# DataZooDE/anofox-forecast

Measured on AMD Instinct MI355X. Metric: series/sec fit+forecast, AutoETS h=28 on M5-shape batches, higher is better.
Workload: dtype f64

## Files before the change

### anofox-forecast_amd/csrc/ets_device.hpp

```cpp
#pragma once
#include <hip/hip_runtime.h>
#include <type_traits>
#include "det_math.hpp"
#include "nm.hpp"

namespace anofox {

enum { C_NONE = 0, C_ADD = 1, C_MUL = 2 };

constexpr double ETS_TOL = 1.0e-10;
constexpr double ETS_HUGEN = 1.0e10;
constexpr double ETS_LN2 = 0.693147180559945309417232121458;
constexpr double PAR_LO = 1.0e-4, PAR_HI = 0.9999, PHI_LO = 0.8, PHI_HI = 0.98;
constexpr int ETS_MERGED_LDS_PERIOD = 16;
constexpr int ETS_LDS_PERIOD = 64;
constexpr int ETS_MAX_PERIOD = 2048;

struct SeriesView {
    const double *y;
    size_t ld;
    int len;
    int wave_len;
    int wave_min_len;
    int rows;
    const double *yb;
    int col;
};

__device__ __forceinline__ int wave_max_i32(int v)
{
#pragma unroll
    for (int o = 32; o >= 1; o >>= 1) { int w = __shfl_xor(v, o); v = w > v ? w : v; }
    return v;
}
__device__ __forceinline__ int wave_min_i32(int v)
{
#pragma unroll
    for (int o = 32; o >= 1; o >>= 1) { int w = __shfl_xor(v, o); v = w < v ? w : v; }
    return v;
}

enum { YT_F64 = 0, YT_F32 = 1, YT_U16 = 2 };
template <class YT> struct YtCode;
template <> struct YtCode<double> { static constexpr int value = YT_F64; };
template <> struct YtCode<float> { static constexpr int value = YT_F32; };
template <> struct YtCode<unsigned short> { static constexpr int value = YT_U16; };
#ifndef ANOFOX_DM_RETRY
#define ANOFOX_DM_RETRY 0
#endif
#ifndef ANOFOX_TWO_BLOCK
#define ANOFOX_TWO_BLOCK 1
#endif
#ifndef ANOFOX_S_DM
#define ANOFOX_S_DM 8
#endif
#ifndef ANOFOX_S_GEN
#define ANOFOX_S_GEN 16
#endif
#ifndef ANOFOX_S_HBM_RING_COMPACT
#define ANOFOX_S_HBM_RING_COMPACT 16
#endif
#ifndef ANOFOX_S_COMPACT_MUL
#define ANOFOX_S_COMPACT_MUL 2
#endif
#ifndef ANOFOX_S_COMPACT_MUL_ADD
#define ANOFOX_S_COMPACT_MUL_ADD 1
#endif
#ifndef ANOFOX_K4_S_SEAS
#define ANOFOX_K4_S_SEAS 8
#endif
template <int ERR, int TREND, bool DAMPED, int SEAS>
struct EtsCfg {
    static constexpr int E = ERR, T = TREND, S = SEAS;
    static constexpr bool D = DAMPED;
    static constexpr int DIM = 1 + (TREND != C_NONE) + (SEAS != C_NONE) + (DAMPED ? 1 : 0);
    static constexpr bool ADDITIVE = (ERR == C_ADD) && (TREND != C_MUL) && (SEAS != C_MUL);
    static constexpr bool CLASSIC = false;
};

struct EtsPar { double alpha, bstar, phi, beta, gamma; DmPowLane pl; DmPowNear1 pc; };
struct EtsState { double l, b, sse, mant; int eacc; int bad; double f; double dlo, dhi, bmin; double rfar; };

template <class Cfg>
__device__ __forceinline__ void ets_unpack(const double (&x)[Cfg::DIM], EtsPar &p)
{
    int k = 0;
    p.alpha = x[k++];
    p.bstar = 0.0;
    double gstar = 0.0;
    p.phi = 1.0;
    if constexpr (Cfg::T != C_NONE) p.bstar = x[k++];
    if constexpr (Cfg::S != C_NONE) gstar = x[k++];
    if constexpr (Cfg::D) p.phi = x[k++];
    p.beta = p.alpha * p.bstar;
    p.gamma = gstar * (1.0 - p.alpha);
}

template <class Cfg, bool NEAR = false>
__device__ __forceinline__ void ets_step(const EtsPar &p, EtsState &st, double y, double &s)
{
    if constexpr (Cfg::ADDITIVE) {
        double phib = 0.0, q = st.l;
        if constexpr (Cfg::T == C_ADD) {
            phib = Cfg::D ? p.phi * st.b : st.b;
            q = st.l + phib;
        }
        double f = q;
        if constexpr (Cfg::S == C_ADD) f = q + s;
        double e = y - f;
        st.sse = fma(e, e, st.sse);
        st.l = fma(p.alpha, e, q);
        st.f = f;
        if constexpr (Cfg::T == C_ADD) st.b = fma(p.beta, e, phib);
        if constexpr (Cfg::S == C_ADD) s = fma(p.gamma, e, s);
    } else {
        double phib = 0.0, q = st.l;
        if constexpr (Cfg::T == C_ADD) {
            phib = Cfg::D ? p.phi * st.b : st.b;
            q = st.l + phib;
        } else if constexpr (Cfg::T == C_MUL) {
            if constexpr (Cfg::D) {
                const double r = st.b - 1.0;
                phib = dm_pow_near1(r, p.pc);
                if constexpr (NEAR) st.rfar = __builtin_fmax(st.rfar, fabs(r));
                else if (!(fabs(r) <= DM_POW_NEAR1_R)) {
                    if (!(st.b >= 0x1p-1000 && st.b <= 0x1p+1000)) st.bad = 1;
                    phib = dm_pow_step(st.b, p.phi, p.pl);
                }
            } else {
                st.bmin = __builtin_fmin(st.bmin, st.b);
                phib = st.b;
            }
            q = st.l * phib;
        }
        double f = q;
        if constexpr (Cfg::S == C_ADD) f = q + s;
        else if constexpr (Cfg::S == C_MUL) f = q * s;
        st.f = f;
        auto recip = [&](const double d) __attribute__((always_inline)) {
            const double ad = fabs(d);
            st.dlo = __builtin_fmin(st.dlo, ad);
            st.dhi = __builtin_fmax(st.dhi, ad);
            return dm_recip(d);
        };
        if constexpr (Cfg::E == C_MUL) {
            static_assert(Cfg::S != C_ADD, "multiplicative error with an additive season is not a valid spec");
            const double rf = recip(f);
            const double eps = (y - f) * rf;
            st.mant = st.mant * fabs(f);
            st.sse = fma(eps, eps, st.sse);
            const double qe = q * eps;
            st.l = fma(p.alpha, qe, q);
            if constexpr (Cfg::T == C_ADD) st.b = fma(p.beta, qe, phib);
            else if constexpr (Cfg::T == C_MUL) st.b = fma(p.beta, phib * eps, phib);
            if constexpr (Cfg::S == C_MUL) s = fma(p.gamma, s * eps, s);
        } else {
            const double e = y - f;
            st.sse = fma(e, e, st.sse);
            if constexpr (Cfg::S == C_MUL && Cfg::T == C_MUL) {
                const double R = recip(f * st.l);
                const double esl = e * (R * q);
                const double es = esl * st.l;
                const double sl = s * st.l;
                st.l = fma(p.alpha, es, q);
                st.b = fma(p.beta, esl, phib);
                s = fma(p.gamma, e * (R * sl), s);
            } else if constexpr (Cfg::S == C_MUL) {
                const double R = recip(f);
                const double es = e * (R * q);
                st.l = fma(p.alpha, es, q);
                if constexpr (Cfg::T == C_ADD) st.b = fma(p.beta, es, phib);
                s = fma(p.gamma, e * (R * s), s);
            } else {
                static_assert(Cfg::T == C_MUL, "general class: a multiplicative component");
                const double rl = recip(st.l);
                st.l = fma(p.alpha, e, q);
                st.b = fma(p.beta, e * rl, phib);
                if constexpr (Cfg::S == C_ADD) s = fma(p.gamma, e, s);
            }
        }
    }
}

template <class Cfg>
__device__ __forceinline__ void ets_renorm(EtsState &st)
{
    if constexpr (Cfg::E == C_MUL) {
        int ex;
        st.mant = frexp(st.mant, &ex);
        st.eacc += ex;
    }
}

template <class Cfg>
__device__ __forceinline__ double ets_objective_value(const EtsState &st, int n)
{
    if (st.bad || !(fabs(st.sse) <= 1.7976931348623157e308)) return __builtin_huge_val();
    if constexpr (!Cfg::ADDITIVE) {
        constexpr double D_LO = Cfg::E == C_MUL ? 0x1p-120 : 0x1p-1000, D_HI = Cfg::E == C_MUL ? 0x1p+120 : 0x1p+1000;
        if (n > 0 && !(st.dlo >= D_LO && st.dhi <= D_HI)) return __builtin_huge_val();
        if constexpr (Cfg::T == C_MUL && !Cfg::D) { if (n > 0 && !(st.bmin > 0.0)) return __builtin_huge_val(); }
    }
    double lik = (double)n * dm_log(st.sse);
    if constexpr (Cfg::E == C_MUL) lik = lik + 2.0 * (dm_log(st.mant) + (double)st.eacc * ETS_LN2);
    if (lik != lik) return __builtin_huge_val();
    if (lik < -1.0e10) lik = -1.0e10;
    return lik;
}

struct EtsInit {
    double l0, b0;
    const double *fig;
    size_t fig_ld;
    int m;
};

struct EtsFinalOut {
    double *yhat; int h; double *sse_out;
    double *fitted; size_t fitted_ld; double *states; size_t states_ld;
    double mean; double *var_out;
};

template <class Cfg, int MS, int K, bool FINAL, class YT = double>
__device__ __forceinline__ void ets_pass(const SeriesView &v, const EtsInit &in,
                                         const double (&cand)[K][Cfg::DIM], double (&fout)[K],
                                         double *ring, const EtsFinalOut *fin)
{
    static_assert((Cfg::S == C_NONE) == (MS == 0), "MS == 0 iff no seasonal component");
    const int lane = threadIdx.x & (NM_BLOCK - 1);
    EtsPar par[K];
    EtsState st[K];
#pragma unroll
    for (int k = 0; k < K; k++) {
        ets_unpack<Cfg>(cand[k], par[k]);
        if constexpr (Cfg::T == C_MUL && Cfg::D) { par[k].pl = dm_pow_lane(); dm_pow_near1_coef(par[k].phi, par[k].pc); }
        st[k].l = in.l0; st[k].b = in.b0; st[k].sse = 0.0; st[k].mant = 1.0; st[k].eacc = 0; st[k].bad = 0;
        st[k].f = 0.0; st[k].dlo = __builtin_huge_val(); st[k].dhi = 0.0; st[k].bmin = __builtin_huge_val(); st[k].rfar = 0.0;

    }
    const double *yp = v.yb;
    const unsigned col_bytes = (unsigned)v.col * (unsigned)sizeof(YT);
    const size_t ld = v.ld;

    const int wave_len = __builtin_amdgcn_readfirstlane(v.wave_len);
    const int wave_min_len = __builtin_amdgcn_readfirstlane(v.wave_min_len);
    const int row_max = __builtin_amdgcn_readfirstlane(v.rows) - 1;
    constexpr int S_WIDE = std::is_same_v<YT, double> ? 1 : (Cfg::ADDITIVE ? ANOFOX_S_COMPACT_MUL_ADD : ANOFOX_S_COMPACT_MUL);
    constexpr int S_FULL = (Cfg::ADDITIVE ? (K == 4 ? (MS > 0 ? ANOFOX_K4_S_SEAS : 16) : 32) : ((Cfg::T == C_MUL && Cfg::D) ? ANOFOX_S_DM : ANOFOX_S_GEN)) * S_WIDE;
    constexpr int S_HBM_CAP = (MS == -2 && !FINAL && !std::is_same_v<YT, double>) ? ANOFOX_S_HBM_RING_COMPACT : 8;
    constexpr int S_TARGET = ((MS == -2 || MS == -4) && K == 1 && S_FULL > S_HBM_CAP) ? S_HBM_CAP : S_FULL;
    constexpr int S = (MS > 0) ? ((S_TARGET / MS > 0 ? S_TARGET / MS : 1) * MS) : S_TARGET;
    typedef std::conditional_t<std::is_same_v<YT, unsigned short>, unsigned, YT> ybuf_t;
    auto widen = [](const ybuf_t x) __attribute__((always_inline)) { return (double)x; };
    ybuf_t cur[S], nxt[S];
    typedef unsigned int u32x2_t __attribute__((ext_vector_type(2)));
    const size_t row_bytes = ld * sizeof(YT);
    const size_t total_bytes = (size_t)(row_max + 1) * row_bytes;
    const int rows_total = row_max + 1;
    auto load_block = [&](ybuf_t (&buf)[S], const int row0) __attribute__((always_inline)) {
        unsigned nrec;
        size_t off;
        if constexpr (Cfg::ADDITIVE) {
            const unsigned rows_left = row0 < rows_total ? (unsigned)(rows_total - row0) : 0u;
            const unsigned long long rem = (unsigned long long)rows_left * (unsigned long long)(unsigned)row_bytes;
            nrec = (unsigned)(rem >> 32) != 0u ? 0xffffffffu : (unsigned)rem;
            off = rows_left ? (size_t)((unsigned long long)(unsigned)row0 * (unsigned long long)(unsigned)row_bytes) : (size_t)0;
        } else {
            const size_t o = (size_t)row0 * row_bytes;
            const size_t rem = o < total_bytes ? total_bytes - o : 0;
            nrec = rem > 0xffffffffull ? 0xffffffffu : (unsigned)rem;
            off = rem ? o : 0;
        }
        const auto rsrc = __builtin_amdgcn_make_buffer_rsrc((void *)((const char *)yp + off), 0, nrec, 0x00020000);
#pragma unroll
        for (int j = 0; j < S; j++) {
            if constexpr (std::is_same_v<YT, double>) {
                const u32x2_t w = __builtin_amdgcn_raw_buffer_load_b64(rsrc, col_bytes, (unsigned)(j * row_bytes), 0);
                buf[j] = __builtin_bit_cast(double, w);
            } else if constexpr (std::is_same_v<YT, float>) {
                const unsigned w = __builtin_amdgcn_raw_buffer_load_b32(rsrc, col_bytes, (unsigned)(j * row_bytes), 0);
                buf[j] = __builtin_bit_cast(float, w);
            } else {
                buf[j] = (unsigned)__builtin_amdgcn_raw_buffer_load_b16(rsrc, col_bytes, (unsigned)(j * row_bytes), 0);
            }
        }
    };
    load_block(cur, 0);
    double var_acc = 0.0;
    auto keep_fit = [&](const int t, const double yv) __attribute__((always_inline)) {
        if constexpr (FINAL) {
            if (fin->fitted && t < v.len) fin->fitted[(size_t)t * fin->fitted_ld] = st[0].f;
            const double dv = yv - fin->mean;
            var_acc += dv * dv;
        }
    };

    if constexpr (MS >= 0) {
        constexpr int MR = MS > 0 ? MS : 1;
        double s[K][MR];
        if constexpr (MS > 0) {
#pragma unroll
            for (int j = 0; j < MS; j++) {
                double f0 = in.fig[(size_t)j * in.fig_ld];
#pragma unroll
                for (int k = 0; k < K; k++) s[k][j] = f0;
            }
        } else {
#pragma unroll
            for (int k = 0; k < K; k++) s[k][0] = 0.0;
        }
        auto run_block = [&](const ybuf_t (&buf)[S], const int base, auto pred_tag) __attribute__((always_inline)) {
            constexpr bool PRED = decltype(pred_tag)::value;
            if constexpr (ANOFOX_DM_RETRY && Cfg::T == C_MUL && Cfg::D && K == 1 && !PRED && !FINAL) {
                const EtsState st0 = st[0];
                double s0[MR];
#pragma unroll
                for (int jj = 0; jj < MR; jj++) s0[jj] = s[0][jj];
                st[0].rfar = 0.0;
#pragma unroll
                for (int j = 0; j < S; j++) {
                    ets_step<Cfg, true>(par[0], st[0], widen(buf[j]), s[0][MS > 0 ? j % MR : 0]);
                    if ((j & 3) == 3 || j == S - 1) ets_renorm<Cfg>(st[0]);
                }
                const bool again = v.len > 0 && (!(st[0].rfar <= DM_POW_NEAR1_R) || st[0].b != st[0].b);
                if (__builtin_amdgcn_ballot_w64(again) == 0ull) return;
                st[0] = st0;
#pragma unroll
                for (int jj = 0; jj < MR; jj++) s[0][jj] = s0[jj];
            }
#pragma unroll
            for (int j = 0; j < S; j++) {
                if (!PRED || base + j < v.len) {
#pragma unroll
                    for (int k = 0; k < K; k++) {
                        ets_step<Cfg>(par[k], st[k], widen(buf[j]), s[k][MS > 0 ? j % MR : 0]);
                        if ((j & 3) == 3 || j == S - 1) ets_renorm<Cfg>(st[k]);
                    }
                    keep_fit(base + j, widen(buf[j]));
                }
            }
        };
        int base = 0;
        constexpr bool TWO = ANOFOX_TWO_BLOCK == 2 || (ANOFOX_TWO_BLOCK == 1 && Cfg::ADDITIVE);
        if constexpr (TWO) {
            for (; base + 2 * S <= wave_min_len; base += 2 * S) {
                load_block(nxt, base + S);
                run_block(cur, base, std::false_type{});
                load_block(cur, base + 2 * S);
                run_block(nxt, base + S, std::false_type{});
            }
        }
        for (; base < wave_len; base += S) {
            load_block(nxt, base + S);
            if (base + S <= wave_min_len) run_block(cur, base, std::false_type{});
            else run_block(cur, base, std::true_type{});
#pragma unroll
            for (int j = 0; j < S; j++) cur[j] = nxt[j];
        }
        if constexpr (FINAL) {
            if constexpr (MS > 0) {
                if (fin->states && v.len > 0) {
#pragma unroll
                    for (int jj = 0; jj < MS; jj++) fin->states[(size_t)(2 + jj) * fin->states_ld] = s[0][jj];
                }
            }
            double pp = par[0].phi, phistar = par[0].phi;
            for (int i = 0; i < fin->h; i++) {
                double f;
                if constexpr (Cfg::T == C_NONE) f = st[0].l;
                else if constexpr (Cfg::T == C_ADD) f = st[0].l + phistar * st[0].b;
                else f = (st[0].b > 0.0) ? st[0].l * dm_pow_pos(st[0].b, phistar) : __builtin_nan("");
                if constexpr (MS > 0) {
                    const int j = (v.len + i) % MS;
                    double sv = s[0][0];
#pragma unroll
                    for (int jj = 1; jj < MS; jj++) sv = (j == jj) ? s[0][jj] : sv;
                    f = (Cfg::S == C_ADD) ? f + sv : f * sv;
                }
                if (v.len > 0) fin->yhat[i] = f;
                pp = pp * par[0].phi;
                phistar = phistar + pp;
            }
        }
    } else {
        constexpr bool LANE_M = MS <= -3;
        static_assert(!LANE_M || K == 1, "per-lane periods: one candidate per lane");
        const int m = LANE_M ? in.m : __builtin_amdgcn_readfirstlane(in.m);
        const int m_max = LANE_M ? __builtin_amdgcn_readfirstlane(wave_max_i32(in.m)) : m;
        for (int j = 0; j < m_max; j++) {
            if (LANE_M && j >= m) continue;
            double f0 = in.fig[(size_t)j * in.fig_ld];
#pragma unroll
            for (int k = 0; k < K; k++) ring[(k * m + j) * NM_BLOCK + lane] = f0;
        }
        int j = 0;
        constexpr bool HBM_RING = (MS == -2 || MS == -4);
        if constexpr (HBM_RING && K == 1) {
            static_assert(2 * S <= ((MS == -2 && !FINAL) ? ETS_LDS_PERIOD : ETS_MERGED_LDS_PERIOD), "the ring prefetch needs periods of at least two blocks");
            double rc[S], rn[S];
            auto ring_load = [&](double (&buf)[S], int j0) __attribute__((always_inline)) {
#pragma unroll
                for (int i = 0; i < S; i++) {
                    buf[i] = ring[(size_t)j0 * NM_BLOCK + lane];
                    j0 = (j0 + 1 == m) ? 0 : j0 + 1;
                }
                return j0;
            };
            int jn = ring_load(rc, 0);
            int base = 0;
            for (; base < wave_len; base += S) {
                load_block(nxt, base + S);
// ... 22 lines not shown
#pragma unroll
                    for (int k = 0; k < K; k++) {
                        double sv = ring[(k * m + j) * NM_BLOCK + lane];
                        ets_step<Cfg>(par[k], st[k], widen(cur[i]), sv);
                        if ((i & 3) == 3 || i == S - 1) ets_renorm<Cfg>(st[k]);
                        ring[(k * m + j) * NM_BLOCK + lane] = sv;
                    }
                    keep_fit(base + i, widen(cur[i]));
                }
                j = (j + 1 == m) ? 0 : j + 1;
            }
        };
        int base = 0;
        for (; base < wave_len; base += S) {
            load_block(nxt, base + S);
            ring_block(base, base + S <= wave_min_len);
#pragma unroll
            for (int i = 0; i < S; i++) cur[i] = nxt[i];
        }
        }
        if constexpr (FINAL) {
            if (fin->states && v.len > 0)
                for (int jj = 0; jj < m; jj++) fin->states[(size_t)(2 + jj) * fin->states_ld] = ring[(0 * m + jj) * NM_BLOCK + lane];
            double pp = par[0].phi, phistar = par[0].phi;
            for (int i = 0; i < fin->h; i++) {
                double f;
                if constexpr (Cfg::T == C_NONE) f = st[0].l;
                else if constexpr (Cfg::T == C_ADD) f = st[0].l + phistar * st[0].b;
                else f = (st[0].b > 0.0) ? st[0].l * dm_pow_pos(st[0].b, phistar) : __builtin_nan("");
                const int jj = (v.len + i) % m;
                double sv = ring[(0 * m + jj) * NM_BLOCK + lane];
                f = (Cfg::S == C_ADD) ? f + sv : f * sv;
                if (v.len > 0) fin->yhat[i] = f;
                pp = pp * par[0].phi;
                phistar = phistar + pp;
            }
        }
    }
#pragma unroll
    for (int k = 0; k < K; k++) {
        ets_renorm<Cfg>(st[k]);
        fout[k] = ets_objective_value<Cfg>(st[k], v.len);
    }
    if constexpr (FINAL) {
        if (fin->sse_out && v.len > 0) *fin->sse_out = st[0].sse;
        if (fin->var_out) *fin->var_out = var_acc;
        if (fin->states && v.len > 0) { fin->states[0] = st[0].l; fin->states[fin->states_ld] = Cfg::T != C_NONE ? st[0].b : __builtin_nan(""); }
    }
}

template <class Cfg, int MS, int CPL, class YT = double>
struct EtsModel {
    static constexpr int DIM = Cfg::DIM;
    SeriesView v;
    EtsInit in;
    double *ring;
    __device__ void bounds(double (&lo)[DIM], double (&hi)[DIM], double (&x0)[DIM]) const
    {
        int k = 0;
        lo[k] = PAR_LO; hi[k] = PAR_HI; x0[k] = 0.3; k++;
        if constexpr (Cfg::T != C_NONE) { lo[k] = PAR_LO; hi[k] = PAR_HI; x0[k] = 0.1; k++; }
        if constexpr (Cfg::S != C_NONE) { lo[k] = PAR_LO; hi[k] = PAR_HI; x0[k] = 0.1; k++; }
        if constexpr (Cfg::D) { lo[k] = PHI_LO; hi[k] = PHI_HI; x0[k] = 0.9; k++; }
    }
    __device__ double eval1(const double (&x)[DIM]) const
    {
        double c1[1][DIM], f1[1];
#pragma unroll
        for (int i = 0; i < DIM; i++) c1[0][i] = x[i];
        ets_pass<Cfg, MS, 1, false, YT>(v, in, c1, f1, ring, nullptr);
        return f1[0];
    }
    __device__ void eval(const double (&cand)[NM_K][DIM], double (&f)[NM_K]) const
    {
        if constexpr (CPL == NM_K) {
            ets_pass<Cfg, MS, NM_K, false, YT>(v, in, cand, f, ring, nullptr);
        } else {
            const int sub = threadIdx.x & 3;
            double mine[1][DIM], f1[1];
#pragma unroll
            for (int i = 0; i < DIM; i++)
                mine[0][i] = sub == 0 ? cand[0][i] : (sub == 1 ? cand[1][i] : (sub == 2 ? cand[2][i] : cand[3][i]));
            ets_pass<Cfg, MS, 1, false, YT>(v, in, mine, f1, ring, nullptr);
            const int base = (threadIdx.x & (NM_BLOCK - 1)) & ~3;
#pragma unroll
            for (int k = 0; k < NM_K; k++) f[k] = __shfl(f1[0], base + k);
        }
    }
};

}
```

### anofox-forecast_amd/csrc/ets_fit_kernel.hpp

```cpp
#pragma once
#include "ets_device.hpp"
#include "classic_device.hpp"
#include "kernels.hpp"

#ifndef ANOFOX_ROUND_WAVES
#define ANOFOX_ROUND_WAVES 2
#endif
namespace anofox {

#ifndef ANOFOX_PARK_CLASS
#define ANOFOX_PARK_CLASS 0
#endif
#ifndef ANOFOX_PARK_WAVES
#define ANOFOX_PARK_WAVES 4
#endif
#ifndef ANOFOX_DM_WPB
#define ANOFOX_DM_WPB 1
#endif
#ifndef ANOFOX_SETPRIO
#define ANOFOX_SETPRIO 0
#endif
#ifndef ANOFOX_ROUND_WAVES_COMPACT
#define ANOFOX_ROUND_WAVES_COMPACT ANOFOX_ROUND_WAVES
#endif
#ifndef ANOFOX_SEQ_WAVES_COMPACT
#define ANOFOX_SEQ_WAVES_COMPACT 0
#endif
template <class Cfg, class YT = double> struct RoundTraits {
    static constexpr bool DAMPED_MUL = !Cfg::CLASSIC && Cfg::T == C_MUL && Cfg::D;
    static constexpr bool PARK = !Cfg::CLASSIC && (ANOFOX_PARK_CLASS >= 3 || (ANOFOX_PARK_CLASS == 2 && !Cfg::ADDITIVE) || (ANOFOX_PARK_CLASS == 1 && DAMPED_MUL));
    static constexpr int WAVES = PARK ? ANOFOX_PARK_WAVES : (std::is_same_v<YT, double> ? ANOFOX_ROUND_WAVES : ANOFOX_ROUND_WAVES_COMPACT);
    static constexpr int WPB = DAMPED_MUL ? ANOFOX_DM_WPB : 1;
};

template <class Cfg, int MS, class YT = double, bool CLASSIC = Cfg::CLASSIC> struct RoundModelOf { using type = EtsModel<Cfg, MS, 1, YT>; };
template <class Cfg, int MS, class YT> struct RoundModelOf<Cfg, MS, YT, true> { using type = ClassicRoundModel<Cfg::KIND, MS>; };

template <class Cfg, int MS, int SPEC, bool K4 = false, class YT = double>
__device__ __forceinline__ void ets_round_body(const FitArgs &a, const int vblock, const int vgrid, const int wave, double *const lds_all)
{
    constexpr int D = Cfg::DIM;
    constexpr bool PARK = RoundTraits<Cfg>::PARK;
    if constexpr (ANOFOX_SETPRIO >= 1 && RoundTraits<Cfg>::DAMPED_MUL) __builtin_amdgcn_s_setprio(3);
    else if constexpr (ANOFOX_SETPRIO >= 2 && !Cfg::CLASSIC && !Cfg::ADDITIVE) __builtin_amdgcn_s_setprio(ANOFOX_SETPRIO == 2 ? 1 : 2);
    if (a.wave_prio == 3) __builtin_amdgcn_s_setprio(3);
    else if (a.wave_prio == 2) __builtin_amdgcn_s_setprio(2);
    else if (a.wave_prio == 1) __builtin_amdgcn_s_setprio(1);
    if constexpr (Cfg::T == C_MUL && Cfg::D) dm_pow_tab_init();
    const int lane = threadIdx.x & (NM_BLOCK - 1);
    const int lds_per_wave = (PARK ? 0 : nm_lds_doubles<D>()) + ((MS == -1 || MS == -3) ? a.m * NM_BLOCK : 0);
    double *const lds = lds_all + (size_t)wave * (size_t)lds_per_wave;
    double *const nmst = PARK ? a.nm_scratch + (size_t)vblock * (size_t)nm_lds_doubles<D>() : lds;
    double *const lds_ring = PARK ? lds : lds + nm_lds_doubles<D>();
    const unsigned long long trace_t0 = a.wave_trace ? __builtin_amdgcn_s_memrealtime() : 0ull;
    const int n_act = a.n_active ? *a.n_active : a.n_series;
    int mode = SPEC;
    if constexpr (SPEC == 3) mode = n_act > a.spec_below ? 0 : ((a.spec2_below > 0 && n_act <= a.spec2_below && n_act <= vgrid) ? 2 : 1);
    else if (a.spec_below >= 0) {
        const int owner = n_act > a.spec_below ? 0 : (n_act > a.spec2_below ? 1 : 2);
        if (owner != SPEC) return;
    }
    const int LPP = mode == 0 ? 1 : (mode == 1 ? NM_K : NM_BLOCK);
    const int PPB = NM_BLOCK / LPP;
    if (vblock * PPB >= n_act) return;
    const int p = vblock * PPB + lane / LPP;
    const bool valid = p < n_act;
    const int s = valid ? (a.series_of ? a.series_of[p] : p) : 0;
    const int len = valid ? a.len[s] : 0;

    const int m = a.m_col ? (MS <= -3 ? a.m_col[s] : __builtin_amdgcn_readfirstlane(a.m_col[s])) : a.m;
    const int n_param = a.n_param - ((Cfg::S != C_NONE && a.m_col) ? a.m - m : 0);
    bool active = valid;
    if (!a.first_round && a.series_of == nullptr && valid && a.st.done[s]) active = false;
    if (a.first_round) {
        int st = FIT_OK;
        if constexpr (Cfg::CLASSIC) {
            const int min_len = Cfg::KIND == CK_HW ? 2 * m : (Cfg::KIND == CK_SEASONAL_ES ? m : a.min_len);
            if (len <= 0 || (a.mask != nullptr && valid && a.mask[s] != a.want)) st = FIT_SKIPPED;
            else if (len < min_len) st = FIT_SHORT;
        } else {
            const uint32_t fl = valid ? a.flags[s] : 0u;
            if (len <= 0) st = FIT_SKIPPED;
            else if (Cfg::S != C_NONE && len < 2 * m) st = FIT_SHORT;
            else if (len < n_param + 2) st = FIT_SHORT;
            else if (a.need_positive && !(fl & SF_POSITIVE)) st = FIT_NONPOSITIVE;
            else if (a.skip_constant && (fl & SF_CONSTANT)) st = FIT_SKIPPED;
        }
        active = valid && st == FIT_OK;
        if (valid) {
            a.status[s] = st;
            if (!active) { a.st.done[s] = 1; a.st.passes[s] = 0; a.st.evals[s] = 0; a.st.iters[s] = 0; }
        }
    }

    SeriesView v;
    const bool gathered = a.gathered != 0 && n_act <= a.gather_cap;
    v.col = valid ? (gathered ? p : s) : 0;
    v.yb = gathered ? a.y_round : a.y;
    v.y = v.yb + v.col;
    v.ld = gathered ? a.ld_round : a.ld;
    v.len = active ? len : 0;
    v.wave_len = wave_max_i32(v.len);
    v.wave_min_len = wave_min_i32(active ? len : 0x7fffffff);
    v.rows = a.t_rows;
    if (v.wave_len == 0) return;

    typename RoundModelOf<Cfg, MS, YT>::type mdl;
    mdl.v = v;
    mdl.in.l0 = (active && !Cfg::CLASSIC) ? a.l0[s] : 0.0;
    mdl.in.b0 = (active && !Cfg::CLASSIC && Cfg::T != C_NONE) ? a.b0[s] : 0.0;
    mdl.in.fig = a.fig ? a.fig + s : nullptr;
    mdl.in.fig_ld = a.fig_ld;
    mdl.in.m = m;
    mdl.ring = (MS == -2 || MS == -4) ? a.ring_scratch + (size_t)vblock * (size_t)a.m * NM_BLOCK : lds_ring;

    NmRun r;
    if (a.first_round) nm_init_simplex(mdl, nmst, r, active);
    else {
#pragma unroll
        for (int k = 0; k <= D; k++) {
#pragma unroll
            for (int i = 0; i < D; i++) nmst[(k * D + i) * NM_BLOCK + lane] = active ? a.st.sim[(size_t)(k * D + i) * a.ld + s] : 0.0;
            nmst[((D + 1) * D + k) * NM_BLOCK + lane] = active ? a.st.fs[(size_t)k * a.ld + s] : 0.0;
        }
        r.phase = active ? a.st.phase[s] : NM_ITER;
        r.evals = active ? a.st.evals[s] : 0;
        r.iters = active ? a.st.iters[s] : 0;
        r.passes = active ? a.st.passes[s] : 0;
        r.done = !active;
    }
    const int passes_in = r.passes;

    const int budget = mode == 2 ? (1 << 30) : ((SPEC == 3 && mode == 0 && !K4) ? a.budget_seq : a.budget);
#define ANOFOX_ADVANCE_LANE()                                                                          \
    do {                                                                                               \
        if constexpr (K4) {                                                                            \
            EtsModel<Cfg, MS, NM_K, YT> mdl4;                                                          \
            mdl4.v = mdl.v; mdl4.in = mdl.in; mdl4.ring = mdl.ring;                                    \
            nm_advance_spec(mdl4, nmst, r, budget);                                                    \
        } else nm_advance_seq(mdl, nmst, r, budget);                                                   \
    } while (0)
    if constexpr (SPEC == 3) {
        if (mode == 2) nm_advance_spec2(mdl, nmst, r, budget);
        else if (mode == 1) nm_advance_spec(mdl, nmst, r, budget);
        else ANOFOX_ADVANCE_LANE();
    } else if constexpr (SPEC == 2) nm_advance_spec2(mdl, nmst, r, budget);
    else if constexpr (SPEC == 1) nm_advance_spec(mdl, nmst, r, budget);
    else ANOFOX_ADVANCE_LANE();
#undef ANOFOX_ADVANCE_LANE
    nm_fence();

    if (a.wave_trace && lane == 0) {
        const unsigned long long slot = atomicAdd(a.wave_trace, 1ull);
        if (slot < a.wave_trace[1]) {
            unsigned long long *rec = a.wave_trace + 4 + 4 * slot;
            rec[0] = a.wave_trace_tag | ((unsigned long long)mode << 8) | (unsigned long long)(K4 ? 4 : 0);
            rec[1] = trace_t0;
            rec[2] = __builtin_amdgcn_s_memrealtime();
            rec[3] = (unsigned long long)__builtin_amdgcn_s_getreg(0xF804) | ((unsigned long long)__builtin_amdgcn_s_getreg(0xF814) << 32);
        }
    }
    if (a.lane_stats) {
        const int mine = r.passes - passes_in;
        int sum = mine;
#pragma unroll
        for (int o = 32; o >= 1; o >>= 1) sum += __shfl_xor(sum, o);
        const int most = wave_max_i32(mine);
        if (lane == 0 && most > 0) {
            atomicAdd(a.lane_stats, (unsigned long long)most);
            atomicAdd(a.lane_stats + 1, (unsigned long long)sum);
        }
    }
    if (active && (lane % LPP) == 0) {
#pragma unroll
        for (int k = 0; k <= D; k++) {
#pragma unroll
            for (int i = 0; i < D; i++) a.st.sim[(size_t)(k * D + i) * a.ld + s] = nmst[(k * D + i) * NM_BLOCK + lane];
            a.st.fs[(size_t)k * a.ld + s] = nmst[((D + 1) * D + k) * NM_BLOCK + lane];
        }
        a.st.phase[s] = r.phase;
        a.st.evals[s] = r.evals;
        a.st.iters[s] = r.iters;
        a.st.passes[s] = r.passes;
        a.st.done[s] = r.done ? 1 : 0;
    }
}

template <class Cfg, int MS, int SPEC, bool K4 = false, class YT = double>
__global__ __launch_bounds__(NM_BLOCK * RoundTraits<Cfg>::WPB, ((ANOFOX_SEQ_WAVES_COMPACT > 0 && SPEC == 0 && !K4 && !std::is_same_v<YT, double> && !Cfg::CLASSIC ? ANOFOX_SEQ_WAVES_COMPACT : RoundTraits<Cfg, YT>::WAVES) + RoundTraits<Cfg>::WPB - 1) / RoundTraits<Cfg>::WPB) void ets_round_kernel(const FitArgs a)
{
    extern __shared__ double lds_all[];
    constexpr int WPB = RoundTraits<Cfg>::WPB;
    const int wave = WPB > 1 ? __builtin_amdgcn_readfirstlane((int)(threadIdx.x >> 6)) : 0;
    ets_round_body<Cfg, MS, SPEC, K4, YT>(a, (int)blockIdx.x * WPB + wave, (int)gridDim.x * WPB, wave, lds_all);
}

template <class Cfg, int MS, class YT = double>
__global__ __launch_bounds__(NM_BLOCK) void ets_final_kernel(const FitArgs a)
{
    extern __shared__ double lds[];
    constexpr int D = Cfg::DIM;
    const int lane = threadIdx.x;
    const int s = blockIdx.x * NM_BLOCK + lane;
    const bool valid = s < a.n_series;
    const int len = valid ? a.len[s] : 0;
    int st = valid ? a.status[s] : FIT_SKIPPED;
    const bool inspect = a.insp_sel != nullptr;
    const bool active = valid && len > 0 && st == FIT_OK && (!inspect || a.insp_sel[s] == a.insp_code);

    SeriesView v;
    v.col = valid ? s : 0;
    v.yb = a.y;
    v.y = a.y + v.col;
    v.ld = a.ld;
    v.len = active ? len : 0;
    v.wave_len = wave_max_i32(v.len);
    v.wave_min_len = wave_min_i32(active ? len : 0x7fffffff);
    v.rows = a.t_rows;
    if (v.wave_len == 0) {
        if (!inspect && valid && len > 0) {
            a.aicc[s] = __builtin_huge_val(); a.evals[s] = 0; a.iters[s] = 0; a.passes[s] = 0;
            if (a.sd_out != nullptr) a.sd_out[s] = 0.0;
        }
// ... 110 lines not shown
```

### anofox-forecast_amd/csrc/host_api.hip

```cpp
#include <hip/hip_runtime.h>

#include <algorithm>
#include <cctype>
#include <atomic>
#include <memory>
#include <unordered_map>
#include <chrono>
#include <cmath>
#include <condition_variable>
#include <mutex>
#include <cstdio>
#include <cstdlib>
#include <cstring>
#include <limits>
#include <map>
#include <stdexcept>
#include <string>
#include <system_error>
#include <thread>
#include <vector>

#include "classic_device.hpp"
#include "host_semantics.hpp"
#include "kernels.hpp"
// ... 12 lines not shown
    ModelType model;
    std::string ets_notation;
    int ets_spec_id = -1;
    int pool = 0;
    std::string static_name;
    double z = 1.645;
};

thread_local unsigned tl_host_thread_share = 1;
std::atomic<int> g_default_arima_method{0};
std::atomic<int> g_arima_runs{0};
thread_local int tl_arima_method = -1;
static int arima_method_in_force() { return tl_arima_method >= 0 ? tl_arima_method : g_default_arima_method.load(); }
struct ArimaMethodScope {
    int saved;
    explicit ArimaMethodScope(int m) : saved(tl_arima_method) { tl_arima_method = m; }
    ~ArimaMethodScope() { tl_arima_method = saved; }
};

}

struct AnofoxHipBatch {
    int dev = 0;
    size_t n = 0, t_max = 0, ld = 0;
    int h = 0;
    ForecastOptions opt;
    Plan plan;
    bool has_block = false, owns_y = false;
    double *d_y = nullptr;
    int32_t *d_len = nullptr;
    bool owns_len = false;
    std::vector<int32_t> h_len;
    bool quiesced = true;
    std::vector<int32_t> h_period;
    std::vector<int32_t> h_base_status;
    std::vector<int32_t> h_slot_spec;
    double *h_stage = nullptr;
    size_t h_stage_elems = 0;
    std::vector<double> h_clean;
    std::vector<size_t> h_clean_off;
    double *d_mean = nullptr, *d_sd = nullptr, *d_fig_add = nullptr, *d_fig_mul = nullptr, *d_l0 = nullptr, *d_b0 = nullptr;
    uint32_t *d_flags = nullptr;
    int fig_m = 0;
    int n_slots_cap = 0;
    double *d_aicc = nullptr, *d_yhat_slots = nullptr;
    int32_t *d_status_slots = nullptr, *d_evals_slots = nullptr, *d_iters_slots = nullptr, *d_passes_slots = nullptr, *d_slot_spec = nullptr;
    float *d_yc32 = nullptr;
    unsigned short *d_yc16 = nullptr;
    size_t yc_cells = 0;
    unsigned int *d_misfit = nullptr;
    unsigned int h_misfit[2] = {1u, 1u};
    int y_type = 0;
    unsigned long long *d_wave_trace = nullptr;
    unsigned long long *d_lane_stats = nullptr;
    double *d_yhat = nullptr, *d_lo = nullptr, *d_hi = nullptr;
    int32_t *d_model_code = nullptr, *d_status = nullptr, *d_detail = nullptr, *d_passes_total = nullptr, *d_evals_total = nullptr;
    uint32_t *d_mask = nullptr;
    int32_t *d_len_group = nullptr;
    int32_t *d_count = nullptr;
    int32_t *d_pos_map = nullptr, *d_pos_cnt = nullptr, *d_notpos = nullptr;
    double *d_ypos = nullptr;
    bool use_pos = false;
    bool none_pos = false;
    std::vector<anofox::FitArgs> insp_args;
    std::vector<anofox::FitLaunchers> insp_fns;
    std::vector<int> insp_spec, insp_stream;
    bool insp_ok = false;
    int insp_m = 1;
    int32_t live_pos = -1, live_all = -1;
    int arima_method = 0;
    size_t ar_ws_bytes = 0;
    double *ar_w = nullptr, *ar_wmean = nullptr, *ar_wsd = nullptr, *ar_l0 = nullptr, *ar_l1 = nullptr, *ar_x = nullptr, *ar_aicc = nullptr;
    int32_t *ar_wlen = nullptr, *ar_d = nullptr, *ar_D = nullptr, *ar_order = nullptr, *ar_status = nullptr, *ar_evals = nullptr, *ar_passes = nullptr, *ar_models = nullptr;
    StreamSet *sset = nullptr;
    hipStream_t own_stream = nullptr;
    hipStream_t aux[N_AUX_STREAMS] = {};
    hipEvent_t ev_start = nullptr, ev_stop = nullptr, ev_fit0 = nullptr, ev_fit1 = nullptr, ev_fork = nullptr;
    hipEvent_t ev_join[N_AUX_STREAMS] = {};
    struct Lane {
        double *ybuf = nullptr;
        size_t ybuf_cols = 0;
        int32_t *map[2] = {nullptr, nullptr};
        int32_t *cnt = nullptr;
        anofox::NmStateBuf st{};
        double *nm_scratch = nullptr;
        size_t nm_scratch_doubles = 0;
    } lanes[N_AUX_STREAMS];
    anofox::FitArgs *d_group_tab = nullptr, *h_group_tab = nullptr;
    size_t group_tab_cap = 0;
    hipEvent_t ev_group_tab = nullptr;
    hipStream_t last_stream = nullptr;
    bool ran = false, timed_fit = false;
    uint32_t fit_launches = 0;
    uint64_t n_problems = 0;
    Tunables tun;
    int seq_rounds = 3;
    int seq_rounds_env = -1;
    int spec_below_md = 8192;
    anofox::NmStateBuf classic_st{};
    int32_t *d_classic_status = nullptr, *classic_map[2] = {nullptr, nullptr}, *classic_cnt = nullptr;
    double *d_classic_ybuf = nullptr;
    size_t classic_ybuf_cols = 0;
    std::vector<void *> retired;
    int merged_m_max = 0;
    int32_t *d_m_col = nullptr;
    int spec2_below_md = 2048;
    int spec2_below = 1024;
    int spec_below = 8192;
    bool use_gather = false;
    double gather_budget = 0.0;
    bool sd_in_final = false;
    double *d_ring = nullptr;
    size_t ring_elems = 0;
    double *d_prep_scratch = nullptr;
    size_t prep_scratch_elems = 0;
    bool fixed_params = false;
    double fixed_x[4] = {0.0, 0.0, 0.0, 0.0};
    int32_t *d_im_level = nullptr, *d_im_gmax = nullptr;
    double *d_im_fc = nullptr;
    size_t im_fc_elems = 0;
    double *d_th_sidx = nullptr;
    size_t th_sidx_elems = 0;
    int32_t *d_th_adj = nullptr;
    int exog_k = 0;
    const double *d_exog_x = nullptr, *d_exog_f = nullptr;
    bool owns_exog = false;
    double *d_exog_b0 = nullptr, *d_exog_beta = nullptr;
    uint32_t *d_exog_used = nullptr;
};

namespace {

bool make_plan(const ForecastOptions *o, Plan &p, AnofoxError *err)
{
    std::string mname = cstr_field(o->model, sizeof o->model);
    if (!parse_model(mname, p.model)) {
// ... 70 lines not shown
void fill_nulls_interpolate(const double *values, const uint64_t *validity, size_t n, double *out)
{
    auto valid = [&](size_t i) { return validity == nullptr || ((validity[i / 64] >> (i % 64)) & 1ull); };
    long first = -1, last = -1;
    for (size_t i = 0; i < n; i++)
        if (valid(i)) { if (first < 0) first = (long)i; last = (long)i; }
    for (size_t i = 0; i < n; i++) out[i] = std::nan("");
    if (first < 0) return;
    for (long i = 0; i < first; i++) out[i] = values[first];
    for (size_t i = (size_t)last + 1; i < n; i++) out[i] = values[last];
    long prev = first;
    double pv = values[first];
    out[first] = pv;
    for (long i = first + 1; i <= last; i++) {
        if (valid((size_t)i)) {
            double v = values[i];
            long gap = i - prev;
            if (gap > 1) {
                double slope = (v - pv) / (double)gap;
                for (long j = 1; j < gap; j++) out[prev + j] = pv + slope * (double)j;
            }
            out[i] = v;
            prev = i;
            pv = v;
        }
    }
}

void batch_attach_streams(AnofoxHipBatch *b)
{
    if (b->sset) return;
    b->sset = stream_set_take();
    b->own_stream = b->sset->own;
    for (int i = 0; i < N_AUX_STREAMS; i++) { b->aux[i] = b->sset->aux[i]; b->ev_join[i] = b->sset->ev_join[i]; }
    b->ev_start = b->sset->ev_start; b->ev_stop = b->sset->ev_stop; b->ev_fit0 = b->sset->ev_fit0; b->ev_fit1 = b->sset->ev_fit1;
    b->ev_fork = b->sset->ev_fork;
}
void batch_detach_streams(AnofoxHipBatch *b)
{
    if (!b->sset) return;
    stream_set_give(b->sset);
    b->sset = nullptr; b->own_stream = nullptr; b->last_stream = nullptr; b->ran = false;
    for (auto &q : b->aux) q = nullptr;
}

void free_batch_buffers(AnofoxHipBatch *b)
{
    auto F = [](void *p) { dev_free(p, true); };
    if (b->owns_y) F(b->d_y);
    pin_free(b->h_stage);
    if (b->owns_len) F(b->d_len);
    F(b->d_mean); F(b->d_sd); F(b->d_fig_add); F(b->d_fig_mul); F(b->d_l0); F(b->d_b0); F(b->d_flags);
    F(b->d_aicc); F(b->d_yhat_slots); F(b->d_status_slots); F(b->d_evals_slots); F(b->d_iters_slots);
    F(b->d_passes_slots); F(b->d_slot_spec); F(b->d_lane_stats); F(b->d_wave_trace); F(b->d_yc32); F(b->d_yc16); F(b->d_misfit);
    F(b->d_yhat); F(b->d_lo); F(b->d_hi); F(b->d_model_code); F(b->d_status); F(b->d_detail);
    F(b->classic_st.sim); F(b->classic_st.fs); F(b->classic_st.phase); F(b->classic_st.evals); F(b->classic_st.iters); F(b->classic_st.passes); F(b->classic_st.done);
    F(b->d_classic_ybuf); F(b->d_classic_status); F(b->classic_map[0]); F(b->classic_map[1]); F(b->classic_cnt);
    for (void *p : b->retired) F(p);
    b->retired.clear();
    F(b->d_m_col); F(b->d_ring); F(b->d_prep_scratch);
    F(b->d_group_tab); pin_free(b->h_group_tab); b->d_group_tab = b->h_group_tab = nullptr; b->group_tab_cap = 0;
    if (b->ev_group_tab) { (void)hipEventDestroy(b->ev_group_tab); b->ev_group_tab = nullptr; }
    F(b->d_im_level); F(b->d_im_gmax); F(b->d_im_fc);
    F(b->d_th_sidx); F(b->d_th_adj);
    if (b->owns_exog) { F((void *)b->d_exog_x); F((void *)b->d_exog_f); }
    b->d_exog_x = b->d_exog_f = nullptr; b->owns_exog = false; b->exog_k = 0;
    F(b->d_exog_b0); F(b->d_exog_beta); F(b->d_exog_used);
    F(b->d_passes_total); F(b->d_evals_total); F(b->d_mask); F(b->d_len_group); F(b->d_count); F(b->d_pos_map); F(b->d_pos_cnt); F(b->d_notpos); F(b->d_ypos);
    F(b->ar_w); F(b->ar_wmean); F(b->ar_wsd); F(b->ar_l0); F(b->ar_l1); F(b->ar_x); F(b->ar_aicc); F(b->ar_wlen); F(b->ar_d); F(b->ar_D);
    F(b->ar_order); F(b->ar_status); F(b->ar_evals); F(b->ar_passes); F(b->ar_models);
    batch_detach_streams(b);
    for (auto &l : b->lanes) {
        F(l.ybuf); l.ybuf_cols = 0; F(l.map[0]); F(l.map[1]); F(l.cnt);
        F(l.st.sim); F(l.st.fs); F(l.st.phase); F(l.st.evals); F(l.st.iters); F(l.st.passes); F(l.st.done);
        F(l.nm_scratch); l.nm_scratch_doubles = 0;
    }
}

int max_slots_for(const Plan &p)
{
    if (p.model == M_AutoETS) return 30;
    if (p.model == M_ETS && p.ets_spec_id >= 0) return 1;
    return 0;
}

void alloc_common(AnofoxHipBatch *b)
{
    const size_t n = b->n, ld = b->ld, h = (size_t)std::max(b->h, 0);
    b->d_mean = dalloc<double>(ld);
    b->d_sd = dalloc<double>(ld);
    b->d_flags = dalloc<uint32_t>(ld);
    b->d_yhat = dalloc<double>(n * h);
    b->d_lo = dalloc<double>(n * h);
    b->d_hi = dalloc<double>(n * h);
    b->d_model_code = dalloc<int32_t>(ld);
    b->d_status = dalloc<int32_t>(ld);
    b->d_detail = dalloc<int32_t>(ld);
    b->d_passes_total = dalloc<int32_t>(ld);
    b->d_evals_total = dalloc<int32_t>(ld);
    b->d_mask = dalloc<uint32_t>(ld);
    b->d_len_group = dalloc<int32_t>(ld);
    b->d_count = dalloc<int32_t>(2);
    if (b->plan.model == M_AutoETS) {
        b->d_pos_map = dalloc<int32_t>(ld); b->d_pos_cnt = dalloc<int32_t>(2); b->d_notpos = dalloc<int32_t>(ld);
    }
    if (is_intermittent_model(b->plan.model)) {
        b->d_im_level = dalloc<int32_t>(ld);
        b->d_im_gmax = dalloc<int32_t>((size_t)intermittent_groups((int)n) + 1);
    }
    if (is_theta_model(b->plan.model)) b->d_th_adj = dalloc<int32_t>(ld);
    if (b->plan.model == M_AutoARIMA) {
        const size_t T = std::max<size_t>(b->t_max, 1);
        b->ar_ws_bytes = arima_workspace_bytes((int)b->n, (int)T);
        b->ar_w = (double *)dalloc<char>(b->ar_ws_bytes);
        HIPCHECK(hipMemset(b->ar_w, 0, b->ar_ws_bytes));
        b->ar_wmean = dalloc<double>(ld); b->ar_wsd = dalloc<double>(ld); b->ar_l0 = dalloc<double>(ld); b->ar_l1 = dalloc<double>(ld);
        b->ar_x = dalloc<double>(6 * ld); b->ar_aicc = dalloc<double>(ld);
        b->ar_wlen = dalloc<int32_t>(ld); b->ar_d = dalloc<int32_t>(ld); b->ar_D = dalloc<int32_t>(ld); b->ar_order = dalloc<int32_t>(5 * ld);
        b->ar_status = dalloc<int32_t>(ld); b->ar_evals = dalloc<int32_t>(ld); b->ar_passes = dalloc<int32_t>(ld); b->ar_models = dalloc<int32_t>(ld);
        HIPCHECK(hipMemset(b->ar_wlen, 0, ld * sizeof(int32_t)));
    }
    HIPCHECK(hipMemset(b->d_model_code, 0, ld * sizeof(int32_t)));
    HIPCHECK(hipMemset(b->d_detail, 0, ld * sizeof(int32_t)));
    HIPCHECK(hipMemset(b->d_passes_total, 0, ld * sizeof(int32_t)));
    HIPCHECK(hipMemset(b->d_evals_total, 0, ld * sizeof(int32_t)));
    HIPCHECK(hipMemset(b->d_mask, 0, ld * sizeof(uint32_t)));
    b->n_slots_cap = max_slots_for(b->plan);
    if (b->n_slots_cap > 0) {
        const size_t S = (size_t)b->n_slots_cap;
        b->d_l0 = dalloc<double>(9 * ld);
        b->d_b0 = dalloc<double>(9 * ld);
        b->d_aicc = dalloc<double>(S * ld);
        b->d_yhat_slots = dalloc<double>(S * n * h);
        b->d_status_slots = dalloc<int32_t>(S * ld);
        b->d_evals_slots = dalloc<int32_t>(S * ld);
        b->d_iters_slots = dalloc<int32_t>(S * ld);
        b->d_passes_slots = dalloc<int32_t>(S * ld);
        b->d_slot_spec = dalloc<int32_t>(S);
        b->d_lane_stats = dalloc<unsigned long long>(2 * S);
        HIPCHECK(hipMemset(b->d_lane_stats, 0, 2 * S * sizeof(unsigned long long)));
        const int n_lanes = std::min<int>(N_AUX_STREAMS, b->n_slots_cap);
        for (int q = 0; q < n_lanes; q++) {
            auto &l = b->lanes[q];
            l.map[0] = dalloc<int32_t>(ld);
            l.map[1] = dalloc<int32_t>(ld);
            l.cnt = dalloc<int32_t>(3);
            l.st.sim = dalloc<double>(20 * ld);
            l.st.fs = dalloc<double>(5 * ld);
            l.st.phase = dalloc<int32_t>(ld);
            l.st.evals = dalloc<int32_t>(ld);
            l.st.iters = dalloc<int32_t>(ld);
            l.st.passes = dalloc<int32_t>(ld);
            l.st.done = dalloc<int32_t>(ld);
        }
    }
    batch_attach_streams(b);
}

void ensure_fig(AnofoxHipBatch *b, int m)
{
    if (m <= b->fig_m) return;
    if (b->d_fig_add) b->retired.push_back(b->d_fig_add);
    if (b->d_fig_mul) b->retired.push_back(b->d_fig_mul);
    b->d_fig_add = nullptr; b->d_fig_mul = nullptr; b->fig_m = 0;
    b->d_fig_add = dalloc<double>((size_t)m * b->ld);
    b->d_fig_mul = dalloc<double>((size_t)m * b->ld);
    b->fig_m = m;
}

double *ensure_ring(AnofoxHipBatch *b, size_t elems)
{
    if (b->ring_elems < elems) {
        if (b->d_ring) b->retired.push_back(b->d_ring);
        b->d_ring = nullptr; b->ring_elems = 0;
        b->d_ring = dalloc<double>(elems);
        b->ring_elems = elems;
    }
    return b->d_ring;
}
double *ensure_prep_scratch(AnofoxHipBatch *b, size_t elems)
{
    if (b->prep_scratch_elems < elems) {
        if (b->d_prep_scratch) b->retired.push_back(b->d_prep_scratch);
        b->d_prep_scratch = nullptr; b->prep_scratch_elems = 0;
        b->d_prep_scratch = dalloc<double>(elems);
        b->prep_scratch_elems = elems;
    }
    return b->d_prep_scratch;
}

void detect_periods_block(const double *d_y, size_t ld, const int32_t *d_len, size_t n, size_t t_rows, int32_t *h_out, hipStream_t st)
{
    if (n == 0) return;
    int32_t *d_per = dalloc<int32_t>(n);
    const size_t sc = detect_scratch_doubles((int)n, (int)t_rows);
    double *d_sc = sc ? dalloc<double>(sc) : nullptr;
    try {
        launch_detect_periods(d_y, ld, d_len, (int)n, (int)t_rows, d_sc, d_per, nullptr, st);
        LAUNCHCHECK("seasonal period detection");
        HIPCHECK(hipMemcpyAsync(h_out, d_per, n * sizeof(int32_t), hipMemcpyDeviceToHost, st));
        HIPCHECK(hipStreamSynchronize(st));
    } catch (...) { dev_free(d_per); dev_free(d_sc); throw; }
    dev_free(d_per, true);
    dev_free(d_sc, true);
}

// ... 361 lines not shown
    const int yt = b->y_type;
    const void *ybase = yt == YT_F32 ? (const void *)b->d_yc32 : (yt == YT_U16 ? (const void *)b->d_yc16 : (const void *)b->d_y);
    const int ybytes = yt == YT_F32 ? 4 : (yt == YT_U16 ? 2 : 8);
    const int lds_limit = merged ? ETS_MERGED_LDS_PERIOD : ETS_LDS_PERIOD;
    const bool inline_stream = specs.size() == 1;
    const int n_fork = inline_stream ? 0 : n_lanes;
    auto spec_stream = [&](int idx) -> hipStream_t { return inline_stream ? st : b->aux[idx]; };
    std::vector<size_t> order(specs.size());
    for (size_t i = 0; i < order.size(); i++) order[i] = i;
    auto cost = [&](int id) {
        static const int measured[30] = { 3, 8, 14,  7, 13, 27,  17, 29, 41,  14, 26, 22,  63, 92, 84,
                                          7, 0, 15,  18, 0, 29,  33, 0, 48,  16, 0, 28,  65, 0, 95};
        return (id >= 0 && id < 30 && measured[id] > 0) ? measured[id] : 1;
    };
    auto work = [&](int id) {
        const double live = (b->live_all >= 0 && spec_has_mult(id)) ? (double)b->live_pos : (b->live_all >= 0 ? (double)b->live_all : 1.0);
        return (double)cost(id) * (live + 1.0);
    };
    std::stable_sort(order.begin(), order.end(), [&](size_t x, size_t y) { return work(specs[x]) > work(specs[y]); });
    std::vector<int> stream_of(order.size());
    for (size_t oi = 0; oi < order.size(); oi++) stream_of[oi] = (int)(oi % (size_t)n_lanes);
    std::vector<FitArgs> args(order.size());
    std::vector<FitLaunchers> fns(order.size());
    for (size_t oi = 0; oi < order.size(); oi++) {
        const size_t k = order[oi];
        const int id = specs[k];
        const int q = (int)(oi % (size_t)n_lanes);
        auto &lane = b->lanes[q];
        const int se = spec_season(id), ti = spec_trend_idx(id);
        const int tt = ti == 0 ? 0 : (ti <= 2 ? 1 : 2);
        FitArgs &a = args[oi];
        a = FitArgs{};
        a.y = (const double *)ybase; a.ld = ld; a.len = d_len; a.n_series = (int)n; a.t_rows = (int)std::max<size_t>(b->t_max, 1);
        a.m = se != 0 ? m : 1; a.h = b->h;
        a.l0 = b->d_l0 + (size_t)(se * 3 + tt) * ld;
        a.b0 = b->d_b0 + (size_t)(se * 3 + tt) * ld;
        a.fig = se == 1 ? b->d_fig_add : (se == 2 ? b->d_fig_mul : nullptr);
        a.fig_ld = ld;
        a.flags = b->d_flags;
        a.need_positive = spec_has_mult(id) ? 1 : 0;
        a.skip_constant = skip_constant ? 1 : 0;
        a.n_param = spec_n_param(id, a.m);
        a.aicc = b->d_aicc + k * ld;
        a.yhat = b->d_yhat_slots + k * n * (size_t)b->h;
        a.status = b->d_status_slots + k * ld;
        a.evals = b->d_evals_slots + k * ld;
        a.iters = b->d_iters_slots + k * ld;
        a.passes = b->d_passes_slots + k * ld;
        a.st = lane.st;
        a.ring_scratch = nullptr;
        a.m_col = b->d_m_col;
        if (b->sd_in_final && order.size() == 1) { a.mean = b->d_mean; a.sd_out = b->d_sd; }
        a.lane_stats = b->d_lane_stats ? b->d_lane_stats + 2 * k : nullptr;
        a.wave_trace = b->d_wave_trace;
        fns[oi] = ets_fit_launcher(id, (merged && se != 0) ? (a.m > lds_limit ? ETS_PERLANE_HBM : ETS_PERLANE_LDS) : a.m, yt);
        if (!fns[oi].round_seq || !fns[oi].round_spec || !fns[oi].round_auto || !fns[oi].final) throw HipFail{"no kernel for ETS spec id " + std::to_string(id)};
    }
    {
        size_t n_long = 0;
        for (size_t oi = 0; oi < order.size(); oi++) if (args[oi].m > lds_limit) n_long++;
        if (n_long) {
            const bool tiny_batch = (uint64_t)n * order.size() <= (uint64_t)TINY_BATCH_PROBLEMS;
            const size_t wg = std::max<size_t>((n + 15) / 16, std::min<size_t>(n, tiny_batch ? n : (size_t)std::max(b->spec2_below, b->spec2_below_md)));
            const size_t per_spec = wg * (size_t)m * 64u;
            if ((double)n_long * (double)per_spec * 8.0 > 64.0 * 1073741824.0)
                throw HipFail{"seasonal period " + std::to_string(m) + " on " + std::to_string(n) + " series needs more than 64 GiB of ring scratch: shard the batch"};
            double *base = ensure_ring(b, n_long * per_spec);
            size_t k = 0;
            for (size_t oi = 0; oi < order.size(); oi++) if (args[oi].m > lds_limit) { args[oi].ring_scratch = base + (k++) * per_spec; args[oi].ring_scratch_doubles = per_spec; }
        }
    }
    {
        const bool tiny_batch = (uint64_t)n * order.size() <= (uint64_t)TINY_BATCH_PROBLEMS;
        const size_t wg = std::max<size_t>((n + 15) / 16, std::min<size_t>(n, tiny_batch ? n : (size_t)std::max(b->spec2_below, b->spec2_below_md)));
        for (size_t oi = 0; oi < order.size(); oi++) {
            if (!fns[oi].nm_scratch_per_wg) continue;
            auto &lane = b->lanes[oi % (size_t)n_lanes];
            const size_t need = (wg + 8) * fns[oi].nm_scratch_per_wg;
            if (lane.nm_scratch_doubles < need) {
                if (lane.nm_scratch) b->retired.push_back(lane.nm_scratch);
                lane.nm_scratch = nullptr; lane.nm_scratch_doubles = 0;
                lane.nm_scratch = dalloc<double>(need);
                lane.nm_scratch_doubles = need;
            }
            args[oi].nm_scratch = lane.nm_scratch; args[oi].nm_scratch_doubles = lane.nm_scratch_doubles;
        }
    }
    std::vector<char> dead(order.size(), 0);
    if (b->none_pos && !b->fixed_params)
        for (size_t oi = 0; oi < order.size(); oi++)
            if (args[oi].need_positive) dead[oi] = 1;
    std::vector<char> k4(order.size(), 0);
    {
        bool all_additive = true;
        for (size_t oi = 0; oi < order.size(); oi++)
            if (!dead[oi] && spec_has_mult(specs[order[oi]]) && !(b->live_all > 0 && b->live_pos >= 0 && 2 * (int64_t)b->live_pos < (int64_t)b->live_all))
                all_additive = false;
        int64_t additive_live = 0;
        for (size_t oi = 0; oi < order.size(); oi++)
            if (!dead[oi] && !spec_has_mult(specs[order[oi]])) additive_live += b->live_all >= 0 ? (int64_t)b->live_all : (int64_t)n;
        int64_t all_live = 0;
        for (size_t oi = 0; oi < order.size(); oi++)
            if (!dead[oi]) all_live += (spec_has_mult(specs[order[oi]]) && b->live_pos >= 0) ? (int64_t)b->live_pos : (b->live_all >= 0 ? (int64_t)b->live_all : (int64_t)n);
        const bool on = b->tun.k4 > 0 || (b->tun.k4 < 0 && yt == YT_F64 && ((all_additive && additive_live >= 131072) || all_live >= 524288));
        for (size_t oi = 0; oi < order.size(); oi++)
            k4[oi] = on && !dead[oi] && !b->fixed_params && !spec_has_mult(specs[order[oi]]) && fns[oi].round_k4 && fns[oi].round_auto_k4;
// ... 94 lines not shown
            else add(of_class[GROUP_GENERAL], GROUP_GENERAL);
            add(of_class[GROUP_ADDITIVE], GROUP_ADDITIVE);
            grouped = !groups.empty();
        }
        if (grouped) {
            for (size_t g = 0; g < groups.size(); g++) {
                const bool dm = spec_trend_idx(specs[order[groups[g][0]]]) == 4;
                group_stream.push_back(dm ? (int)g : N_AUX_STREAMS - 1 - (int)g);
                for (size_t oi : groups[g]) { group_of[oi] = (int)g; stream_of[oi] = group_stream[g]; slot_of[oi] = n_slots++; }
            }
            for (size_t oi = 0; oi < order.size(); oi++) if (dead[oi]) stream_of[oi] = group_stream[0];
        }
    }
    bool emit = true;
    std::vector<int> slot_blocks, slot_k4;
    GroupCompactArgs gc{};
    GroupGatherArgs gg{};
    int gg_cols = 0;
    auto run_round = [&](const size_t oi, const int kind, const FitArgs &a, hipStream_t sq, const int r) {
        if (!grouped) {
            const FitLaunchFn f = kind == RK_SEQ ? fns[oi].round_seq : kind == RK_SPEC ? fns[oi].round_spec : kind == RK_SPEC2 ? fns[oi].round_spec2 :
                                  kind == RK_AUTO ? fns[oi].round_auto : kind == RK_K4 ? fns[oi].round_k4 : fns[oi].round_auto_k4;
            f(a, sq);
            return;
        }
        if (emit) return;
        FitArgs t = a;
        if (kind == RK_SEQ || kind == RK_K4) { t.spec_below = -1; t.spec2_below = -1; t.budget_seq = t.budget; }
        else if (kind == RK_SPEC) { t.spec_below = 0x7fffffff; t.spec2_below = -1; }
        else if (kind == RK_SPEC2) throw HipFail{"launch_fit_slots: the one-wave-per-problem round of a tiny batch has no group form"};
        const int g_seq = (int)((n + NM_BLOCK - 1) / NM_BLOCK);
        const int g_spec = (int)((std::min<int64_t>((int64_t)n, std::max(t.spec_below, 0)) + NM_BLOCK / NM_K - 1) / (NM_BLOCK / NM_K));
        const int g_spec2 = (int)std::min<int64_t>((int64_t)n, std::max(t.spec2_below, 0));
        const int blocks = std::max(g_seq, std::max(g_spec, g_spec2));
        if (t.ring_scratch != nullptr && (size_t)blocks * (size_t)t.m * NM_BLOCK > t.ring_scratch_doubles)
            throw HipFail{"launch_fit_slots: the seasonal-ring scratch does not cover a group slot"};
        const size_t cell = (size_t)r * n_slots + slot_of[oi];
        b->h_group_tab[cell] = t;
        slot_blocks[cell] = blocks;
        slot_k4[cell] = (kind == RK_K4 || kind == RK_AUTO_K4) ? 1 : 0;
    };
    auto enqueue_round = [&](const int r, const size_t oi) {
            if (dead[oi]) return;
            const int q = (int)(oi % (size_t)n_lanes);
            auto &lane = b->lanes[q];
            hipStream_t sq = spec_stream(stream_of[oi]);
            FitArgs &a = args[oi];
            const bool spec_mode = r >= b->seq_rounds;
            a.first_round = (r == 0);
            a.wave_trace_tag = ((unsigned long long)specs[order[oi]] << 32) | ((unsigned long long)r << 16);
            a.wave_prio = (int)oi < b->tun.prio_top ? std::max(1, 3 - (int)oi) : 0;
            a.spec_below = -1; a.spec2_below = -1;
            a.gathered = 0;
            if (tiny) {
                a.y_round = b->d_y; a.ld_round = ld; a.series_of = nullptr; a.n_active = nullptr;
                a.budget = 1 << 30; a.budget_seq = a.budget;
                run_round(oi, RK_SPEC2, a, sq, r);
                b->fit_launches++;
                return;
            }
            if (r == 0 && b->use_pos && a.need_positive) {
                if (emit)
                    hipLaunchKernelGGL(retire_nonpositive_kernel, dim3((unsigned)((n + 255) / 256)), dim3(256), 0, sq, (int)n, d_len, b->d_notpos,
                                       a.status, lane.st.done, lane.st.passes, lane.st.evals, lane.st.iters);
                a.series_of = b->d_pos_map; a.n_active = b->d_pos_cnt;
                if (b->d_ypos) { a.y_round = b->d_ypos; a.ld_round = ld; a.gathered = 1; a.gather_cap = (int)ld; }
                else { a.y_round = b->d_y; a.ld_round = ld; }
            } else if (r == 0) {
                a.y_round = a.y; a.ld_round = ld; a.series_of = nullptr; a.n_active = nullptr;
            } else {
                const int32_t *prev_map = (r == 1) ? nullptr : lane.map[(r - 1) & 1];
                const int32_t *prev_cnt = (r == 1) ? nullptr : lane.cnt + ((r - 1) % 3);
                if (emit && !grouped && r == 1) HIPCHECK(hipMemsetAsync(lane.cnt, 0, 3 * sizeof(int32_t), sq));
                if (emit && !grouped) launch_compact(prev_map, prev_cnt, (int)n, lane.st.done, lane.map[r & 1], lane.cnt + (r % 3), sq, lane.cnt + ((r + 1) % 3));
                if (emit && grouped) {
                    const int k = gc.n_slots++;
                    gc.prev[k] = prev_map; gc.n_prev[k] = prev_cnt; gc.done[k] = lane.st.done;
                    gc.next[k] = lane.map[r & 1]; gc.n_next[k] = lane.cnt + (r % 3); gc.n_clear[k] = lane.cnt + ((r + 1) % 3);
                }
                a.series_of = lane.map[r & 1]; a.n_active = lane.cnt + (r % 3);
                if (b->use_gather && lane.ybuf) {
                    if (emit && !grouped)
                        launch_gather_columns(a.y, ld, lane.map[r & 1], lane.cnt + (r % 3), (int)n, (int)b->t_max, lane.ybuf, lane.ybuf_cols, sq,
                                              (int)lane.ybuf_cols, ybytes);
                    if (emit && grouped) {
                        const int k = gg.n_slots++;
                        gg.series_of[k] = lane.map[r & 1]; gg.n_active[k] = lane.cnt + (r % 3);
                        gg.out[k] = lane.ybuf; gg.ld_out[k] = lane.ybuf_cols; gg.cap[k] = (int)lane.ybuf_cols;
                        gg_cols = std::max(gg_cols, (int)std::min<size_t>(n, lane.ybuf_cols));
                    }
                    a.y_round = lane.ybuf; a.ld_round = lane.ybuf_cols; a.gathered = 1; a.gather_cap = (int)lane.ybuf_cols;
                } else {
                    a.y_round = a.y; a.ld_round = ld;
                }
            }
            const int s2 = (spec_trend_idx(specs[order[oi]]) == 4) ? b->spec2_below_md : b->spec2_below;
            if (fill_mode && !k4[oi]) {
                const int64_t live_i = (spec_has_mult(specs[order[oi]]) && b->live_pos >= 0) ? (int64_t)b->live_pos : (b->live_all >= 0 ? (int64_t)b->live_all : (int64_t)n);
                const int s2v = (int)std::max<int64_t>(32, std::min<int64_t>(s2 > 0 ? s2 : 32, live_i / std::max(1, b->tun.fill_s2_div)));
                a.budget = BUDGET[r]; a.budget_seq = (BUDGET[r] * 7) / 4;
                if (r == 0) {
                    if (fill_spec4[oi]) run_round(oi, RK_SPEC, a, sq, r);
                    else { a.budget = a.budget_seq; run_round(oi, RK_SEQ, a, sq, r); }
                } else {
                    a.spec_below = fill_spec4[oi] ? 0x7fffffff : (int)std::max<int64_t>(64, live_i / std::max(1, b->tun.fill_late_div));
                    a.spec2_below = s2v;
                    run_round(oi, RK_AUTO, a, sq, r);
                }
                if (!grouped) b->fit_launches++;
                return;
            }
            if (k4[oi]) {
                a.budget = BUDGET[r]; a.budget_seq = BUDGET[r];
                const int64_t live = b->live_all >= 0 ? b->live_all : (int64_t)n;
                const int sb = ((int)oi < b->tun.k4_top && b->tun.k4_top_below > 0) ? b->tun.k4_top_below : b->spec_below;
                if (r == 0) run_round(oi, live > sb ? RK_K4 : RK_SPEC, a, sq, r);
                else {
                    a.spec_below = sb; a.spec2_below = s2 > 0 ? s2 : -1;
                    run_round(oi, RK_AUTO_K4, a, sq, r);
                }
            } else if (r == 0 || b->seq_rounds_env >= 0 || b->seq_rounds == 0) {
                a.budget = spec_mode ? BUDGET[r] : (BUDGET[r] * 7) / 4;
                if (spec_mode && r > 0 && s2 > 0) {
                    a.spec_below = 0x7fffffff; a.spec2_below = s2; a.budget_seq = a.budget;
                    run_round(oi, RK_AUTO, a, sq, r);
                } else
                    run_round(oi, spec_mode ? RK_SPEC : RK_SEQ, a, sq, r);
            } else {
                a.spec_below = (spec_trend_idx(specs[order[oi]]) == 4) ? b->spec_below_md : b->spec_below;
                a.spec2_below = s2 > 0 ? s2 : -1;
                if ((int)oi < b->tun.top_boost_n) {
                    a.spec_below = (int)std::min<int64_t>(0x7fffffff, (int64_t)a.spec_below * b->tun.top_boost_pct / 100);
                    if (a.spec2_below > 0) a.spec2_below = (int)std::min<int64_t>(0x7fffffff, (int64_t)a.spec2_below * b->tun.top_boost_pct / 100);
                }
                a.budget_seq = (BUDGET[r] * 7) / 4;
                a.budget = BUDGET[r];
                run_round(oi, RK_AUTO, a, sq, r);
            }
            if (!grouped) b->fit_launches++;
    };
    if (grouped) {
        const size_t cells = (size_t)total_rounds * n_slots;
        if (b->ev_group_tab) HIPCHECK(hipEventSynchronize(b->ev_group_tab));
        else HIPCHECK(hipEventCreateWithFlags(&b->ev_group_tab, hipEventDisableTiming));
        if (b->group_tab_cap < cells) {
            if (b->d_group_tab) b->retired.push_back(b->d_group_tab);
            pin_free(b->h_group_tab);
            b->d_group_tab = nullptr; b->h_group_tab = nullptr; b->group_tab_cap = 0;
            b->d_group_tab = dalloc<FitArgs>(cells);
            b->h_group_tab = (FitArgs *)pin_alloc_bytes(cells * sizeof(FitArgs));
            b->group_tab_cap = cells;
        }
        slot_blocks.assign(cells, 0); slot_k4.assign(cells, 0);
        emit = false;
        for (int r = 0; r < total_rounds; r++) for (size_t oi = 0; oi < order.size(); oi++) enqueue_round(r, oi);
        emit = true;
        HIPCHECK(hipMemcpyAsync(b->d_group_tab, b->h_group_tab, cells * sizeof(FitArgs), hipMemcpyHostToDevice, st));
        HIPCHECK(hipEventRecord(b->ev_group_tab, st));
        HIPCHECK(hipEventRecord(b->ev_fork, st));
        for (int q : group_stream) HIPCHECK(hipStreamWaitEvent(b->aux[q], b->ev_fork, 0));
    } else
        for (int i = 0; i < n_fork; i++) HIPCHECK(hipStreamWaitEvent(b->aux[i], b->ev_fit0, 0));
    for (size_t oi = 0; oi < order.size(); oi++)
        if (dead[oi]) {
            const FitArgs &a = args[oi];
            hipLaunchKernelGGL(retire_nonpositive_kernel, dim3((unsigned)((n + 255) / 256)), dim3(256), 0, spec_stream(stream_of[oi]), (int)n, d_len,
                               b->d_notpos, a.status, a.st.done, a.st.passes, a.st.evals, a.st.iters, a.aicc, a.passes, a.evals, a.iters);
        }
    if (b->fixed_params) {
        for (size_t oi = 0; oi < order.size(); oi++) {
            const int id = specs[order[oi]];
            FitArgs &a = args[oi];
            double x[4] = {0.0, 0.0, 0.0, 0.0};
            int d = 0;
            x[d++] = b->fixed_x[0];
            if (spec_trend_idx(id) != 0) x[d++] = b->fixed_x[1];
            if (spec_season(id) != 0) x[d++] = b->fixed_x[2];
            if (spec_trend_idx(id) == 2 || spec_trend_idx(id) == 4) x[d++] = b->fixed_x[3];
            hipLaunchKernelGGL(ets_fixed_setup_kernel, dim3((unsigned)((n + 255) / 256)), dim3(256), 0, spec_stream(stream_of[oi]), (int)n, ld, d_len,
                               b->d_flags, spec_season(id) != 0 ? 1 : 0, a.m, a.n_param, a.need_positive, d, x[0], x[1], x[2], x[3], a.status,
                               a.st.sim, a.st.evals, a.st.iters, a.st.passes, a.st.done);
        }
        LAUNCHCHECK("ETS fixed-parameter setup");
    }
    auto enqueue_group_round = [&](const int r, const size_t g) {
        hipStream_t sg = b->aux[group_stream[g]];
        if (r == 0) {
            int32_t *zero[GROUP_MAX_SLOTS] = {};
            for (size_t k = 0; k < groups[g].size(); k++) zero[k] = b->lanes[groups[g][k] % (size_t)n_lanes].cnt;
            launch_group_zero3((int)groups[g].size(), zero, sg);
        }
        gc = GroupCompactArgs{}; gc.n_series = (int)n;
        gg = GroupGatherArgs{}; gg.t_max = (int)b->t_max; gg.elem_bytes = ybytes; gg.y = ybase; gg.ld = ld; gg_cols = 0;
        for (size_t oi : groups[g]) enqueue_round(r, oi);
        if (gc.n_slots > 0) launch_group_compact(gc, sg);
        if (gg.n_slots > 0) launch_group_gather(gg, gg_cols, sg);
        GroupRoundArgs ga{};
        ga.n_slots = (int)groups[g].size();
        const size_t row = (size_t)r * n_slots + slot_of[groups[g][0]];
        for (int k = 0; k < ga.n_slots; k++) {
            const size_t oi = groups[g][(size_t)k];
            ga.spec[k] = specs[order[oi]];
            ga.k4[k] = slot_k4[(size_t)r * n_slots + slot_of[oi]];
            ga.start[k + 1] = ga.start[k] + slot_blocks[(size_t)r * n_slots + slot_of[oi]];
        }
        group_fn[g](b->d_group_tab + row, ga, m, sg);
        b->fit_launches++;
    };
    int head = 0;
    if (grouped && total_rounds > 0 && b->tun.dm_head_rounds > 0 && groups.size() > 1 && group_stream[0] == 0 &&
        spec_trend_idx(specs[order[groups[0][0]]]) == 4) {
        head = std::min(b->tun.dm_head_rounds, total_rounds);
        for (int r = 0; r < head; r++) enqueue_group_round(r, 0);
        LAUNCHCHECK("ETS fit head rounds");
        HIPCHECK(hipEventRecord(b->ev_join[0], b->aux[0]));
        for (size_t g = 1; g < groups.size(); g++) HIPCHECK(hipStreamWaitEvent(b->aux[group_stream[g]], b->ev_join[0], 0));
    } else if (!grouped && !tiny && !inline_stream && total_rounds > 0 && b->tun.dm_head_rounds > 0) {
        std::vector<size_t> dm, rest;
        for (size_t oi = 0; oi < order.size(); oi++)
            if (!dead[oi]) (spec_trend_idx(specs[order[oi]]) == 4 ? dm : rest).push_back(oi);
        if (!dm.empty() && !rest.empty()) {
            head = std::min(b->tun.dm_head_rounds, total_rounds);
            for (int r = 0; r < head; r++) for (size_t oi : dm) enqueue_round(r, oi);
            LAUNCHCHECK("ETS fit head rounds");
            for (size_t oi : dm) HIPCHECK(hipEventRecord(b->ev_join[stream_of[oi]], spec_stream(stream_of[oi])));
            for (size_t oi : rest) for (size_t od : dm) HIPCHECK(hipStreamWaitEvent(spec_stream(stream_of[oi]), b->ev_join[stream_of[od]], 0));
        }
    }
    for (int r = 0; r < total_rounds; r++) {
        if (grouped) {
            for (size_t g = 0; g < groups.size(); g++) if (!(r < head && g == 0)) enqueue_group_round(r, g);
        } else
            for (size_t oi = 0; oi < order.size(); oi++) {
                if (r < head && spec_trend_idx(specs[order[oi]]) == 4) continue;
                enqueue_round(r, oi);
            }
        LAUNCHCHECK("ETS fit round");
    }
    if (b->fixed_params && order.size() == 1) HIPCHECK(hipEventRecord(b->ev_fit0, spec_stream(stream_of[0])));
    for (size_t oi = 0; oi < order.size(); oi++) if (!dead[oi]) fns[oi].final(args[oi], spec_stream(stream_of[oi]));
    if (b->fixed_params && order.size() == 1) HIPCHECK(hipEventRecord(b->ev_fit1, spec_stream(stream_of[0])));
    LAUNCHCHECK("ETS final pass");
    if (grouped)
        for (int q : group_stream) {
            HIPCHECK(hipEventRecord(b->ev_join[q], b->aux[q]));
            HIPCHECK(hipStreamWaitEvent(st, b->ev_join[q], 0));
// ... 266 lines not shown
        aa.m = period > 1 ? period : 1;
        aa.long_scratch = nullptr;
        aa.m_col = (b->d_m_col && aa.m > 24) ? b->d_m_col : nullptr;
        if (aa.m > 24) aa.long_scratch = ensure_ring(b, arima_long_scratch_doubles((int)n, aa.m, arima_max_fit_waves()));
        aa.h = b->h;
        aa.ws = b->ar_w; aa.ws_bytes = b->ar_ws_bytes; aa.t_max = (int)std::max<size_t>(b->t_max, 1); aa.wlen = b->ar_wlen; aa.d = b->ar_d; aa.D = b->ar_D; aa.wmean = b->ar_wmean; aa.wsd = b->ar_wsd;
        aa.last_d0 = b->ar_l0; aa.last_d1 = b->ar_l1; aa.order = b->ar_order; aa.xbest = b->ar_x; aa.aicc = b->ar_aicc;
        aa.status = b->d_detail; aa.evals = b->d_evals_total; aa.passes = b->d_passes_total; aa.models = b->ar_models;
        aa.yhat = b->d_yhat; aa.model_code = b->d_model_code;
        aa.ml_refit = b->arima_method == ANOFOX_ARIMA_CSS_ML ? 1 : 0;
        aa.trace = b->tun.arima_trace;
        aa.lookahead = b->tun.arima_lookahead; aa.lookahead_depth = b->tun.arima_lookahead_depth; aa.spec_factor = b->tun.arima_spec_factor; aa.refit_budget = b->tun.arima_refit_budget; aa.queue_sort = b->tun.arima_queue_sort;
        aa.prep_lanes = b->tun.arima_prep_lanes < 1 ? 1 : (b->tun.arima_prep_lanes > 64 ? 64 : b->tun.arima_prep_lanes);
        aa.concurrent = &g_arima_runs; aa.shared_chunk_rounds = b->tun.arima_shared_chunk_rounds;
        HIPCHECK(hipEventRecord(b->ev_fit0, st));
        struct RunCount { RunCount() { g_arima_runs.fetch_add(1); } ~RunCount() { g_arima_runs.fetch_sub(1); } } run_count;
        try { b->fit_launches += launch_arima(aa, st); }
        catch (const std::exception &e) { throw HipFail{e.what()}; }
        HIPCHECK(hipEventRecord(b->ev_fit1, st));
        b->timed_fit = true;
        b->n_problems += n;
        finish();
        break;
    }
    case M_CrostonClassic: case M_CrostonSBA: case M_TSB: case M_ADIDA: case M_IMAPA: {
        prep(1, false);
        run_intermittent(b, d_len, st);
        finish();
        break;
    }
    case M_DynamicTheta: case M_DynamicOptimizedTheta: {
        prep(1, false);
        run_theta(b, period, d_len, st);
        finish();
        break;
    }
    default: throw HipFail{"model not implemented"};
    }
    LAUNCHCHECK(model_name(p.model));
}

void run_batch(AnofoxHipBatch *b, hipStream_t st)
{
    const size_t n = b->n, ld = b->ld;
    (void)hipGetLastError();
    b->fit_launches = 0;
    b->n_problems = 0;
    b->timed_fit = false;
    b->insp_ok = false;
    b->quiesced = false;
    b->last_stream = st;
    HIPCHECK(hipEventRecord(b->ev_start, st));
    if (b->d_lane_stats) HIPCHECK(hipMemsetAsync(b->d_lane_stats, 0, 2 * (size_t)b->n_slots_cap * sizeof(unsigned long long), st));
    if (!b->tun.wave_trace.empty() && b->n_slots_cap > 0) {
        constexpr size_t WAVE_TRACE_RECORDS = 4u << 20;
        if (!b->d_wave_trace) b->d_wave_trace = dalloc<unsigned long long>(4 + 4 * WAVE_TRACE_RECORDS);
        const unsigned long long head[4] = {0ull, (unsigned long long)WAVE_TRACE_RECORDS, 0ull, 0ull};
        HIPCHECK(hipMemcpyAsync(b->d_wave_trace, head, sizeof head, hipMemcpyHostToDevice, st));
        HIPCHECK(hipStreamSynchronize(st));
    }
    {
        const size_t nh = n * (size_t)std::max(b->h, 0);
        const size_t cover = std::max<size_t>(std::max(nh, ld), 1);
        hipLaunchKernelGGL(seed_outputs_kernel, dim3((unsigned)((cover + 255) / 256)), dim3(256), 0, st, (int)n, (int)ld, nh, (const int32_t *)b->d_len, b->d_status,
                           b->d_yhat, b->d_lo, b->d_hi, b->d_passes_total, b->d_evals_total, b->d_model_code);
        LAUNCHCHECK("output seeding");
    }
    auto used_period = [&](int period) {
        switch (b->plan.model) {
        case M_Naive: case M_RandomWalkDrift: case M_ARIMA: case M_SES: case M_SESOptimized: case M_Holt: return 1;
        case M_CrostonClassic: case M_CrostonSBA: case M_TSB: case M_ADIDA: case M_IMAPA: return 1;
        case M_AutoARIMA:
            if (exog_in_force(b)) return 1;
            return period > ETS_MAX_PERIOD ? ETS_MAX_PERIOD + 1 : (period > 1 ? period : 1);
        default: return period;
        }
    };
    std::map<int, std::vector<size_t>> groups;
    bool uniform = true;
    for (size_t s = 1; s < n; s++) if (used_period(b->h_period[s]) != used_period(b->h_period[0])) { uniform = false; break; }
    if (b->d_m_col) run_group(b, b->merged_m_max, b->d_len, st);
    else if (uniform) run_group(b, n ? used_period(b->h_period[0]) : 1, b->d_len, st);
    else {
        for (size_t s = 0; s < n; s++) groups[used_period(b->h_period[s])].push_back(s);
        std::vector<int32_t> eff(ld);
        for (auto &g : groups) {
            std::fill(eff.begin(), eff.end(), 0);
            for (size_t s : g.second) if (b->h_base_status[s] == 0) eff[s] = b->h_len[s];
            HIPCHECK(hipStreamSynchronize(st));
            HIPCHECK(hipMemcpy(b->d_len_group, eff.data(), ld * sizeof(int32_t), hipMemcpyHostToDevice));
            run_group(b, g.first, b->d_len_group, st);
        }
    }
    IntervalArgs ia{};
    ia.n_series = (int)n; ia.h = b->h; ia.yhat = b->d_yhat; ia.sd = b->d_sd; ia.status = b->d_status; ia.z = b->plan.z;
    ia.lower = b->d_lo; ia.upper = b->d_hi;
    launch_intervals(ia, st);
    LAUNCHCHECK("intervals");
    HIPCHECK(hipEventRecord(b->ev_stop, st));
    b->last_stream = st;
    b->ran = true;
    b->quiesced = false;
}

std::string series_error_message(const AnofoxHipBatch *b, size_t s, int code, int detail)
{
// ... 438 lines not shown
    return true;
}

bool anofox_hip_selftest_recip(uint64_t n_operands, uint64_t seed, uint64_t *out_mismatches, double *out_first_bad)
{
    if (!out_mismatches) return false;
    AnofoxError err;
    if (!device_ready(&err)) return false;
    double fb = 0.0;
    const unsigned long long r = anofox::recip_selftest(n_operands, seed, &fb, nullptr);
    if (r == ~0ull) return false;
    *out_mismatches = r;
    if (out_first_bad) *out_first_bad = fb;
    return true;
}

bool anofox_hip_batch_lane_stats(AnofoxHipBatch *b, AnofoxHipLaneStats *out, size_t struct_size)
{
    if (!b || !out || !b->ran || struct_size < sizeof(uint64_t)) return false;
    DeviceGuard guard(b->dev);
    AnofoxHipLaneStats r;
    std::memset(&r, 0, sizeof r);
    r.struct_size = sizeof r;
    if (hipEventSynchronize(b->ev_stop) != hipSuccess) return false;
    if (b->d_wave_trace && !b->tun.wave_trace.empty()) {
        unsigned long long head[4] = {0, 0, 0, 0};
        if (hipMemcpy(head, b->d_wave_trace, sizeof head, hipMemcpyDeviceToHost) != hipSuccess) return false;
        const size_t used = (size_t)std::min(head[0], head[1]);
        std::vector<unsigned long long> rec(4 * used);
        if (used && hipMemcpy(rec.data(), b->d_wave_trace + 4, rec.size() * sizeof(unsigned long long), hipMemcpyDeviceToHost) != hipSuccess) return false;
        if (FILE *f = std::fopen(b->tun.wave_trace.c_str(), "wb")) {
            std::fwrite(head, sizeof head, 1, f);
            if (used) std::fwrite(rec.data(), sizeof(unsigned long long), rec.size(), f);
            std::fclose(f);
        }
    }
    if (b->insp_ok && b->d_lane_stats && !b->fixed_params) {
        std::vector<unsigned long long> c(2 * (size_t)b->n_slots_cap);
        if (hipMemcpy(c.data(), b->d_lane_stats, c.size() * sizeof(unsigned long long), hipMemcpyDeviceToHost) != hipSuccess) return false;
        for (size_t k = 0; k < b->h_slot_spec.size() && k < (size_t)b->n_slots_cap; k++) {
            const int id = b->h_slot_spec[k];
            const int cls = !spec_has_mult(id) ? 0 : (spec_trend_idx(id) == 4 ? 2 : 1);
            r.wave_passes[cls] += c[2 * k];
            r.live_lane_passes[cls] += c[2 * k + 1];
            if (k < 30) { r.slot_spec_id[k] = id; r.slot_wave_passes[k] = c[2 * k]; r.slot_live_lane_passes[k] = c[2 * k + 1]; r.n_slots = (uint32_t)(k + 1); }
        }
    }
    const size_t nbytes = std::min(struct_size, sizeof r);
    r.struct_size = nbytes;
    std::memcpy(out, &r, nbytes);
    return true;
}

bool anofox_hip_batch_device_results(AnofoxHipBatch *b, void **d_yhat, void **d_lower, void **d_upper, void **d_model_code,
                                     void **d_status)
{
    if (!b) return false;
    if (d_yhat) *d_yhat = b->d_yhat;
    if (d_lower) *d_lower = b->d_lo;
    if (d_upper) *d_upper = b->d_hi;
    if (d_model_code) *d_model_code = b->d_model_code;
    if (d_status) *d_status = b->d_status;
    return true;
}

void anofox_hip_model_name(const ForecastOptions *options, int32_t model_code, char out_name[64])
{
    out_name[0] = 0;
    if (model_code >= 1000000) { auto_arima_name(model_code, options ? options->seasonal_period : 1, out_name); return; }
    if (model_code >= 100 && model_code < 130) { auto_ets_name(model_code - 100, out_name); return; }
    if (model_code == MODEL_CODE_ARIMAX) { std::snprintf(out_name, 64, "ARIMAX"); return; }
    Plan p;
    AnofoxError e;
    if (options && make_plan(options, p, &e)) {
        std::snprintf(out_name, 64, "%s", p.static_name.c_str());
    }
}

void anofox_hip_batch_model_name(const AnofoxHipBatch *b, size_t series, int32_t model_code, char out_name[64])
{
    out_name[0] = 0;
    if (!b) return;
    if (model_code >= 1000000) {
        const int period = (series < b->h_period.size()) ? b->h_period[series] : (b->opt.seasonal_period > 0 ? b->opt.seasonal_period : 1);
        auto_arima_name(model_code, period, out_name);
        return;
    }
    anofox_hip_model_name(&b->opt, model_code, out_name);
}

bool anofox_hip_batch_fetch(AnofoxHipBatch *b, ForecastResult *out_results, AnofoxError *out_errors)
{
    if (!b || !out_results || !b->ran) return false;
    DeviceGuard guard(b->dev);
    const size_t n = b->n, h = (size_t)std::max(b->h, 0);
    if (hipStreamSynchronize(b->last_stream) != hipSuccess) return false;
    b->quiesced = true;
    const size_t nh = n * h;
    struct PinBlock { void *p = nullptr; ~PinBlock() { pin_free(p); } } pin;
    try { pin.p = pin_alloc_bytes(std::max<size_t>(3 * nh * sizeof(double) + 3 * n * sizeof(int32_t), 64)); }
    catch (...) { return false; }
    double *const yhat = (double *)pin.p, *const lo = yhat + nh, *const hi = lo + nh;
    int32_t *const status = (int32_t *)(hi + nh), *const code = status + n, *const detail = code + n;
    bool ok = true;
    hipStream_t cs = b->last_stream;
    if (nh) {
// ... 4235 lines not shown
```

### anofox-forecast_amd/csrc/host_resources.hpp

```cpp
#pragma once

constexpr int N_AUX_STREAMS = 32;

struct HipFail { std::string msg; bool oom = false; };
void report_hip_failure(AnofoxError *out_error, const HipFail &f)
{
    if (f.oom) anofox::set_error(out_error, ALLOCATION_ERROR, "Allocation error: " + f.msg);
    else anofox::set_error(out_error, INTERNAL_ERROR, "Internal error: " + f.msg);
}
#define HIPCHECK(expr)                                                                             \
    do {                                                                                           \
        hipError_t _e = (expr);                                                                    \
        if (_e != hipSuccess) throw HipFail{std::string(#expr) + ": " + hipGetErrorString(_e), _e == hipErrorOutOfMemory};    \
    } while (0)

#define LAUNCHCHECK(what)                                                                          \
    do {                                                                                           \
        hipError_t _e = hipGetLastError();                                                         \
        if (_e != hipSuccess) throw HipFail{std::string("kernel launch failed (") + (what) + "): " + hipGetErrorString(_e), false};    \
    } while (0)

constexpr int32_t STATUS_NOT_COMPUTED = -1;

struct Tunables {
    std::vector<int> budgets{24, 24, 24, 24, 24, 24, 48, 48, 96, 96, 192, 1024};
    int seq_rounds = -1;
    int gather_cols = 0;
    int gather = -1;
    int spec_below = 8192;
    int spec_below_md = 8192;
    int spec2_below = 1024;
    int spec2_below_md = 2048;
    int k4 = -1;
    int k4_top = 1, k4_top_below = 20480;
    std::string wave_trace;
    int compact = -1;
    int fill_policy = 1;
    int fill_target = 150;
    int fill_late_div = 2;
    int fill_s2_div = 16;
    int top_boost_n = 0, top_boost_pct = 200;
    int prio_top = 0;
    int group_launch = 1;
    int group_split = 1;
    int dm_head_rounds = 0;
    bool merge_periods = true;
    int part_threads = 16;
    int pack_threads = 0;
    bool timing = false;
    int arima_trace = 0;
    double arima_lookahead = 6.0;
    int arima_lookahead_depth = 2;
    double arima_spec_factor = 4.0;
    double arima_shared_chunk_rounds = 1.0;
    int arima_prep_lanes = 64;
    int arima_queue_sort = 1;
    int arima_refit_budget = 100;
    static std::map<std::string, std::string> tune_map()
    {
        std::map<std::string, std::string> kv;
        const char *e = std::getenv("ANOFOX_HIP_TUNE");
        if (!e) return kv;
        std::string all(e);
        for (size_t pos = 0; pos < all.size();) {
            size_t end = all.find(';', pos);
            if (end == std::string::npos) end = all.size();
            const std::string item = all.substr(pos, end - pos);
            const size_t eq = item.find('=');
            if (eq != std::string::npos) {
                std::string k = item.substr(0, eq), v = item.substr(eq + 1);
                while (!k.empty() && k.front() == ' ') k.erase(k.begin());
                while (!k.empty() && k.back() == ' ') k.pop_back();
                kv[k] = v;
            }
            pos = end + 1;
        }
        return kv;
    }
    static Tunables from_env()
    {
        Tunables t;
        const std::map<std::string, std::string> kv = tune_map();
        auto geti = [&](const char *k, int &v) { auto it = kv.find(k); if (it != kv.end()) v = std::atoi(it->second.c_str()); };
        auto getd = [&](const char *k, double &v) { auto it = kv.find(k); if (it != kv.end()) v = std::atof(it->second.c_str()); };
        if (kv.count("budgets")) {
            std::vector<int> v;
            for (const char *q = kv.at("budgets").c_str(); *q;) {
                char *end = nullptr;
                long x = std::strtol(q, &end, 10);
                if (end == q) break;
                if (x > 0) v.push_back((int)x);
                q = (*end == ',') ? end + 1 : end;
            }
            if (!v.empty()) t.budgets = v;
        }
        if (kv.count("wave_trace")) t.wave_trace = kv.at("wave_trace");
        geti("compact", t.compact); geti("prio_top", t.prio_top); geti("top_boost_n", t.top_boost_n); geti("top_boost_pct", t.top_boost_pct);
        geti("fill_policy", t.fill_policy); geti("fill_target", t.fill_target); geti("fill_late_div", t.fill_late_div); geti("fill_s2_div", t.fill_s2_div);
        geti("seq_rounds", t.seq_rounds);
        geti("gather", t.gather);
        if (kv.count("spec_below")) t.spec_below = t.spec_below_md = std::atoi(kv.at("spec_below").c_str());
        geti("spec_below_md", t.spec_below_md);
        geti("gather_cols", t.gather_cols);
        geti("group_launch", t.group_launch); geti("group_split", t.group_split);
        geti("k4", t.k4); geti("dm_head_rounds", t.dm_head_rounds); geti("k4_top", t.k4_top); geti("k4_top_below", t.k4_top_below);
        if (kv.count("spec2_below")) t.spec2_below = t.spec2_below_md = std::atoi(kv.at("spec2_below").c_str());
        geti("spec2_below_md", t.spec2_below_md);
        if (kv.count("merge_periods")) t.merge_periods = std::atoi(kv.at("merge_periods").c_str()) != 0;
        geti("part_threads", t.part_threads);
        if (kv.count("arima_trace")) t.arima_trace = std::atoi(kv.at("arima_trace").c_str());
        getd("arima_lookahead", t.arima_lookahead);
        geti("arima_lookahead_depth", t.arima_lookahead_depth);
        getd("arima_spec_factor", t.arima_spec_factor);
        geti("arima_queue_sort", t.arima_queue_sort);
        geti("arima_prep_lanes", t.arima_prep_lanes);
        getd("arima_shared_chunk_rounds", t.arima_shared_chunk_rounds);
        geti("arima_refit_budget", t.arima_refit_budget);
        if (const char *e = std::getenv("ANOFOX_HIP_PACK_THREADS")) t.pack_threads = std::max(1, std::atoi(e));
        t.timing = std::getenv("ANOFOX_HIP_TIMING") != nullptr;
        return t;
    }
};
struct ProcessTunables {
    double cache_gb = -1.0, pinned_cache_gb = 2.0;
    double coalesce_us = 1000.0;
    int prio_streams = -1;
    std::string devices;
    static const ProcessTunables &get()
    {
        static const ProcessTunables t = [] {
            ProcessTunables p;
            if (const char *e = std::getenv("ANOFOX_HIP_CACHE_GB")) p.cache_gb = std::atof(e);
            if (const char *e = std::getenv("ANOFOX_HIP_PINNED_CACHE_GB")) p.pinned_cache_gb = std::atof(e);
            { const auto kv = Tunables::tune_map(); auto it = kv.find("prio_streams"); if (it != kv.end()) p.prio_streams = std::atoi(it->second.c_str()); }
            if (const char *e = std::getenv("ANOFOX_HIP_COALESCE_US")) p.coalesce_us = std::atof(e);
            if (const char *e = std::getenv("ANOFOX_HIP_DEVICES")) p.devices = e;
            return p;
        }();
        return t;
    }
};

struct DeviceGuard {
    int prev = -1;
    bool switched = false;
    explicit DeviceGuard(int dev)
    {
        if (hipGetDevice(&prev) == hipSuccess && prev != dev) switched = hipSetDevice(dev) == hipSuccess;
    }
    ~DeviceGuard() { if (switched) (void)hipSetDevice(prev); }
};

struct DevCache {
    struct Idle { int dev; size_t size; void *ptr; };
    std::mutex mu;
    std::map<uint64_t, Idle> by_age;
    std::multimap<std::pair<int, size_t>, uint64_t> by_key;
// ... 406 lines not shown
```

### anofox-forecast_amd/csrc/kernels.hip

```cpp
#include "classic_device.hpp"
#include "fit_units.hpp"
#include "kernels.hpp"

namespace anofox {

__global__ __launch_bounds__(NM_BLOCK) void select_kernel(const SelectArgs a)
{
    const int s = blockIdx.x * NM_BLOCK + threadIdx.x;
    if (s >= a.n_series) return;
    if (a.len[s] <= 0) { a.fallback_mask[s] = 0u; return; }
    int best = -1;
    double best_aicc = __builtin_huge_val();
    int passes = 0, evals = 0;
    for (int k = 0; k < a.n_slots; k++) {
        passes += a.passes_slots[(size_t)k * a.ld + s];
        evals += a.evals_slots[(size_t)k * a.ld + s];
        if (a.status_slots[(size_t)k * a.ld + s] != FIT_OK) continue;
        double v = a.aicc[(size_t)k * a.ld + s];
        if (v < best_aicc) { best_aicc = v; best = k; }
    }
    a.passes_total[s] = passes;
    a.evals_total[s] = evals;
    if (best < 0) {
        a.status[s] = -1;
// ... 222 lines not shown
        keep = done[s] == 0;
    }
    const unsigned long long bal = __ballot(keep);
    const int cnt = __popcll(bal);
    if (cnt == 0) return;
    int base = 0;
    if (lane == 0) base = atomicAdd(n_next_ptr, cnt);
    base = __shfl(base, 0);
    const int before = __popcll(bal & ((1ull << lane) - 1ull));
    if (keep) series_next[base + before] = s;
}

void launch_compact(const int32_t *series_prev, const int32_t *n_prev, int n_series, const int32_t *done,
                    int32_t *series_next, int32_t *n_next, hipStream_t stream, int32_t *n_clear)
{
    if (!n_clear) anofox_check_attr(hipMemsetAsync(n_next, 0, sizeof(int32_t), stream));
    const int grid = (n_series + NM_BLOCK - 1) / NM_BLOCK;
    hipLaunchKernelGGL(compact_kernel, dim3(grid), dim3(NM_BLOCK), 0, stream, series_prev, n_prev, n_series, done, series_next, n_next, n_clear);
}

constexpr int GATHER_TB = 32;
template <class E>
__global__ __launch_bounds__(NM_BLOCK) void gather_columns_kernel(const E *y, size_t ld, const int32_t *series_of,
                                                                  const int32_t *n_active, int t_max, E *out, size_t ld_out, int cap)
{
    const int n_act = *n_active;
    if ((int)blockIdx.x * NM_BLOCK >= n_act || n_act > cap) return;
    const int p = blockIdx.x * NM_BLOCK + threadIdx.x;
    const int s = series_of[p < n_act ? p : n_act - 1];
    const int t0 = blockIdx.y * GATHER_TB;
    const int t1 = t0 + GATHER_TB < t_max ? t0 + GATHER_TB : t_max;
    for (int t = t0; t < t1; t++) out[(size_t)t * ld_out + p] = y[(size_t)t * ld + s];
}

void launch_gather_columns(const void *y, size_t ld, const int32_t *series_of, const int32_t *n_active, int n_series,
                           int t_max, void *out, size_t ld_out, hipStream_t stream, int cap, int elem_bytes)
{
    if (n_series <= 0 || t_max <= 0) return;
    const int n_cols = std::min(n_series, cap);
    if (n_cols <= 0) return;
    dim3 grid((n_cols + NM_BLOCK - 1) / NM_BLOCK, (t_max + GATHER_TB - 1) / GATHER_TB);
    if (elem_bytes == 8)
        hipLaunchKernelGGL(gather_columns_kernel<double>, grid, dim3(NM_BLOCK), 0, stream, (const double *)y, ld, series_of, n_active, t_max, (double *)out, ld_out, cap);
    else if (elem_bytes == 4)
        hipLaunchKernelGGL(gather_columns_kernel<float>, grid, dim3(NM_BLOCK), 0, stream, (const float *)y, ld, series_of, n_active, t_max, (float *)out, ld_out, cap);
    else
        hipLaunchKernelGGL(gather_columns_kernel<unsigned short>, grid, dim3(NM_BLOCK), 0, stream, (const unsigned short *)y, ld, series_of, n_active, t_max, (unsigned short *)out, ld_out, cap);
}

constexpr int GROUP_COMPACT_BLOCKS = 256, GROUP_GATHER_COL_BLOCKS = 128, GROUP_GATHER_ROW_BLOCKS = 8;
__global__ __launch_bounds__(NM_BLOCK) void group_compact_kernel(const GroupCompactArgs g)
{
    const int k = blockIdx.y;
    if (g.n_clear[k] && blockIdx.x == 0 && threadIdx.x == 0) *g.n_clear[k] = 0;
    const int n_prev = g.n_prev[k] ? *g.n_prev[k] : g.n_series;
    const int32_t *prev = g.prev[k], *done = g.done[k];
    const int lane = threadIdx.x;
    for (int base0 = (int)blockIdx.x * NM_BLOCK; base0 < n_prev; base0 += (int)gridDim.x * NM_BLOCK) {
        const int idx = base0 + lane;
        int s = 0;
        bool keep = false;
        if (idx < n_prev) {
            s = prev ? prev[idx] : idx;
            keep = done[s] == 0;
        }
        const unsigned long long bal = __ballot(keep);
        const int cnt = __popcll(bal);
        if (cnt == 0) continue;
        int base = 0;
        if (lane == 0) base = atomicAdd(g.n_next[k], cnt);
        base = __shfl(base, 0);
        const int before = __popcll(bal & ((1ull << lane) - 1ull));
        if (keep) g.next[k][base + before] = s;
    }
}

void launch_group_compact(const GroupCompactArgs &g, hipStream_t stream)
{
    if (g.n_slots <= 0 || g.n_series <= 0) return;
    const int grid = std::min((g.n_series + NM_BLOCK - 1) / NM_BLOCK, GROUP_COMPACT_BLOCKS);
    hipLaunchKernelGGL(group_compact_kernel, dim3(grid, g.n_slots), dim3(NM_BLOCK), 0, stream, g);
}

struct GroupZeroArgs { int32_t *p[GROUP_MAX_SLOTS]; };
__global__ void group_zero3_kernel(const int n, const GroupZeroArgs z)
{
    const int i = threadIdx.x;
    if (i < 3 * n) z.p[i / 3][i % 3] = 0;
}

void launch_group_zero3(int n, int32_t *const *zero, hipStream_t stream)
{
    if (n <= 0) return;
    GroupZeroArgs z{};
    for (int k = 0; k < n && k < GROUP_MAX_SLOTS; k++) z.p[k] = zero[k];
    hipLaunchKernelGGL(group_zero3_kernel, dim3(1), dim3(64), 0, stream, std::min(n, GROUP_MAX_SLOTS), z);
}

template <class E>
__global__ __launch_bounds__(NM_BLOCK) void group_gather_kernel(const GroupGatherArgs g)
{
    const int k = blockIdx.z;
    const int n_act = *g.n_active[k];
    if (n_act > g.cap[k]) return;
    const E *y = (const E *)g.y;
    E *out = (E *)g.out[k];
    const size_t ld_out = g.ld_out[k];
    const int32_t *series_of = g.series_of[k];
    for (int p0 = (int)blockIdx.x * NM_BLOCK; p0 < n_act; p0 += (int)gridDim.x * NM_BLOCK) {
        const int p = p0 + (int)threadIdx.x;
        const int s = series_of[p < n_act ? p : n_act - 1];
        for (int t0 = (int)blockIdx.y * GATHER_TB; t0 < g.t_max; t0 += (int)gridDim.y * GATHER_TB) {
            const int t1 = t0 + GATHER_TB < g.t_max ? t0 + GATHER_TB : g.t_max;
            for (int t = t0; t < t1; t++) out[(size_t)t * ld_out + p] = y[(size_t)t * g.ld + s];
        }
    }
}

void launch_group_gather(const GroupGatherArgs &g, int n_cols_max, hipStream_t stream)
{
    if (g.n_slots <= 0 || g.t_max <= 0 || n_cols_max <= 0) return;
    dim3 grid(std::min((n_cols_max + NM_BLOCK - 1) / NM_BLOCK, GROUP_GATHER_COL_BLOCKS),
              std::min((g.t_max + GATHER_TB - 1) / GATHER_TB, GROUP_GATHER_ROW_BLOCKS), g.n_slots);
    if (g.elem_bytes == 8) hipLaunchKernelGGL(group_gather_kernel<double>, grid, dim3(NM_BLOCK), 0, stream, g);
    else if (g.elem_bytes == 4) hipLaunchKernelGGL(group_gather_kernel<float>, grid, dim3(NM_BLOCK), 0, stream, g);
    else hipLaunchKernelGGL(group_gather_kernel<unsigned short>, grid, dim3(NM_BLOCK), 0, stream, g);
}

__global__ __launch_bounds__(NM_BLOCK) void compact_block_kernel(const double *y, size_t ld, const int32_t *len, int n_series, int t_rows, float *out32,
                                                                 unsigned short *out16, unsigned int *misfit)
{
    const int s = blockIdx.x * NM_BLOCK + threadIdx.x;
    const int t0 = blockIdx.y * GATHER_TB;
    const int t1 = t0 + GATHER_TB < t_rows ? t0 + GATHER_TB : t_rows;
    const int L = s < n_series ? len[s] : 0;
    unsigned bad32 = 0, bad16 = 0;
    if ((size_t)s < ld) {
        for (int t = t0; t < t1; t++) {
            const double v = y[(size_t)t * ld + s];
            const float f = (float)v;
            const unsigned short u = (v >= 0.0 && v <= 65535.0) ? (unsigned short)v : (unsigned short)0;
            out32[(size_t)t * ld + s] = f;
            if (out16) out16[(size_t)t * ld + s] = u;
            if (t < L) {
                bad32 += (__double_as_longlong((double)f) == __double_as_longlong(v)) ? 0u : 1u;
                bad16 += (__double_as_longlong((double)u) == __double_as_longlong(v)) ? 0u : 1u;
            }
        }
    }
#pragma unroll
    for (int o = 32; o >= 1; o >>= 1) { bad32 += __shfl_xor(bad32, o); bad16 += __shfl_xor(bad16, o); }
    if (threadIdx.x == 0) {
        if (bad32) atomicAdd(misfit, bad32);
        if (bad16) atomicAdd(misfit + 1, bad16);
    }
}

void launch_compact_block(const double *y, size_t ld, const int32_t *len, int n_series, int t_rows, float *out32, unsigned short *out16,
                          unsigned int *misfit, hipStream_t stream)
{
    if (ld == 0 || t_rows <= 0) return;
    dim3 grid((unsigned)((ld + NM_BLOCK - 1) / NM_BLOCK), (unsigned)((t_rows + GATHER_TB - 1) / GATHER_TB));
    hipLaunchKernelGGL(compact_block_kernel, grid, dim3(NM_BLOCK), 0, stream, y, ld, len, n_series, t_rows, out32, out16, misfit);
}
// ... 119 lines not shown
```

### anofox-forecast_amd/csrc/kernels.hpp

```cpp
#pragma once
#include <hip/hip_runtime.h>
#include <stddef.h>
#include <stdint.h>
#include <atomic>

#include <stdexcept>
#include <string>

namespace anofox {

inline void anofox_check_attr(hipError_t e)
{
    if (e != hipSuccess) throw std::runtime_error(std::string("launch preparation failed: ") + hipGetErrorString(e));
}

enum : uint32_t { SF_POSITIVE = 1u, SF_CONSTANT = 2u, SF_HAS_NAN = 4u };

enum : int32_t { FIT_OK = 0, FIT_SHORT = 1, FIT_NONPOSITIVE = 2, FIT_NONFINITE = 3, FIT_PERIOD = 4, FIT_SKIPPED = 5 };

struct PrepArgs {
    const double *y; size_t ld; const int32_t *len; int n_series;
    int m;
    const int32_t *m_col;
    double *mean, *sd;
    uint32_t *flags;
    double *fig_add, *fig_mul;
    double *l0, *b0;
    double *scratch;
    int pre_fig;
    int t_rows;
    int skip_sd;
    int skip_types;
};

size_t season_scratch_doubles(int n_series, int t_rows, int m_max);
void launch_season_figures(const PrepArgs &a, hipStream_t stream);

struct NmStateBuf {
    double *sim;
    double *fs;
    int32_t *phase, *evals, *iters, *passes, *done;
};

struct FitArgs {
    const double *y; size_t ld; const int32_t *len; int n_series;
    int t_rows;
    const double *y_round; size_t ld_round;
    const int32_t *series_of;
    const int32_t *n_active;
    int budget, first_round;
    const int32_t *m_col;
    int spec_below;
    const uint32_t *mask;
    uint32_t want;
    int min_len;
    int budget_seq;
    int spec2_below;
    int gathered;
    int gather_cap;
    NmStateBuf st;
    double *ring_scratch;
    size_t ring_scratch_doubles;
    double *nm_scratch;
    size_t nm_scratch_doubles;
    int m, h;
    const double *l0, *b0;
    const double *fig; size_t fig_ld;
    const uint32_t *flags;
    int need_positive;
    int skip_constant;
    int n_param;
    double *aicc;
    double *yhat;
    int32_t *status;
    int32_t *evals, *iters, *passes;
    const int32_t *insp_sel;
    int32_t insp_code;
    double *insp_fitted;
    double *insp_states;
    double *insp_info;
    unsigned long long *lane_stats;
    const double *mean;
    double *sd_out;
    int wave_prio;
    unsigned long long *wave_trace;
    unsigned long long wave_trace_tag;
};

struct SelectArgs {
    int n_series, h, n_slots;
    size_t ld;
    const int32_t *len;
    const double *aicc;
    const double *yhat_slots;
    const int32_t *slot_spec;
    const int32_t *status_slots;
    const int32_t *passes_slots;
    const int32_t *evals_slots;
    double *yhat;
    int32_t *model_code;
    int32_t *status;
    uint32_t *fallback_mask;
// ... 335 lines not shown
constexpr int EXOG_MAX_REGRESSORS = 8;
constexpr int32_t MODEL_CODE_ARIMAX = 50;
struct ExogArgs {
    const double *y; size_t ld; const int32_t *len; int n_series;
    int k, h;
    size_t t_rows;
    const double *x;
    const double *f;
    double *yhat;
    int32_t *status;
    int32_t *model_code;
    double *b0, *beta;
    uint32_t *used;
};
void launch_exog_arimax(const ExogArgs &, hipStream_t);

struct IntervalArgs {
    int n_series, h;
    const double *yhat, *sd;
    const int32_t *status;
    double z;
    double *lower, *upper;
};

typedef void (*FitLaunchFn)(const FitArgs &, hipStream_t);
struct FitLaunchers { FitLaunchFn round_seq, round_spec, round_spec2, round_auto, final; size_t nm_scratch_per_wg; FitLaunchFn round_k4, round_auto_k4; };
constexpr int ETS_PERLANE_LDS = -3, ETS_PERLANE_HBM = -4;
FitLaunchers ets_fit_launcher(int spec_id, int m, int yt = 0);
constexpr int GROUP_MAX_SLOTS = 16;
enum { GROUP_DAMPED_MUL = 0, GROUP_GENERAL = 1, GROUP_ADDITIVE = 2, N_GROUP_CLASSES = 3 };
struct GroupRoundArgs {
    int n_slots;
    int spec[GROUP_MAX_SLOTS];
    int k4[GROUP_MAX_SLOTS];
    int start[GROUP_MAX_SLOTS + 1];
};
typedef void (*GroupLaunchFn)(const FitArgs *tab, const GroupRoundArgs &g, int m, hipStream_t);
GroupLaunchFn ets_group_launcher(int group_class, int m, int yt);
inline int ets_group_class(int spec_id)
{
    if (spec_id < 0 || spec_id >= 30 || (spec_id >= 15 && spec_id % 3 == 1)) return -1;
    const int e = spec_id / 15, ti = (spec_id % 15) / 3, s = spec_id % 3;
    if (ti == 4) return GROUP_DAMPED_MUL;
    return (e == 0 && ti < 3 && s < 2) ? GROUP_ADDITIVE : GROUP_GENERAL;
}
FitLaunchers classic_fit_launcher(int kind, int m);
struct ClassicArgs;
void launch_classic_final(int kind, const FitArgs &a, const ClassicArgs &c, hipStream_t stream);

struct GroupCompactArgs {
    int n_slots, n_series;
    const int32_t *prev[GROUP_MAX_SLOTS], *n_prev[GROUP_MAX_SLOTS], *done[GROUP_MAX_SLOTS];
    int32_t *next[GROUP_MAX_SLOTS], *n_next[GROUP_MAX_SLOTS], *n_clear[GROUP_MAX_SLOTS];
};
void launch_group_compact(const GroupCompactArgs &g, hipStream_t);
void launch_group_zero3(int n, int32_t *const *zero, hipStream_t);
struct GroupGatherArgs {
    int n_slots, t_max, elem_bytes;
    const void *y; size_t ld;
    const int32_t *series_of[GROUP_MAX_SLOTS], *n_active[GROUP_MAX_SLOTS];
    void *out[GROUP_MAX_SLOTS]; size_t ld_out[GROUP_MAX_SLOTS]; int cap[GROUP_MAX_SLOTS];
};
void launch_group_gather(const GroupGatherArgs &g, int n_cols_max, hipStream_t);
void launch_compact(const int32_t *series_prev, const int32_t *n_prev, int n_series, const int32_t *done,
                    int32_t *series_next, int32_t *n_next, hipStream_t, int32_t *n_clear = nullptr);
constexpr int DETECT_LDS_ROWS = 8192;
constexpr int DETECT_LONG_GRID = 1024;
size_t detect_scratch_doubles(int n_series, int t_rows);
void launch_detect_periods(const double *y, size_t ld, const int32_t *len, int n_series, int t_rows, double *scratch, int32_t *period,
                           double *best_acf, hipStream_t stream);
void launch_gather_columns(const void *y, size_t ld, const int32_t *series_of, const int32_t *n_active, int n_series,
                           int t_max, void *out, size_t ld_out, hipStream_t stream, int cap, int elem_bytes = 8);
void launch_compact_block(const double *y, size_t ld, const int32_t *len, int n_series, int t_rows, float *out32, unsigned short *out16,
                          unsigned int *misfit, hipStream_t stream);

struct ArimaArgs {
    const double *y; size_t ld; const int32_t *len; int n_series;
    int m, h;
    int t_max;
    void *ws; size_t ws_bytes;
    int32_t *wlen, *d, *D;
    double *wmean, *wsd, *last_d0, *last_d1;
    int32_t *order;
    double *xbest;
    double *aicc;
    int32_t *status, *evals, *passes, *models;
    double *yhat;
    int32_t *model_code;
    int trace;
    double lookahead, spec_factor;
    int lookahead_depth;
    const std::atomic<int> *concurrent;
    double shared_chunk_rounds;
    int prep_lanes;
    int queue_sort;
    int refit_budget;
    double *long_scratch;
    int ml_refit;
    const int32_t *m_col;
};
size_t arima_workspace_bytes(int n_series, int t_max);
size_t arima_long_scratch_doubles(int n_series, int m, int max_fit_waves);
int arima_max_fit_waves();
int launch_arima(const ArimaArgs &, hipStream_t);

unsigned long long recip_selftest(unsigned long long n, unsigned long long seed, double *first_bad, hipStream_t stream);

void launch_prep(const PrepArgs &, hipStream_t);
void launch_select(const SelectArgs &, hipStream_t);
void launch_classic(int kind, const ClassicArgs &, hipStream_t);
void launch_simple(const SimpleArgs &, hipStream_t);
void launch_intervals(const IntervalArgs &, hipStream_t);

// ... 2 lines not shown
```

### anofox-forecast_amd/csrc/nm.hpp

```cpp
#pragma once
#include <hip/hip_runtime.h>

namespace anofox {

constexpr int NM_K = 4;
constexpr int NM_BLOCK = 64;

__device__ __forceinline__ double nm_clip(double v, double lo, double hi)
{
    if (v < lo) v = lo;
    if (v > hi) v = hi;
    return v;
}

enum { NM_INIT0 = 0, NM_INIT1 = 1, NM_ITER = 2, NM_SHRINK = 3, NM_SEQ_INIT = 4, NM_SEQ_E = 5, NM_SEQ_OC = 6, NM_SEQ_IC = 7, NM_SEQ_SHRINK = 8 };

struct NmRun { int phase; int evals; int iters; int passes; bool done; };
struct NmStats { int iters; int evals; int passes; };

template <int D> constexpr int nm_lds_doubles() { return ((D + 1) * D + (D + 1)) * NM_BLOCK; }

template <int D> struct NmSimplex { double x[D + 1][D]; double f[D + 1]; };

template <int D> __device__ __forceinline__ void nm_load(const double *st, int lane, NmSimplex<D> &S)
{
#pragma unroll
    for (int k = 0; k <= D; k++) {
#pragma unroll
        for (int i = 0; i < D; i++) S.x[k][i] = st[(k * D + i) * NM_BLOCK + lane];
        S.f[k] = st[((D + 1) * D + k) * NM_BLOCK + lane];
    }
}
template <int D> __device__ __forceinline__ void nm_store(double *st, int lane, const NmSimplex<D> &S)
{
#pragma unroll
    for (int k = 0; k <= D; k++) {
#pragma unroll
        for (int i = 0; i < D; i++) st[(k * D + i) * NM_BLOCK + lane] = S.x[k][i];
        st[((D + 1) * D + k) * NM_BLOCK + lane] = S.f[k];
    }
}
__device__ __forceinline__ void nm_fence() { __asm__ volatile("" ::: "memory"); }

template <int D> __device__ __forceinline__ double nm_store_x(const double *st, int lane, int k, int i) { return st[(k * D + i) * NM_BLOCK + lane]; }
template <int D> __device__ __forceinline__ void nm_store_set_f(double *st, int lane, int k, double f) { st[((D + 1) * D + k) * NM_BLOCK + lane] = f; }

template <int D> __device__ __forceinline__ bool nm_converged(const NmSimplex<D> &S)
{
    bool small = true;
#pragma unroll
    for (int k = 1; k <= D; k++) {
#pragma unroll
        for (int i = 0; i < D; i++)
            if (!(fabs(S.x[k][i] - S.x[0][i]) <= 1.0e-4)) small = false;
        if (!(fabs(S.f[0] - S.f[k]) <= 1.0e-8)) small = false;
    }
    return small;
}

template <int D> __device__ __forceinline__ double nm_trial(const NmSimplex<D> &S, int which, int i, double lo, double hi)
{
    double s = S.x[0][i];
#pragma unroll
    for (int k = 1; k < D; k++) s = s + S.x[k][i];
    const double xb = s / (double)D;
    const double xw = S.x[D][i];
    const double a = which == 0 ? 2.0 : (which == 1 ? 3.0 : (which == 2 ? 1.5 : 0.5));
    const double b = which == 0 ? 1.0 : (which == 1 ? 2.0 : 0.5);
    const double v = which == 3 ? a * xb + b * xw : a * xb - b * xw;
    return nm_clip(v, lo, hi);
}
// ... 26 lines not shown
#pragma unroll
    for (int k = 1; k <= D; k++)
#pragma unroll
        for (int i = 0; i < D; i++)
            S.x[k][i] = nm_clip(S.x[0][i] + 0.5 * (S.x[k][i] - S.x[0][i]), lo[i], hi[i]);
}

template <int D> __device__ __forceinline__ void nm_sort_all(NmSimplex<D> &S)
{
#pragma unroll
    for (int k = 1; k <= D; k++) {
#pragma unroll
        for (int j = k; j >= 1; j--) {
            const bool sw = S.f[j] < S.f[j - 1];
            const double t = S.f[j];
            S.f[j] = sw ? S.f[j - 1] : t;
            S.f[j - 1] = sw ? t : S.f[j - 1];
#pragma unroll
            for (int i = 0; i < D; i++) {
                const double u = S.x[j][i];
                S.x[j][i] = sw ? S.x[j - 1][i] : u;
                S.x[j - 1][i] = sw ? u : S.x[j - 1][i];
            }
        }
    }
}

template <class Model>
__device__ void nm_init_simplex(Model &mdl, double *st, NmRun &r, bool active)
{
    constexpr int D = Model::DIM;
    const int lane = threadIdx.x & (NM_BLOCK - 1);
    double lo[D], hi[D], x0[D];
    mdl.bounds(lo, hi, x0);
    NmSimplex<D> S;
#pragma unroll
    for (int i = 0; i < D; i++) S.x[0][i] = nm_clip(x0[i], lo[i], hi[i]);
#pragma unroll
    for (int k = 0; k < D; k++) {
#pragma unroll
        for (int i = 0; i < D; i++) S.x[k + 1][i] = S.x[0][i];
        double v = S.x[0][k];
        v = (v != 0.0) ? (1.0 + 0.05) * v : 0.00025;
        S.x[k + 1][k] = nm_clip(v, lo[k], hi[k]);
    }
#pragma unroll
    for (int k = 0; k <= D; k++) S.f[k] = 0.0;
    nm_store<D>(st, lane, S);
    r.phase = NM_INIT0;
    r.evals = 0;
    r.iters = 1;
    r.passes = 0;
    r.done = !active;
}

template <class Model>
__device__ void nm_advance_spec(Model &mdl, double *st, NmRun &r, int budget)
{
    constexpr int D = Model::DIM;
    const int lane = threadIdx.x & (NM_BLOCK - 1);
    double lo[D], hi[D], x0[D];
    mdl.bounds(lo, hi, x0);
    const int maxiter = 200 * D, maxfun = 200 * D;
    int phase = r.phase, evals = r.evals, iters = r.iters, passes = r.passes;
    bool done = r.done, parked = false;
    double cand[NM_K][D], fc[NM_K];

    for (int pass = 0;; pass++) {
        if (!done && !parked) {
            NmSimplex<D> S;
            nm_load<D>(st, lane, S);
            if (phase == NM_INIT0) {
#pragma unroll
                for (int k = 0; k < NM_K; k++)
#pragma unroll
                    for (int i = 0; i < D; i++) cand[k][i] = S.x[k <= D ? k : D][i];
            } else if (phase == NM_INIT1) {
#pragma unroll
                for (int i = 0; i < D; i++) cand[0][i] = S.x[D][i];
            } else if (phase == NM_ITER) {
                if (!(evals < maxfun && iters < maxiter)) done = true;
                else if (nm_converged<D>(S)) done = true;
                if (!done) {
#pragma unroll
                    for (int k = 0; k < NM_K; k++)
#pragma unroll
                        for (int i = 0; i < D; i++) cand[k][i] = nm_trial<D>(S, k, i, lo[i], hi[i]);
                }
            } else {
#pragma unroll
                for (int k = 0; k < NM_K; k++)
#pragma unroll
                    for (int i = 0; i < D; i++) cand[k][i] = S.x[k + 1 <= D ? k + 1 : D][i];
            }
        }
        if (!done && pass >= budget && (phase == NM_ITER || phase == NM_INIT0)) parked = true;
        if (__all(done || parked)) break;

        mdl.eval(cand, fc);
        passes += (done || parked) ? 0 : 1;
        nm_fence();

        if (!done && !parked) {
            NmSimplex<D> S;
            nm_load<D>(st, lane, S);
            if (phase == NM_INIT0) {
#pragma unroll
                for (int k = 0; k < NM_K; k++)
                    if (k <= D) S.f[k] = fc[k];
                evals += (D + 1 < NM_K ? D + 1 : NM_K);
                phase = (D + 1 > NM_K) ? NM_INIT1 : NM_ITER;
                if (phase == NM_ITER) nm_sort_all<D>(S);
            } else if (phase == NM_INIT1) {
                S.f[D] = fc[0];
                evals += 1;
                phase = NM_ITER;
                nm_sort_all<D>(S);
            } else if (phase == NM_ITER) {
                const double fxr = fc[0];
                evals += 1;
                bool shrink = false;
                int which = 0;
                double fnew = fxr;
                if (fxr < S.f[0]) {
                    evals += 1;
                    if (fc[1] < fxr) { which = 1; fnew = fc[1]; }
                } else if (fxr < S.f[D - 1]) {
                    which = 0;
                } else if (fxr < S.f[D]) {
                    evals += 1;
                    if (fc[2] <= fxr) { which = 2; fnew = fc[2]; } else shrink = true;
                } else {
                    evals += 1;
                    if (fc[3] < S.f[D]) { which = 3; fnew = fc[3]; } else shrink = true;
                }
                if (!shrink) {
                    nm_accept<D>(S, which, fnew, lo, hi);
                    iters += 1;
                } else {
                    nm_shrink_vertices<D>(S, lo, hi);
                    phase = NM_SHRINK;
                }
            } else {
#pragma unroll
                for (int k = 0; k < NM_K; k++)
                    if (k + 1 <= D) S.f[k + 1] = fc[k];
                evals += D;
                iters += 1;
                phase = NM_ITER;
                nm_sort_all<D>(S);
            }
            nm_store<D>(st, lane, S);
        }
    }
    r.phase = phase; r.evals = evals; r.iters = iters; r.passes = passes; r.done = done;
}

template <int D> __device__ __forceinline__ void nm_hypothesis(int hh, int &P, int &j)
{
    if (hh == 0) { P = 1; j = 0; }
    else if (hh <= D) { P = 0; j = hh - 1; }
    else if (hh <= 2 * D + 1) { P = 2; j = hh - D - 1; }
    else { P = 3; j = hh - 2 * D - 2; }
}

template <int D> __device__ __forceinline__ double nm_trial2(const NmSimplex<D> &S, int P, int j, int which, int i, double lo, double hi)
{
    const double xp = nm_trial<D>(S, P, i, lo, hi);
    double s = 0.0;
#pragma unroll
    for (int pos = 0; pos < D; pos++) {
        double v;
        if (j == D) v = S.x[pos][i];
        else {
            const double before = S.x[pos][i];
            const double after = pos >= 1 ? S.x[pos - 1][i] : before;
            v = pos < j ? before : (pos == j ? xp : after);
        }
        s = pos == 0 ? v : s + v;
    }
    const double xb = s / (double)D;
    const double xw = j == D ? xp : S.x[D - 1][i];
    const double a = which == 0 ? 2.0 : (which == 1 ? 3.0 : (which == 2 ? 1.5 : 0.5));
    const double b = which == 0 ? 1.0 : (which == 1 ? 2.0 : 0.5);
    const double t = which == 3 ? a * xb + b * xw : a * xb - b * xw;
    return nm_clip(t, lo, hi);
}

template <int D> __device__ __forceinline__ bool nm_decide(const NmSimplex<D> &S, const double (&fc)[NM_K], int &evals, int &which, double &fnew)
{
    const double fxr = fc[0];
    evals += 1;
    which = 0;
    fnew = fxr;
    if (fxr < S.f[0]) {
        evals += 1;
        if (fc[1] < fxr) { which = 1; fnew = fc[1]; }
        return true;
    }
    if (fxr < S.f[D - 1]) return true;
    if (fxr < S.f[D]) {
        evals += 1;
        if (fc[2] <= fxr) { which = 2; fnew = fc[2]; return true; }
        return false;
    }
    evals += 1;
    if (fc[3] < S.f[D]) { which = 3; fnew = fc[3]; return true; }
    return false;
}

template <class Model>
__device__ void nm_advance_spec2(Model &mdl, double *st, NmRun &r, int budget)
{
    constexpr int D = Model::DIM;
    constexpr int NH = 3 * D + 3;
    const int lane = threadIdx.x & (NM_BLOCK - 1);
    double lo[D], hi[D], x0[D];
    mdl.bounds(lo, hi, x0);
    const int maxiter = 200 * D, maxfun = 200 * D;
    int phase = r.phase, evals = r.evals, iters = r.iters, passes = r.passes;
    bool done = r.done, parked = false;
    const int hh = lane >= NM_K ? (lane - NM_K) >> 2 : 0, w2 = (lane - NM_K) & 3;
    int hp = 0, hj = 0;
    nm_hypothesis<D>(hh < NH ? hh : 0, hp, hj);
    double x[D];

    for (int pass = 0;; pass++) {
        if (!done && !parked) {
            NmSimplex<D> S;
            nm_load<D>(st, lane, S);
            const int sub = lane < NM_K ? lane : NM_K - 1;
            if (phase == NM_INIT0) {
#pragma unroll
                for (int i = 0; i < D; i++) x[i] = nm_store_x<D>(st, lane, sub <= D ? sub : D, i);
            } else if (phase == NM_INIT1) {
#pragma unroll
                for (int i = 0; i < D; i++) x[i] = S.x[D][i];
            } else if (phase == NM_ITER) {
                if (!(evals < maxfun && iters < maxiter)) done = true;
                else if (nm_converged<D>(S)) done = true;
                if (!done) {
                    if (lane < NM_K) {
#pragma unroll
                        for (int i = 0; i < D; i++) x[i] = nm_trial<D>(S, lane, i, lo[i], hi[i]);
                    } else {
#pragma unroll
                        for (int i = 0; i < D; i++) x[i] = nm_trial2<D>(S, hp, hj, w2, i, lo[i], hi[i]);
                    }
                }
            } else {
#pragma unroll
                for (int i = 0; i < D; i++) x[i] = nm_store_x<D>(st, lane, sub + 1 <= D ? sub + 1 : D, i);
            }
        }
        if (!done && pass >= budget && (phase == NM_ITER || phase == NM_INIT0)) parked = true;
        if (done || parked) break;

        const double f = mdl.eval1(x);
        passes += 1;
        nm_fence();
        double fc[NM_K];
#pragma unroll
        for (int k = 0; k < NM_K; k++) fc[k] = __shfl(f, k);

        NmSimplex<D> S;
        nm_load<D>(st, lane, S);
        if (phase == NM_INIT0) {
#pragma unroll
            for (int k = 0; k < NM_K; k++)
                if (k <= D) S.f[k] = fc[k];
            evals += (D + 1 < NM_K ? D + 1 : NM_K);
            phase = (D + 1 > NM_K) ? NM_INIT1 : NM_ITER;
            if (phase == NM_ITER) nm_sort_all<D>(S);
        } else if (phase == NM_INIT1) {
            S.f[D] = fc[0];
            evals += 1;
            phase = NM_ITER;
            nm_sort_all<D>(S);
        } else if (phase == NM_ITER) {
            int which = 0;
            double fnew = 0.0;
            if (!nm_decide<D>(S, fc, evals, which, fnew)) {
                nm_shrink_vertices<D>(S, lo, hi);
                phase = NM_SHRINK;
            } else {
                int j = D;
#pragma unroll
                for (int k = D; k >= 1; k--)
                    if (j == k && fnew < S.f[k - 1]) j = k - 1;
                const int hstar = which == 1 ? 0 : (which == 0 ? 1 + j : (which == 2 ? D + 1 + j : 2 * D + 2 + j));
                double fc2[NM_K];
#pragma unroll
                for (int k = 0; k < NM_K; k++) fc2[k] = __shfl(f, NM_K + 4 * hstar + k);
                nm_accept<D>(S, which, fnew, lo, hi);
                iters += 1;
                if (!(evals < maxfun && iters < maxiter) || nm_converged<D>(S)) done = true;
                else if (NM_K + 4 * NH <= NM_BLOCK) {
                    if (!nm_decide<D>(S, fc2, evals, which, fnew)) {
                        nm_shrink_vertices<D>(S, lo, hi);
                        phase = NM_SHRINK;
                    } else {
                        nm_accept<D>(S, which, fnew, lo, hi);
                        iters += 1;
                    }
                }
            }
        } else {
#pragma unroll
            for (int k = 0; k < NM_K; k++)
                if (k + 1 <= D) S.f[k + 1] = fc[k];
            evals += D;
            iters += 1;
            phase = NM_ITER;
            nm_sort_all<D>(S);
        }
        nm_store<D>(st, lane, S);
    }
    r.phase = phase; r.evals = evals; r.iters = iters; r.passes = passes; r.done = done;
}

template <class Model>
__device__ void nm_advance_seq(Model &mdl, double *st, NmRun &r, int budget)
{
    constexpr int D = Model::DIM;
    const int lane = threadIdx.x & (NM_BLOCK - 1);
    double lo[D], hi[D], x0[D];
    mdl.bounds(lo, hi, x0);
    const int maxiter = 200 * D, maxfun = 200 * D;
    int phase = r.phase, evals = r.evals, iters = r.iters, passes = r.passes;
    bool done = r.done, parked = false;
    int vi = 0;
    double fxr = 0.0;
    double x[D];

    for (int pass = 0;; pass++) {
        if (!done && !parked) {
            if (phase == NM_INIT0) { phase = NM_SEQ_INIT; vi = 0; }
            if (phase == NM_SEQ_INIT || phase == NM_SEQ_SHRINK) {
                const int k = phase == NM_SEQ_INIT ? vi : 1 + vi;
#pragma unroll
                for (int i = 0; i < D; i++) x[i] = nm_store_x<D>(st, lane, k, i);
            } else {
                NmSimplex<D> S;
                nm_load<D>(st, lane, S);
                if (phase == NM_ITER) {
                    if (!(evals < maxfun && iters < maxiter)) done = true;
                    else if (nm_converged<D>(S)) done = true;
                }
                const int which = phase == NM_ITER ? 0 : (phase == NM_SEQ_E ? 1 : (phase == NM_SEQ_OC ? 2 : 3));
                if (!done) {
#pragma unroll
                    for (int i = 0; i < D; i++) x[i] = nm_trial<D>(S, which, i, lo[i], hi[i]);
                }
            }
        }
        if (!done && pass >= budget && (phase == NM_ITER || phase == NM_INIT0)) parked = true;
        if (__all(done || parked)) break;

        const double f = mdl.eval1(x);
        passes += (done || parked) ? 0 : 1;
        nm_fence();

        if (!done && !parked) {
            if (phase == NM_SEQ_INIT || phase == NM_SEQ_SHRINK) {
                const bool init = phase == NM_SEQ_INIT;
                nm_store_set_f<D>(st, lane, init ? vi : 1 + vi, f);
                vi += 1;
                evals += 1;
                if (vi == (init ? D + 1 : D)) {
                    if (!init) iters += 1;
                    nm_fence();
                    NmSimplex<D> S;
                    nm_load<D>(st, lane, S);
                    nm_sort_all<D>(S);
                    nm_store<D>(st, lane, S);
                    phase = NM_ITER;
                }
            } else {
                NmSimplex<D> S;
                nm_load<D>(st, lane, S);
                bool changed = true;
                if (phase == NM_ITER) {
                    fxr = f;
                    evals += 1;
                    if (fxr < S.f[0]) { phase = NM_SEQ_E; changed = false; }
                    else if (fxr < S.f[D - 1]) { nm_accept<D>(S, 0, fxr, lo, hi); iters += 1; }
                    else if (fxr < S.f[D]) { phase = NM_SEQ_OC; changed = false; }
                    else { phase = NM_SEQ_IC; changed = false; }
                } else if (phase == NM_SEQ_E) {
                    evals += 1;
                    if (f < fxr) nm_accept<D>(S, 1, f, lo, hi);
                    else nm_accept<D>(S, 0, fxr, lo, hi);
                    iters += 1;
                    phase = NM_ITER;
                } else {
                    evals += 1;
                    const bool ok = (phase == NM_SEQ_OC) ? (f <= fxr) : (f < S.f[D]);
                    if (ok) {
                        nm_accept<D>(S, phase == NM_SEQ_OC ? 2 : 3, f, lo, hi);
                        iters += 1;
                        phase = NM_ITER;
                    } else {
                        nm_shrink_vertices<D>(S, lo, hi);
                        vi = 0;
                        phase = NM_SEQ_SHRINK;
                    }
                }
                if (changed) nm_store<D>(st, lane, S);
            }
        }
    }
    r.phase = phase; r.evals = evals; r.iters = iters; r.passes = passes; r.done = done;
}

template <class Model>
__device__ void nm_minimize(Model &mdl, bool active, double *st, double (&xbest)[Model::DIM], double &fbest, NmStats &stats)
{
    constexpr int D = Model::DIM;
    const int lane = threadIdx.x & (NM_BLOCK - 1);
    NmRun r;
    nm_init_simplex(mdl, st, r, active);
    nm_advance_spec(mdl, st, r, 0x7fffffff);
#pragma unroll
    for (int i = 0; i < D; i++) xbest[i] = st[(0 * D + i) * NM_BLOCK + lane];
    fbest = st[((D + 1) * D + 0) * NM_BLOCK + lane];
    stats.iters = r.iters;
    stats.evals = r.evals;
    stats.passes = r.passes;
}

}
```

### anofox-forecast_amd/device.py

```python
from __future__ import annotations

import ctypes as C

import numpy as np
import torch

from . import lib as _lib


def pack_time_major(series_major: np.ndarray, ld: int | None = None) -> np.ndarray:
    n, T = series_major.shape
    ld = ld or (n + 63) // 64 * 64
    out = np.zeros((T, ld), dtype=np.float64)
    out[:, :n] = series_major.T
    return out


def prepare_block(y: torch.Tensor, lengths: torch.Tensor, valid: torch.Tensor | None = None, dates: torch.Tensor | None = None, *,
                  n_series: int | None = None, gaps: bool = False, frequency_micros: int = 0, frequency_type: str = "FIXED",
                  trim: str = "none", fill: str = "none", fill_value: float = 0.0, t_out: int | None = None,
                  count_only: bool = False, out: dict | None = None, stream: torch.cuda.Stream | None = None) -> dict:
    L = _lib.load()
    assert y.dtype == torch.float64 and y.is_cuda and y.is_contiguous() and y.dim() == 2
    t_rows, ld = int(y.shape[0]), int(y.shape[1])
# ... 430 lines not shown
        err = _lib.AnofoxError()
        if not self.L.anofox_hip_batch_exog_coefficients(self.handle, b0.ctypes.data, beta.ctypes.data, used.ctypes.data, C.byref(err)):
            raise RuntimeError(f"exog_coefficients failed: [{err.code}] {err.message.decode()}")
        return {"intercept": b0, "beta": beta, "used": ((used[:, None] >> np.arange(k, dtype=np.uint32)[None, :]) & 1).astype(bool)}

    def periods(self) -> np.ndarray:
        out = np.zeros(self.n, dtype=np.int32)
        if not self.L.anofox_hip_batch_periods(self.handle, out.ctypes.data):
            raise RuntimeError("anofox_hip_batch_periods: no block set")
        return out

    def run(self, stream: torch.cuda.Stream | None = None):
        cur = stream if stream is not None else torch.cuda.current_stream(self.device)
        st = cur
        if cur.cuda_stream == 0:
            if self._side is None:
                self._side = torch.cuda.Stream(device=self.device)
            self._side.wait_stream(cur)
            st = self._side
        err = _lib.AnofoxError()
        ok = self.L.anofox_hip_batch_run(self.handle, C.c_void_p(st.cuda_stream), C.byref(err))
        if st is not cur:
            cur.wait_stream(st)
        if not ok:
            raise RuntimeError(f"anofox_hip_batch_run failed: [{err.code}] {err.message.decode()}")

    def stats(self) -> dict:
        s = _lib.AnofoxHipStats()
        if not self.L.anofox_hip_batch_stats(self.handle, C.byref(s)):
            raise RuntimeError("anofox_hip_batch_stats failed")
        return {f: getattr(s, f) for f, _ in s._fields_}

    SPEC_CLASSES = ("additive", "general", "damped_mul_trend")

    def lane_stats(self) -> dict:
        s = _lib.AnofoxHipLaneStats()
        if not self.L.anofox_hip_batch_lane_stats(self.handle, C.byref(s), C.sizeof(s)):
            raise RuntimeError("anofox_hip_batch_lane_stats failed")
        eff = lambda live, waves: round(live / (64.0 * waves), 4) if waves else None
        E, T, S = "AM", ("N", "A", "Ad", "M", "Md"), "NAM"
        out = {"by_class": {}, "by_spec": {}}
        tw = tl = 0
        for c, name in enumerate(self.SPEC_CLASSES):
            w, l = int(s.wave_passes[c]), int(s.live_lane_passes[c])
            tw += w; tl += l
            out["by_class"][name] = {"wave_passes": w, "live_lane_passes": l, "lane_efficiency": eff(l, w)}
        out["wave_passes"], out["live_lane_passes"], out["lane_efficiency"] = tw, tl, eff(tl, tw)
        for k in range(int(s.n_slots)):
            sid = int(s.slot_spec_id[k])
            name = E[sid // 15] + T[(sid % 15) // 3] + S[sid % 3]
            out["by_spec"][name] = {"wave_passes": int(s.slot_wave_passes[k]), "lane_efficiency": eff(int(s.slot_live_lane_passes[k]), int(s.slot_wave_passes[k]))}
        return out

    def results(self) -> dict:
        ptrs = [C.c_void_p() for _ in range(5)]
        self.L.anofox_hip_batch_device_results(self.handle, *[C.byref(p) for p in ptrs])

        def view(ptr, shape, dtype, itemsize):
            n = int(np.prod(shape))
            if n == 0:
                return torch.empty(shape, dtype=dtype, device=self.device)
            iface = {"shape": tuple(shape), "typestr": {8: "<f8", 4: "<i4"}[itemsize], "data": (ptr.value, False), "version": 2}
            holder = type("H", (), {"__cuda_array_interface__": iface})()
            return torch.as_tensor(holder, device=self.device)

        return {
            "yhat": view(ptrs[0], (self.n, self.h), torch.float64, 8),
            "lower": view(ptrs[1], (self.n, self.h), torch.float64, 8),
            "upper": view(ptrs[2], (self.n, self.h), torch.float64, 8),
            "model_code": view(ptrs[3], (self.n,), torch.int32, 4),
            "status": view(ptrs[4], (self.n,), torch.int32, 4),
        }

    def model_name(self, code: int, series: int | None = None) -> str:
        buf = (C.c_char * 64)()
        if series is None:
            self.L.anofox_hip_model_name(C.byref(self.opts), int(code), buf)
        else:
            self.L.anofox_hip_batch_model_name(self.handle, int(series), int(code), buf)
        return buf.value.decode()

    def close(self):
        if getattr(self, "handle", None):
            self.L.anofox_hip_batch_destroy(self.handle)
            self.handle = None

    def __del__(self):
        try:
            self.close()
        except Exception:
            pass
```

### anofox-forecast_amd/lib.py

```python
from __future__ import annotations

import ctypes as C
import os

os.environ.setdefault("GPU_MAX_HW_QUEUES", "16")

_HERE = os.path.dirname(os.path.abspath(__file__))
LIB_PATH = os.environ.get("ANOFOX_HIP_LIB", os.path.join(_HERE, "libanofox_fcst_hip.so"))

SUCCESS, NULL_POINTER, INVALID_INPUT, COMPUTATION_ERROR, ALLOCATION_ERROR, INVALID_MODEL = 0, 1, 2, 3, 4, 5
INSUFFICIENT_DATA, INVALID_DATE_FORMAT, INVALID_FREQUENCY, PANIC_CAUGHT, INTERNAL_ERROR = 6, 7, 8, 9, 10


class AnofoxError(C.Structure):
    _fields_ = [("code", C.c_int), ("message", C.c_char * 256)]


class ForecastOptions(C.Structure):
    _fields_ = [
        ("model", C.c_char * 32),
        ("ets_model", C.c_char * 8),
        ("horizon", C.c_int),
        ("confidence_level", C.c_double),
        ("seasonal_period", C.c_int),
# ... 284 lines not shown
        ("laplace_variant", C.c_char * 16),
        ("laplace_seasonal_batch_init", C.c_bool),
    ]


class AnofoxHipFold(C.Structure):
    _fields_ = [(n, C.c_int64) for n in ("fold_id", "train_start", "train_end", "test_start", "test_end")]


assert C.sizeof(AnofoxHipFold) == 40
BACKTEST_WINDOWS = {"expanding": 0, "fixed": 1, "sliding": 2}


class AnofoxHipHierarchyOptions(C.Structure):
    _fields_ = [("route", C.c_int32), ("tile_min_members", C.c_int32), ("reserved", C.c_int32 * 2)]


assert C.sizeof(AnofoxHipHierarchyOptions) == 16
HIERARCHY_ROUTES = {"auto": 0, "lane": 1, "tile": 2}


assert C.sizeof(ExogenousRegressor) == 32 and C.sizeof(ExogenousData) == 16 and C.sizeof(ForecastOptionsExog) == 192
MODEL_CODE_ARIMAX = 50


class AnofoxHipInspection(C.Structure):
    _fields_ = [("model_code", C.c_int32), ("status", C.c_int32), ("seasonal_period", C.c_int32), ("reserved", C.c_int32),
                ("alpha", C.c_double), ("beta", C.c_double), ("gamma", C.c_double), ("phi", C.c_double),
                ("aic", C.c_double), ("aicc", C.c_double), ("bic", C.c_double), ("sse", C.c_double),
                ("level", C.c_double), ("trend", C.c_double)]


class AnofoxHipArimaFit(C.Structure):
    _fields_ = [(k, C.c_int32) for k in ("status", "model_code", "seasonal_period", "p", "d", "q", "P", "D", "Q", "has_constant",
                                         "n_diff", "models_tried", "evals", "reserved")] + \
               [("phi", C.c_double * 5), ("theta", C.c_double * 5), ("Phi", C.c_double * 2), ("Theta", C.c_double * 2),
                ("constant", C.c_double), ("aicc", C.c_double)]


assert C.sizeof(AnofoxHipArimaFit) == 184


EXPORTED_SYMBOLS = [
    "anofox_ts_forecast", "anofox_free_forecast_result", "anofox_fcst_version", "anofox_ts_forecast_batch",
    "anofox_hip_device_count", "anofox_hip_set_device", "anofox_hip_batch_create", "anofox_hip_batch_destroy",
    "anofox_hip_batch_ld", "anofox_hip_batch_pack_host", "anofox_hip_batch_set_device_block", "anofox_hip_batch_run",
    "anofox_hip_batch_stats", "anofox_hip_batch_device_results", "anofox_hip_batch_fetch", "anofox_hip_model_name", "anofox_hip_batch_model_name",
    "anofox_hip_ingest_create", "anofox_hip_ingest_destroy", "anofox_hip_ingest_append", "anofox_hip_ingest_finish",
    "anofox_hip_ingest_group_keys", "anofox_hip_ingest_last_dates", "anofox_hip_ingest_lengths", "anofox_hip_ingest_values",
    "anofox_hip_ingest_validity", "anofox_hip_batch_pack_ingest", "anofox_hip_batch_inspect", "anofox_hip_batch_arima_fit",
    "anofox_hip_batch_n_series", "anofox_hip_batch_periods", "anofox_hip_batch_set_fixed_params",
    "anofox_hip_set_devices", "anofox_hip_get_devices", "anofox_hip_set_min_series_per_device", "anofox_hip_shard_range",
    "anofox_hip_set_default_arima_method", "anofox_hip_batch_set_arima_method", "anofox_hip_release_caches",
    "anofox_hip_batch_run_many", "anofox_hip_batch_lane_stats", "anofox_hip_selftest_recip",
    "anofox_ts_mstl_decomposition", "anofox_free_mstl_result", "anofox_hip_mstl_decompose_batch", "anofox_hip_mstl_decompose_device",
    "anofox_ts_forecast_exog", "anofox_ts_forecast_exog_batch", "anofox_hip_batch_set_exog_device", "anofox_hip_batch_exog_coefficients",
    "anofox_ts_detect_changepoints_bocpd", "anofox_free_bocpd_result", "anofox_hip_changepoints_batch", "anofox_hip_changepoints_device",
    "anofox_ts_detect_changepoints", "anofox_free_changepoint_result", "anofox_hip_pelt_batch", "anofox_hip_pelt_device",
    "anofox_ts_stats", "anofox_ts_stats_with_dates", "anofox_ts_stats_with_dates_and_type", "anofox_free_ts_stats_result",
    "anofox_hip_stats_batch", "anofox_hip_stats_device",
    "anofox_ts_data_quality", "anofox_hip_quality_batch", "anofox_hip_quality_device",
    "anofox_ts_features", "anofox_free_features_result", "anofox_ts_features_list", "anofox_ts_validate_feature_params",
    "anofox_free_warnings", "anofox_hip_features_batch", "anofox_hip_features_device", "anofox_hip_features_families_device",
    "anofox_ts_detect_seasonality", "anofox_ts_analyze_seasonality", "anofox_free_seasonality_result", "anofox_free_int_array",
    "anofox_hip_seasonality_batch", "anofox_hip_seasonality_device",
    "anofox_ts_lomb_scargle", "anofox_ts_aic_period", "anofox_ts_sazed_period", "anofox_ts_detect_periods_flat",
    "anofox_free_flat_multi_period_result", "anofox_hip_periods_batch", "anofox_hip_periods_device",
    "anofox_ts_mae", "anofox_ts_mse", "anofox_ts_rmse", "anofox_ts_mape", "anofox_ts_smape", "anofox_ts_r2", "anofox_ts_bias",
    "anofox_ts_rmae", "anofox_ts_mase", "anofox_ts_quantile_loss", "anofox_ts_mqloss", "anofox_ts_coverage",
    "anofox_hip_metrics_batch", "anofox_hip_metrics_device",
    "anofox_ts_fill_nulls_const", "anofox_ts_fill_nulls_mean", "anofox_ts_fill_nulls_interpolate", "anofox_ts_fill_nulls_forward",
    "anofox_ts_fill_nulls_backward", "anofox_ts_fill_gaps", "anofox_free_gap_fill_result", "anofox_free_filled_values_result",
    "anofox_free_double_array", "anofox_hip_prepare_device", "anofox_hip_prepare_batch", "anofox_hip_free_prepared",
    "anofox_hip_conformal_learn_device", "anofox_hip_conformal_apply_device", "anofox_hip_conformal_evaluate_device",
    "anofox_hip_conformal_batch", "anofox_hip_free_conformal",
    "anofox_ts_conformal_quantile", "anofox_ts_conformal_intervals", "anofox_ts_conformal_predict", "anofox_ts_conformal_predict_multi",
    "anofox_ts_conformal_predict_adaptive", "anofox_ts_conformal_predict_asymmetric", "anofox_ts_mean_interval_width",
    "anofox_ts_conformal_learn", "anofox_ts_conformal_apply", "anofox_ts_conformal_coverage", "anofox_ts_conformal_evaluate",
    "anofox_free_conformal_result", "anofox_free_conformal_multi_result", "anofox_free_calibration_profile", "anofox_free_prediction_intervals",
    "anofox_hip_backtest_folds", "anofox_hip_backtest_sizes", "anofox_hip_backtest_expand_device", "anofox_hip_backtest_collect_device",
    "anofox_hip_backtest_batch",
    "anofox_hip_hierarchy_plan", "anofox_hip_hierarchy_device", "anofox_hip_hierarchy_batch",
]

ARIMA_CSS, ARIMA_CSS_ML = 0, 1

_lib = None


def load():
    global _lib
    if _lib is not None:
        return _lib
    if not os.path.exists(LIB_PATH):
        raise RuntimeError(f"{LIB_PATH} is missing: build it with `make -C anofox-forecast_amd/csrc` "
                           "(or __graft_entry__.build()); the backend has no CPU fallback")
    try:
        import torch
    except ImportError:
        pass
    L = C.CDLL(LIB_PATH)
    P = C.POINTER
    L.anofox_ts_forecast.restype = C.c_bool
    L.anofox_ts_forecast.argtypes = [C.c_void_p, C.c_void_p, C.c_size_t, P(ForecastOptions), P(ForecastResult), P(AnofoxError)]
    L.anofox_free_forecast_result.argtypes = [P(ForecastResult)]
    L.anofox_fcst_version.restype = C.c_char_p
    L.anofox_ts_forecast_batch.restype = C.c_bool
    L.anofox_ts_forecast_batch.argtypes = [C.c_void_p, C.c_void_p, C.c_void_p, C.c_size_t, P(ForecastOptions), C.c_void_p,
                                          C.c_void_p, C.c_void_p, P(AnofoxError)]
    L.anofox_hip_device_count.restype = C.c_int
    L.anofox_hip_set_device.restype = C.c_int
    L.anofox_hip_set_device.argtypes = [C.c_int]
    L.anofox_hip_batch_create.restype = C.c_bool
    L.anofox_hip_batch_create.argtypes = [C.c_size_t, C.c_size_t, P(ForecastOptions), P(C.c_void_p), P(AnofoxError)]
    L.anofox_hip_batch_destroy.argtypes = [C.c_void_p]
    L.anofox_hip_batch_ld.restype = C.c_size_t
    L.anofox_hip_batch_ld.argtypes = [C.c_void_p]
    L.anofox_hip_batch_n_series.restype = C.c_size_t
    L.anofox_hip_batch_n_series.argtypes = [C.c_void_p]
    L.anofox_hip_batch_periods.restype = C.c_bool
    L.anofox_hip_batch_periods.argtypes = [C.c_void_p, C.c_void_p]
    L.anofox_hip_batch_set_fixed_params.restype = C.c_bool
    L.anofox_hip_batch_set_fixed_params.argtypes = [C.c_void_p, C.c_double, C.c_double, C.c_double, C.c_double, P(AnofoxError)]
    L.anofox_hip_batch_pack_host.restype = C.c_bool
    L.anofox_hip_batch_pack_host.argtypes = [C.c_void_p, C.c_void_p, C.c_void_p, C.c_void_p, P(AnofoxError)]
    L.anofox_hip_batch_set_device_block.restype = C.c_bool
    L.anofox_hip_batch_set_device_block.argtypes = [C.c_void_p, C.c_void_p, C.c_size_t, C.c_void_p, P(AnofoxError)]
    L.anofox_hip_batch_run.restype = C.c_bool
    L.anofox_hip_batch_run.argtypes = [C.c_void_p, C.c_void_p, P(AnofoxError)]
    L.anofox_hip_batch_stats.restype = C.c_bool
    L.anofox_hip_batch_stats.argtypes = [C.c_void_p, P(AnofoxHipStats)]
    L.anofox_hip_selftest_recip.restype = C.c_bool
    L.anofox_hip_selftest_recip.argtypes = [C.c_uint64, C.c_uint64, P(C.c_uint64), P(C.c_double)]
    L.anofox_hip_batch_lane_stats.restype = C.c_bool
    L.anofox_hip_batch_lane_stats.argtypes = [C.c_void_p, P(AnofoxHipLaneStats), C.c_size_t]
    L.anofox_hip_batch_device_results.restype = C.c_bool
    L.anofox_hip_batch_device_results.argtypes = [C.c_void_p] + [P(C.c_void_p)] * 5
    L.anofox_hip_batch_fetch.restype = C.c_bool
    L.anofox_hip_batch_fetch.argtypes = [C.c_void_p, C.c_void_p, C.c_void_p]
    L.anofox_hip_model_name.argtypes = [P(ForecastOptions), C.c_int32, C.c_char * 64]
    L.anofox_hip_batch_model_name.argtypes = [C.c_void_p, C.c_size_t, C.c_int32, C.c_char * 64]
    L.anofox_hip_batch_model_name.restype = None
    L.anofox_hip_batch_inspect.restype = C.c_bool
    L.anofox_hip_batch_inspect.argtypes = [C.c_void_p, C.c_void_p, C.c_void_p, C.c_void_p, C.c_size_t, P(AnofoxError)]
    L.anofox_hip_batch_arima_fit.restype = C.c_bool
    L.anofox_hip_batch_arima_fit.argtypes = [C.c_void_p, C.c_void_p, P(AnofoxError)]
    L.anofox_hip_set_devices.restype = C.c_bool
    L.anofox_hip_set_devices.argtypes = [C.c_void_p, C.c_size_t]
    L.anofox_hip_get_devices.restype = C.c_size_t
    L.anofox_hip_get_devices.argtypes = [C.c_void_p, C.c_size_t]
    L.anofox_hip_set_min_series_per_device.argtypes = [C.c_size_t]
    L.anofox_hip_shard_range.argtypes = [C.c_size_t, C.c_size_t, C.c_size_t, P(C.c_size_t), P(C.c_size_t)]
    L.anofox_hip_set_default_arima_method.restype = C.c_bool
    L.anofox_hip_set_default_arima_method.argtypes = [C.c_int]
    L.anofox_hip_batch_set_arima_method.restype = C.c_bool
    L.anofox_hip_batch_set_arima_method.argtypes = [C.c_void_p, C.c_int, P(AnofoxError)]
    L.anofox_hip_release_caches.argtypes = []
    L.anofox_hip_batch_run_many.restype = C.c_bool
    L.anofox_hip_batch_run_many.argtypes = [C.c_void_p, C.c_size_t, C.c_void_p]
    L.anofox_ts_mstl_decomposition.restype = C.c_bool
    L.anofox_ts_mstl_decomposition.argtypes = [C.c_void_p, C.c_size_t, C.c_void_p, C.c_size_t, C.c_int, P(MstlResult), P(AnofoxError)]
    L.anofox_free_mstl_result.argtypes = [P(MstlResult)]
    L.anofox_hip_mstl_decompose_batch.restype = C.c_bool
    L.anofox_hip_mstl_decompose_batch.argtypes = [C.c_void_p, C.c_void_p, C.c_void_p, C.c_size_t, C.c_void_p, C.c_size_t, C.c_int,
                                                  C.c_void_p, C.c_void_p, C.c_void_p, C.c_void_p, C.c_void_p, C.c_void_p, P(AnofoxError)]
    L.anofox_hip_mstl_decompose_device.restype = C.c_bool
    L.anofox_hip_mstl_decompose_device.argtypes = [C.c_void_p, C.c_size_t, C.c_void_p, C.c_size_t, C.c_size_t, C.c_void_p, C.c_size_t,
                                                   C.c_int, C.c_void_p, C.c_void_p, C.c_void_p, C.c_void_p, C.c_void_p, P(AnofoxError)]
    L.anofox_ts_forecast_exog.restype = C.c_bool
    L.anofox_ts_forecast_exog.argtypes = [C.c_void_p, C.c_void_p, C.c_size_t, P(ForecastOptionsExog), P(ForecastResult), P(AnofoxError)]
    L.anofox_ts_forecast_exog_batch.restype = C.c_bool
    L.anofox_ts_forecast_exog_batch.argtypes = [C.c_void_p, C.c_void_p, C.c_void_p, C.c_size_t, P(ForecastOptions), C.c_size_t, C.c_void_p,
                                                C.c_void_p, C.c_void_p, C.c_void_p, P(AnofoxError), C.c_void_p, C.c_void_p]
    L.anofox_hip_batch_set_exog_device.restype = C.c_bool
    L.anofox_hip_batch_set_exog_device.argtypes = [C.c_void_p, C.c_void_p, C.c_void_p, C.c_size_t, P(AnofoxError)]
    L.anofox_hip_batch_exog_coefficients.restype = C.c_bool
    L.anofox_hip_batch_exog_coefficients.argtypes = [C.c_void_p, C.c_void_p, C.c_void_p, C.c_void_p, P(AnofoxError)]
    L.anofox_ts_detect_changepoints_bocpd.restype = C.c_bool
    L.anofox_ts_detect_changepoints_bocpd.argtypes = [C.c_void_p, C.c_size_t, C.c_double, C.c_bool, P(BocpdResult), P(AnofoxError)]
    L.anofox_free_bocpd_result.argtypes = [P(BocpdResult)]
    L.anofox_hip_changepoints_batch.restype = C.c_bool
    L.anofox_hip_changepoints_batch.argtypes = [C.c_void_p, C.c_void_p, C.c_void_p, C.c_size_t, C.c_double, C.c_void_p, C.c_void_p,
                                                C.c_void_p, C.c_void_p, P(AnofoxError)]
    L.anofox_hip_changepoints_device.restype = C.c_bool
    L.anofox_hip_changepoints_device.argtypes = [C.c_void_p, C.c_size_t, C.c_void_p, C.c_size_t, C.c_size_t, C.c_double, C.c_void_p,
                                                 C.c_void_p, C.c_void_p, C.c_void_p, P(AnofoxError)]
# ... 345 lines not shown
```

### include/anofox_fcst_hip.h

```cpp
#ifndef ANOFOX_FCST_HIP_H
#define ANOFOX_FCST_HIP_H

#include <stdbool.h>
#include <stddef.h>
#include <stdint.h>

#ifdef __cplusplus
extern "C" {
#endif


#ifndef ANOFOX_FCST_FFI_H

typedef enum ErrorCode {
    SUCCESS = 0,
    NULL_POINTER = 1,
    INVALID_INPUT = 2,
    COMPUTATION_ERROR = 3,
    ALLOCATION_ERROR = 4,
    INVALID_MODEL = 5,
    INSUFFICIENT_DATA = 6,
    INVALID_DATE_FORMAT = 7,
    INVALID_FREQUENCY = 8,
    PANIC_CAUGHT = 9,
// ... 992 lines not shown
} AnofoxHipStats;

typedef struct AnofoxHipLaneStats {
    uint64_t struct_size;
    uint64_t wave_passes[3];
    uint64_t live_lane_passes[3];
    uint32_t n_slots;
    uint32_t reserved;
    int32_t  slot_spec_id[30];
    uint64_t slot_wave_passes[30];
    uint64_t slot_live_lane_passes[30];
} AnofoxHipLaneStats;

int anofox_hip_device_count(void);
int anofox_hip_set_device(int device);

bool anofox_hip_batch_create(size_t n_series, size_t t_max,
                             const struct ForecastOptions *options,
                             AnofoxHipBatch **out_batch,
                             struct AnofoxError *out_error);
void anofox_hip_batch_destroy(AnofoxHipBatch *batch);

size_t anofox_hip_batch_ld(const AnofoxHipBatch *batch);
size_t anofox_hip_batch_n_series(const AnofoxHipBatch *batch);

bool anofox_hip_batch_set_fixed_params(AnofoxHipBatch *batch, double alpha, double beta, double gamma, double phi,
                                       struct AnofoxError *out_error);

bool anofox_hip_batch_set_arima_method(AnofoxHipBatch *batch, int method, struct AnofoxError *out_error);

bool anofox_hip_batch_pack_host(AnofoxHipBatch *batch,
                                const double *const *values,
                                const uint64_t *const *validity,
                                const size_t *lengths,
                                struct AnofoxError *out_error);

bool anofox_hip_batch_set_device_block(AnofoxHipBatch *batch,
                                       const void *d_y, size_t ld,
                                       const void *d_len,
                                       struct AnofoxError *out_error);

bool anofox_hip_batch_set_exog_device(AnofoxHipBatch *batch, const void *d_x, const void *d_future, size_t k,
                                      struct AnofoxError *out_error);

bool anofox_hip_batch_exog_coefficients(AnofoxHipBatch *batch, double *out_intercept, double *out_beta, uint32_t *out_used,
                                        struct AnofoxError *out_error);

bool anofox_hip_batch_periods(const AnofoxHipBatch *batch, int32_t *out_periods);

bool anofox_hip_selftest_recip(uint64_t n_operands, uint64_t seed, uint64_t *out_mismatches, double *out_first_bad);

bool anofox_hip_batch_lane_stats(AnofoxHipBatch *batch, AnofoxHipLaneStats *out, size_t struct_size);

bool anofox_hip_batch_run(AnofoxHipBatch *batch, void *stream,
                          struct AnofoxError *out_error);

bool anofox_hip_batch_run_many(AnofoxHipBatch *const *batches, size_t n_batches, struct AnofoxError *out_errors);

bool anofox_hip_batch_stats(AnofoxHipBatch *batch, AnofoxHipStats *out_stats);

bool anofox_hip_batch_device_results(AnofoxHipBatch *batch,
                                     void **d_yhat, void **d_lower, void **d_upper,
                                     void **d_model_code, void **d_status);

bool anofox_hip_batch_fetch(AnofoxHipBatch *batch,
                            struct ForecastResult *out_results,
                            struct AnofoxError *out_errors);

typedef struct AnofoxHipInspection {
    int32_t model_code;
    int32_t status;
    int32_t seasonal_period;
    int32_t reserved;
    double alpha, beta, gamma, phi;
    double aic, aicc, bic, sse;
    double level, trend;
} AnofoxHipInspection;
bool anofox_hip_batch_inspect(AnofoxHipBatch *batch, AnofoxHipInspection *out,
                              double *fitted, double *seasonal, size_t seasonal_stride,
                              struct AnofoxError *out_error);

typedef struct AnofoxHipArimaFit {
    int32_t status;
    int32_t model_code;
    int32_t seasonal_period;
    int32_t p, d, q, P, D, Q;
    int32_t has_constant;
    int32_t n_diff;
    int32_t models_tried;
    int32_t evals;
    int32_t reserved;
    double phi[5], theta[5], Phi[2], Theta[2];
    double constant;
    double aicc;
} AnofoxHipArimaFit;
bool anofox_hip_batch_arima_fit(AnofoxHipBatch *batch, AnofoxHipArimaFit *out, struct AnofoxError *out_error);

void anofox_hip_model_name(const struct ForecastOptions *options, int32_t model_code,
                           char out_name[64]);
void anofox_hip_batch_model_name(const AnofoxHipBatch *batch, size_t series, int32_t model_code, char out_name[64]);

typedef struct AnofoxHipIngest AnofoxHipIngest;
AnofoxHipIngest *anofox_hip_ingest_create(void);
void anofox_hip_ingest_destroy(AnofoxHipIngest *ingest);
bool anofox_hip_ingest_append(AnofoxHipIngest *ingest,
                              const int64_t *group_key, const int64_t *date,
// ... 160 lines not shown
```

Measured before the change: 80770.

## Route damped multiplicative-trend ETS evals through guarded near-1 pow with redo fallback

Replaces the disabled per-block retry with a routing scheme. Waves whose series are not marked far-prone run a guarded fast path that uses the near-1 power approximation everywhere, then flag a trip so the candidate is re-evaluated on the branchy path. Series that see far values are recorded per series and compacted to the back of the active map, so later rounds group far-prone series together. This is meant to cut the divergent pow_step cost in damped multiplicative-trend fits, at the price of occasional redo passes, extra compaction state and stats counters.

```diff
diff --git a/anofox-forecast_amd/csrc/ets_device.hpp b/anofox-forecast_amd/csrc/ets_device.hpp
--- a/anofox-forecast_amd/csrc/ets_device.hpp
+++ b/anofox-forecast_amd/csrc/ets_device.hpp
@@ -45,9 +45,6 @@
 template <> struct YtCode<double> { static constexpr int value = YT_F64; };
 template <> struct YtCode<float> { static constexpr int value = YT_F32; };
 template <> struct YtCode<unsigned short> { static constexpr int value = YT_U16; };
-#ifndef ANOFOX_DM_RETRY
-#define ANOFOX_DM_RETRY 0
-#endif
 #ifndef ANOFOX_TWO_BLOCK
 #define ANOFOX_TWO_BLOCK 1
 #endif
@@ -124,7 +121,7 @@
                 phib = dm_pow_near1(r, p.pc);
                 if constexpr (NEAR) st.rfar = __builtin_fmax(st.rfar, fabs(r));
                 else if (!(fabs(r) <= DM_POW_NEAR1_R)) {
-                    if (!(st.b >= 0x1p-1000 && st.b <= 0x1p+1000)) st.bad = 1;
+                    st.bad |= (st.b >= 0x1p-1000 && st.b <= 0x1p+1000) ? 2 : 3;
                     phib = dm_pow_step(st.b, p.phi, p.pl);
                 }
             } else {
@@ -195,7 +192,7 @@
 template <class Cfg>
 __device__ __forceinline__ double ets_objective_value(const EtsState &st, int n)
 {
-    if (st.bad || !(fabs(st.sse) <= 1.7976931348623157e308)) return __builtin_huge_val();
+    if ((st.bad & 1) || !(fabs(st.sse) <= 1.7976931348623157e308)) return __builtin_huge_val();
     if constexpr (!Cfg::ADDITIVE) {
         constexpr double D_LO = Cfg::E == C_MUL ? 0x1p-120 : 0x1p-1000, D_HI = Cfg::E == C_MUL ? 0x1p+120 : 0x1p+1000;
         if (n > 0 && !(st.dlo >= D_LO && st.dhi <= D_HI)) return __builtin_huge_val();
@@ -221,12 +218,13 @@
     double mean; double *var_out;
 };
 
-template <class Cfg, int MS, int K, bool FINAL, class YT = double>
+template <class Cfg, int MS, int K, bool FINAL, class YT = double, bool ROUTE = false>
 __device__ __forceinline__ void ets_pass(const SeriesView &v, const EtsInit &in,
                                          const double (&cand)[K][Cfg::DIM], double (&fout)[K],
-                                         double *ring, const EtsFinalOut *fin)
+                                         double *ring, const EtsFinalOut *fin, NmRoute *rt = nullptr)
 {
     static_assert((Cfg::S == C_NONE) == (MS == 0), "MS == 0 iff no seasonal component");
+    static_assert(!ROUTE || (Cfg::T == C_MUL && Cfg::D && K == 1 && !FINAL && MS >= 0), "the far route: damped multiplicative trend, one candidate, ring in registers");
     const int lane = threadIdx.x & (NM_BLOCK - 1);
     EtsPar par[K];
     EtsState st[K];
@@ -311,23 +309,6 @@
         }
         auto run_block = [&](const ybuf_t (&buf)[S], const int base, auto pred_tag) __attribute__((always_inline)) {
             constexpr bool PRED = decltype(pred_tag)::value;
-            if constexpr (ANOFOX_DM_RETRY && Cfg::T == C_MUL && Cfg::D && K == 1 && !PRED && !FINAL) {
-                const EtsState st0 = st[0];
-                double s0[MR];
-#pragma unroll
-                for (int jj = 0; jj < MR; jj++) s0[jj] = s[0][jj];
-                st[0].rfar = 0.0;
-#pragma unroll
-                for (int j = 0; j < S; j++) {
-                    ets_step<Cfg, true>(par[0], st[0], widen(buf[j]), s[0][MS > 0 ? j % MR : 0]);
-                    if ((j & 3) == 3 || j == S - 1) ets_renorm<Cfg>(st[0]);
-                }
-                const bool again = v.len > 0 && (!(st[0].rfar <= DM_POW_NEAR1_R) || st[0].b != st[0].b);
-                if (__builtin_amdgcn_ballot_w64(again) == 0ull) return;
-                st[0] = st0;
-#pragma unroll
-                for (int jj = 0; jj < MR; jj++) s[0][jj] = s0[jj];
-            }
 #pragma unroll
             for (int j = 0; j < S; j++) {
                 if (!PRED || base + j < v.len) {
@@ -342,6 +323,22 @@
         };
         int base = 0;
         constexpr bool TWO = ANOFOX_TWO_BLOCK == 2 || (ANOFOX_TWO_BLOCK == 1 && Cfg::ADDITIVE);
+        bool tripped = false;
+        if constexpr (ROUTE) {
+            if (rt->guarded) {
+                for (; base + S <= wave_min_len; base += S) {
+                    load_block(nxt, base + S);
+#pragma unroll
+                    for (int j = 0; j < S; j++) {
+                        ets_step<Cfg, true>(par[0], st[0], widen(cur[j]), s[0][MS > 0 ? j % MR : 0]);
+                        if ((j & 3) == 3 || j == S - 1) ets_renorm<Cfg>(st[0]);
+                    }
+#pragma unroll
+                    for (int j = 0; j < S; j++) cur[j] = nxt[j];
+                }
+                tripped = !(st[0].rfar <= DM_POW_NEAR1_R) || st[0].b != st[0].b;
+            }
+        }
         if constexpr (TWO) {
             for (; base + 2 * S <= wave_min_len; base += 2 * S) {
                 load_block(nxt, base + S);
@@ -357,6 +354,7 @@
 #pragma unroll
             for (int j = 0; j < S; j++) cur[j] = nxt[j];
         }
+        if constexpr (ROUTE) { rt->tripped = tripped; rt->far = (st[0].bad & 2) != 0; }
         if constexpr (FINAL) {
             if constexpr (MS > 0) {
                 if (fin->states && v.len > 0) {
@@ -485,6 +483,7 @@
 template <class Cfg, int MS, int CPL, class YT = double>
 struct EtsModel {
     static constexpr int DIM = Cfg::DIM;
+    static constexpr bool FAR_ROUTE = Cfg::T == C_MUL && Cfg::D && MS >= 0 && CPL == 1;
     SeriesView v;
     EtsInit in;
     double *ring;
@@ -504,7 +503,18 @@
         ets_pass<Cfg, MS, 1, false, YT>(v, in, c1, f1, ring, nullptr);
         return f1[0];
     }
-    __device__ void eval(const double (&cand)[NM_K][DIM], double (&f)[NM_K]) const
+    __device__ double eval1_routed(const double (&x)[DIM], NmRoute &rt) const
+    {
+        double c1[1][DIM], f1[1];
+#pragma unroll
+        for (int i = 0; i < DIM; i++) c1[0][i] = x[i];
+        ets_pass<Cfg, MS, 1, false, YT, FAR_ROUTE>(v, in, c1, f1, ring, nullptr, &rt);
+        return f1[0];
+    }
+    __device__ void eval_routed(const double (&cand)[NM_K][DIM], double (&f)[NM_K], NmRoute &rt) const { eval_impl<FAR_ROUTE>(cand, f, &rt); }
+    __device__ void eval(const double (&cand)[NM_K][DIM], double (&f)[NM_K]) const { eval_impl<false>(cand, f, nullptr); }
+    template <bool ROUTE>
+    __device__ __forceinline__ void eval_impl(const double (&cand)[NM_K][DIM], double (&f)[NM_K], NmRoute *rt) const
     {
         if constexpr (CPL == NM_K) {
             ets_pass<Cfg, MS, NM_K, false, YT>(v, in, cand, f, ring, nullptr);
@@ -514,7 +524,7 @@
 #pragma unroll
             for (int i = 0; i < DIM; i++)
                 mine[0][i] = sub == 0 ? cand[0][i] : (sub == 1 ? cand[1][i] : (sub == 2 ? cand[2][i] : cand[3][i]));
-            ets_pass<Cfg, MS, 1, false, YT>(v, in, mine, f1, ring, nullptr);
+            ets_pass<Cfg, MS, 1, false, YT, ROUTE>(v, in, mine, f1, ring, nullptr, rt);
             const int base = (threadIdx.x & (NM_BLOCK - 1)) & ~3;
 #pragma unroll
             for (int k = 0; k < NM_K; k++) f[k] = __shfl(f1[0], base + k);
diff --git a/anofox-forecast_amd/csrc/ets_fit_kernel.hpp b/anofox-forecast_amd/csrc/ets_fit_kernel.hpp
--- a/anofox-forecast_amd/csrc/ets_fit_kernel.hpp
+++ b/anofox-forecast_amd/csrc/ets_fit_kernel.hpp
@@ -65,7 +65,7 @@
     if (vblock * PPB >= n_act) return;
     const int p = vblock * PPB + lane / LPP;
     const bool valid = p < n_act;
-    const int s = valid ? (a.series_of ? a.series_of[p] : p) : 0;
+    const int s = valid ? (a.series_of ? a.series_of[far_map_pos(p, n_act, a.n_back ? *a.n_back : 0, a.map_cap)] : p) : 0;
     const int len = valid ? a.len[s] : 0;
 
     const int m = a.m_col ? (MS <= -3 ? a.m_col[s] : __builtin_amdgcn_readfirstlane(a.m_col[s])) : a.m;
@@ -128,6 +128,13 @@
         r.iters = active ? a.st.iters[s] : 0;
         r.passes = active ? a.st.passes[s] : 0;
         r.done = !active;
+        r.far_prone = true; r.far_seen = false;
+        r.live = 0; r.wp_guarded = 0; r.wp_branchy = 0; r.redo = 0;
+    }
+    constexpr bool FAR_ROUTE = nm_far_route<typename RoundModelOf<Cfg, MS, YT>::type>::value;
+    if constexpr (FAR_ROUTE) {
+        r.route_on = a.far_route != 0;
+        r.far_prone = a.first_round || a.st.far == nullptr || (active && a.st.far[s] != 0);
     }
     const int passes_in = r.passes;
 
@@ -161,7 +168,7 @@
         }
     }
     if (a.lane_stats) {
-        const int mine = r.passes - passes_in;
+        const int mine = FAR_ROUTE ? r.live : r.passes - passes_in;
         int sum = mine;
 #pragma unroll
         for (int o = 32; o >= 1; o >>= 1) sum += __shfl_xor(sum, o);
@@ -169,6 +176,24 @@
         if (lane == 0 && most > 0) {
             atomicAdd(a.lane_stats, (unsigned long long)most);
             atomicAdd(a.lane_stats + 1, (unsigned long long)sum);
+        }
+    }
+    if constexpr (RoundTraits<Cfg>::DAMPED_MUL) {
+        const bool flag = FAR_ROUTE && r.far_seen;
+        if (a.st.far && active && (lane % LPP) == 0) a.st.far[s] = flag ? 1 : 0;
+        if constexpr (FAR_ROUTE) {
+            if (a.far_stats) {
+                int redo = r.redo;
+#pragma unroll
+                for (int o = 32; o >= 1; o >>= 1) redo += __shfl_xor(redo, o);
+                const int flagged = __popcll(__ballot(active && (lane % LPP) == 0 && r.done && flag));
+                if (lane == 0) {
+                    if (r.wp_guarded) atomicAdd(a.far_stats, (unsigned long long)r.wp_guarded);
+                    if (r.wp_branchy) atomicAdd(a.far_stats + 1, (unsigned long long)r.wp_branchy);
+                    if (redo) atomicAdd(a.far_stats + 2, (unsigned long long)redo);
+                    if (flagged) atomicAdd(a.far_stats + 3, (unsigned long long)flagged);
+                }
+            }
         }
     }
     if (active && (lane % LPP) == 0) {
diff --git a/anofox-forecast_amd/csrc/host_api.hip b/anofox-forecast_amd/csrc/host_api.hip
--- a/anofox-forecast_amd/csrc/host_api.hip
+++ b/anofox-forecast_amd/csrc/host_api.hip
@@ -88,6 +88,7 @@
     unsigned int h_misfit[2] = {1u, 1u};
     int y_type = 0;
     unsigned long long *d_wave_trace = nullptr;
+    unsigned long long *d_far_stats = nullptr;
     unsigned long long *d_lane_stats = nullptr;
     double *d_yhat = nullptr, *d_lo = nullptr, *d_hi = nullptr;
     int32_t *d_model_code = nullptr, *d_status = nullptr, *d_detail = nullptr, *d_passes_total = nullptr, *d_evals_total = nullptr;
@@ -118,6 +119,7 @@
         size_t ybuf_cols = 0;
         int32_t *map[2] = {nullptr, nullptr};
         int32_t *cnt = nullptr;
+        int32_t *far_cnt = nullptr;
         anofox::NmStateBuf st{};
         double *nm_scratch = nullptr;
         size_t nm_scratch_doubles = 0;
@@ -294,7 +296,7 @@
     if (b->owns_len) F(b->d_len);
     F(b->d_mean); F(b->d_sd); F(b->d_fig_add); F(b->d_fig_mul); F(b->d_l0); F(b->d_b0); F(b->d_flags);
     F(b->d_aicc); F(b->d_yhat_slots); F(b->d_status_slots); F(b->d_evals_slots); F(b->d_iters_slots);
-    F(b->d_passes_slots); F(b->d_slot_spec); F(b->d_lane_stats); F(b->d_wave_trace); F(b->d_yc32); F(b->d_yc16); F(b->d_misfit);
+    F(b->d_passes_slots); F(b->d_slot_spec); F(b->d_lane_stats); F(b->d_far_stats); F(b->d_wave_trace); F(b->d_yc32); F(b->d_yc16); F(b->d_misfit);
     F(b->d_yhat); F(b->d_lo); F(b->d_hi); F(b->d_model_code); F(b->d_status); F(b->d_detail);
     F(b->classic_st.sim); F(b->classic_st.fs); F(b->classic_st.phase); F(b->classic_st.evals); F(b->classic_st.iters); F(b->classic_st.passes); F(b->classic_st.done);
     F(b->d_classic_ybuf); F(b->d_classic_status); F(b->classic_map[0]); F(b->classic_map[1]); F(b->classic_cnt);
@@ -313,8 +315,8 @@
     F(b->ar_order); F(b->ar_status); F(b->ar_evals); F(b->ar_passes); F(b->ar_models);
     batch_detach_streams(b);
     for (auto &l : b->lanes) {
-        F(l.ybuf); l.ybuf_cols = 0; F(l.map[0]); F(l.map[1]); F(l.cnt);
-        F(l.st.sim); F(l.st.fs); F(l.st.phase); F(l.st.evals); F(l.st.iters); F(l.st.passes); F(l.st.done);
+        F(l.ybuf); l.ybuf_cols = 0; F(l.map[0]); F(l.map[1]); F(l.cnt); F(l.far_cnt);
+        F(l.st.far); F(l.st.sim); F(l.st.fs); F(l.st.phase); F(l.st.evals); F(l.st.iters); F(l.st.passes); F(l.st.done);
         F(l.nm_scratch); l.nm_scratch_doubles = 0;
     }
 }
@@ -381,6 +383,8 @@
         b->d_slot_spec = dalloc<int32_t>(S);
         b->d_lane_stats = dalloc<unsigned long long>(2 * S);
         HIPCHECK(hipMemset(b->d_lane_stats, 0, 2 * S * sizeof(unsigned long long)));
+        b->d_far_stats = dalloc<unsigned long long>(4);
+        HIPCHECK(hipMemset(b->d_far_stats, 0, 4 * sizeof(unsigned long long)));
         const int n_lanes = std::min<int>(N_AUX_STREAMS, b->n_slots_cap);
         for (int q = 0; q < n_lanes; q++) {
             auto &l = b->lanes[q];
@@ -394,6 +398,10 @@
             l.st.iters = dalloc<int32_t>(ld);
             l.st.passes = dalloc<int32_t>(ld);
             l.st.done = dalloc<int32_t>(ld);
+            l.far_cnt = dalloc<int32_t>(6);
+            l.st.far = dalloc<uint8_t>(ld);
+            HIPCHECK(hipMemset(l.far_cnt, 0, 6 * sizeof(int32_t)));
+            HIPCHECK(hipMemset(l.st.far, 0, ld));
         }
     }
     batch_attach_streams(b);
@@ -861,6 +869,9 @@
         a.m_col = b->d_m_col;
         if (b->sd_in_final && order.size() == 1) { a.mean = b->d_mean; a.sd_out = b->d_sd; }
         a.lane_stats = b->d_lane_stats ? b->d_lane_stats + 2 * k : nullptr;
+        a.far_route = b->tun.far_route > 0 ? 1 : 0;
+        a.far_stats = b->d_far_stats;
+        a.map_cap = (int)n;
         a.wave_trace = b->d_wave_trace;
         fns[oi] = ets_fit_launcher(id, (merged && se != 0) ? (a.m > lds_limit ? ETS_PERLANE_HBM : ETS_PERLANE_LDS) : a.m, yt);
         if (!fns[oi].round_seq || !fns[oi].round_spec || !fns[oi].round_auto || !fns[oi].final) throw HipFail{"no kernel for ETS spec id " + std::to_string(id)};
@@ -1061,6 +1072,8 @@
             a.wave_prio = (int)oi < b->tun.prio_top ? std::max(1, 3 - (int)oi) : 0;
             a.spec_below = -1; a.spec2_below = -1;
             a.gathered = 0;
+            a.n_back = nullptr;
+            const bool far_part = grouped && b->tun.far_route > 0 && lane.far_cnt && lane.st.far && spec_trend_idx(specs[order[oi]]) == 4;
             if (tiny) {
                 a.y_round = b->d_y; a.ld_round = ld; a.series_of = nullptr; a.n_active = nullptr;
                 a.budget = 1 << 30; a.budget_seq = a.budget;
@@ -1086,8 +1099,10 @@
                     const int k = gc.n_slots++;
                     gc.prev[k] = prev_map; gc.n_prev[k] = prev_cnt; gc.done[k] = lane.st.done;
                     gc.next[k] = lane.map[r & 1]; gc.n_next[k] = lane.cnt + (r % 3); gc.n_clear[k] = lane.cnt + ((r + 1) % 3);
+                    gc.far[k] = far_part ? lane.st.far : nullptr; gc.far_cnt[k] = far_part ? lane.far_cnt : nullptr;
                 }
                 a.series_of = lane.map[r & 1]; a.n_active = lane.cnt + (r % 3);
+                if (far_part) a.n_back = lane.far_cnt + 3 + (r % 3);
                 if (b->use_gather && lane.ybuf) {
                     if (emit && !grouped)
                         launch_gather_columns(a.y, ld, lane.map[r & 1], lane.cnt + (r % 3), (int)n, (int)b->t_max, lane.ybuf, lane.ybuf_cols, sq,
@@ -1095,6 +1110,7 @@
                     if (emit && grouped) {
                         const int k = gg.n_slots++;
                         gg.series_of[k] = lane.map[r & 1]; gg.n_active[k] = lane.cnt + (r % 3);
+                        gg.n_back[k] = a.n_back;
                         gg.out[k] = lane.ybuf; gg.ld_out[k] = lane.ybuf_cols; gg.cap[k] = (int)lane.ybuf_cols;
                         gg_cols = std::max(gg_cols, (int)std::min<size_t>(n, lane.ybuf_cols));
                     }
@@ -1196,11 +1212,13 @@
         hipStream_t sg = b->aux[group_stream[g]];
         if (r == 0) {
             int32_t *zero[GROUP_MAX_SLOTS] = {};
+            int32_t *far_zero[GROUP_MAX_SLOTS] = {};
             for (size_t k = 0; k < groups[g].size(); k++) zero[k] = b->lanes[groups[g][k] % (size_t)n_lanes].cnt;
-            launch_group_zero3((int)groups[g].size(), zero, sg);
-        }
-        gc = GroupCompactArgs{}; gc.n_series = (int)n;
-        gg = GroupGatherArgs{}; gg.t_max = (int)b->t_max; gg.elem_bytes = ybytes; gg.y = ybase; gg.ld = ld; gg_cols = 0;
+            for (size_t k = 0; k < groups[g].size(); k++) far_zero[k] = b->lanes[groups[g][k] % (size_t)n_lanes].far_cnt;
+            launch_group_zero3((int)groups[g].size(), zero, sg, far_zero);
+        }
+        gc = GroupCompactArgs{}; gc.n_series = (int)n; gc.round = r; gc.cap = (int)n;
+        gg = GroupGatherArgs{}; gg.map_cap = (int)n; gg.t_max = (int)b->t_max; gg.elem_bytes = ybytes; gg.y = ybase; gg.ld = ld; gg_cols = 0;
         for (size_t oi : groups[g]) enqueue_round(r, oi);
         if (gc.n_slots > 0) launch_group_compact(gc, sg);
         if (gg.n_slots > 0) launch_group_gather(gg, gg_cols, sg);
@@ -1573,6 +1591,7 @@
     b->last_stream = st;
     HIPCHECK(hipEventRecord(b->ev_start, st));
     if (b->d_lane_stats) HIPCHECK(hipMemsetAsync(b->d_lane_stats, 0, 2 * (size_t)b->n_slots_cap * sizeof(unsigned long long), st));
+    if (b->d_far_stats) HIPCHECK(hipMemsetAsync(b->d_far_stats, 0, 4 * sizeof(unsigned long long), st));
     if (!b->tun.wave_trace.empty() && b->n_slots_cap > 0) {
         constexpr size_t WAVE_TRACE_RECORDS = 4u << 20;
         if (!b->d_wave_trace) b->d_wave_trace = dalloc<unsigned long long>(4 + 4 * WAVE_TRACE_RECORDS);
@@ -2117,6 +2136,17 @@
     return true;
 }
 
+bool anofox_hip_batch_far_route_stats(AnofoxHipBatch *b, uint64_t out[4])
+{
+    if (!b || !out || !b->ran) return false;
+    DeviceGuard guard(b->dev);
+    if (hipEventSynchronize(b->ev_stop) != hipSuccess) return false;
+    unsigned long long c[4] = {0ull, 0ull, 0ull, 0ull};
+    if (b->d_far_stats && hipMemcpy(c, b->d_far_stats, sizeof c, hipMemcpyDeviceToHost) != hipSuccess) return false;
+    for (int i = 0; i < 4; i++) out[i] = c[i];
+    return true;
+}
+
 bool anofox_hip_batch_device_results(AnofoxHipBatch *b, void **d_yhat, void **d_lower, void **d_upper, void **d_model_code,
                                      void **d_status)
 {
diff --git a/anofox-forecast_amd/csrc/host_resources.hpp b/anofox-forecast_amd/csrc/host_resources.hpp
--- a/anofox-forecast_amd/csrc/host_resources.hpp
+++ b/anofox-forecast_amd/csrc/host_resources.hpp
@@ -43,6 +43,7 @@
     int prio_top = 0;
     int group_launch = 1;
     int group_split = 1;
+    int far_route = 0;
     int dm_head_rounds = 0;
     bool merge_periods = true;
     int part_threads = 16;
@@ -102,7 +103,7 @@
         if (kv.count("spec_below")) t.spec_below = t.spec_below_md = std::atoi(kv.at("spec_below").c_str());
         geti("spec_below_md", t.spec_below_md);
         geti("gather_cols", t.gather_cols);
-        geti("group_launch", t.group_launch); geti("group_split", t.group_split);
+        geti("group_launch", t.group_launch); geti("group_split", t.group_split); geti("far_route", t.far_route);
         geti("k4", t.k4); geti("dm_head_rounds", t.dm_head_rounds); geti("k4_top", t.k4_top); geti("k4_top_below", t.k4_top_below);
         if (kv.count("spec2_below")) t.spec2_below = t.spec2_below_md = std::atoi(kv.at("spec2_below").c_str());
         geti("spec2_below_md", t.spec2_below_md);
diff --git a/anofox-forecast_amd/csrc/kernels.hip b/anofox-forecast_amd/csrc/kernels.hip
--- a/anofox-forecast_amd/csrc/kernels.hip
+++ b/anofox-forecast_amd/csrc/kernels.hip
@@ -298,26 +298,50 @@
 __global__ __launch_bounds__(NM_BLOCK) void group_compact_kernel(const GroupCompactArgs g)
 {
     const int k = blockIdx.y;
-    if (g.n_clear[k] && blockIdx.x == 0 && threadIdx.x == 0) *g.n_clear[k] = 0;
+    const uint8_t *far = g.far[k];
+    int32_t *fc = g.far_cnt[k];
+    const int r3 = g.round % 3, rp3 = (g.round + 2) % 3, rn3 = (g.round + 1) % 3;
+    if (blockIdx.x == 0 && threadIdx.x == 0) {
+        if (g.n_clear[k]) *g.n_clear[k] = 0;
+        if (far) { fc[rn3] = 0; fc[3 + rn3] = 0; }
+    }
     const int n_prev = g.n_prev[k] ? *g.n_prev[k] : g.n_series;
     const int32_t *prev = g.prev[k], *done = g.done[k];
+    const int nb_prev = (far && prev) ? fc[3 + rp3] : 0;
     const int lane = threadIdx.x;
     for (int base0 = (int)blockIdx.x * NM_BLOCK; base0 < n_prev; base0 += (int)gridDim.x * NM_BLOCK) {
         const int idx = base0 + lane;
         int s = 0;
         bool keep = false;
         if (idx < n_prev) {
-            s = prev ? prev[idx] : idx;
+            s = prev ? prev[far_map_pos(idx, n_prev, nb_prev, g.cap)] : idx;
             keep = done[s] == 0;
         }
         const unsigned long long bal = __ballot(keep);
         const int cnt = __popcll(bal);
         if (cnt == 0) continue;
-        int base = 0;
-        if (lane == 0) base = atomicAdd(g.n_next[k], cnt);
-        base = __shfl(base, 0);
-        const int before = __popcll(bal & ((1ull << lane) - 1ull));
-        if (keep) g.next[k][base + before] = s;
+        if (!far) {
+            int base = 0;
+            if (lane == 0) base = atomicAdd(g.n_next[k], cnt);
+            base = __shfl(base, 0);
+            const int before = __popcll(bal & ((1ull << lane) - 1ull));
+            if (keep) g.next[k][base + before] = s;
+        } else {
+            const bool back = keep && far[s] != 0;
+            const unsigned long long balb = __ballot(back), balf = bal & ~balb;
+            const int cb = __popcll(balb), cf = cnt - cb;
+            int bf = 0, bb = 0;
+            if (lane == 0) {
+                atomicAdd(g.n_next[k], cnt);
+                if (cf) bf = atomicAdd(fc + r3, cf);
+                if (cb) bb = atomicAdd(fc + 3 + r3, cb);
+            }
+            bf = __shfl(bf, 0);
+            bb = __shfl(bb, 0);
+            const unsigned long long below = (1ull << lane) - 1ull;
+            if (back) g.next[k][g.cap - 1 - (bb + __popcll(balb & below))] = s;
+            else if (keep) g.next[k][bf + __popcll(balf & below)] = s;
+        }
     }
 }
 
@@ -328,18 +352,20 @@
     hipLaunchKernelGGL(group_compact_kernel, dim3(grid, g.n_slots), dim3(NM_BLOCK), 0, stream, g);
 }
 
-struct GroupZeroArgs { int32_t *p[GROUP_MAX_SLOTS]; };
+struct GroupZeroArgs { int32_t *p[GROUP_MAX_SLOTS]; int32_t *far_cnt[GROUP_MAX_SLOTS]; };
 __global__ void group_zero3_kernel(const int n, const GroupZeroArgs z)
 {
     const int i = threadIdx.x;
     if (i < 3 * n) z.p[i / 3][i % 3] = 0;
-}
-
-void launch_group_zero3(int n, int32_t *const *zero, hipStream_t stream)
+    for (int j = i; j < 6 * n; j += (int)blockDim.x)
+        if (z.far_cnt[j / 6]) z.far_cnt[j / 6][j % 6] = 0;
+}
+
+void launch_group_zero3(int n, int32_t *const *zero, hipStream_t stream, int32_t *const *far_cnt)
 {
     if (n <= 0) return;
     GroupZeroArgs z{};
-    for (int k = 0; k < n && k < GROUP_MAX_SLOTS; k++) z.p[k] = zero[k];
+    for (int k = 0; k < n && k < GROUP_MAX_SLOTS; k++) { z.p[k] = zero[k]; z.far_cnt[k] = far_cnt ? far_cnt[k] : nullptr; }
     hipLaunchKernelGGL(group_zero3_kernel, dim3(1), dim3(64), 0, stream, std::min(n, GROUP_MAX_SLOTS), z);
 }
 
@@ -353,9 +379,10 @@
     E *out = (E *)g.out[k];
     const size_t ld_out = g.ld_out[k];
     const int32_t *series_of = g.series_of[k];
+    const int n_back = g.n_back[k] ? *g.n_back[k] : 0;
     for (int p0 = (int)blockIdx.x * NM_BLOCK; p0 < n_act; p0 += (int)gridDim.x * NM_BLOCK) {
         const int p = p0 + (int)threadIdx.x;
-        const int s = series_of[p < n_act ? p : n_act - 1];
+        const int s = series_of[far_map_pos(p < n_act ? p : n_act - 1, n_act, n_back, g.map_cap)];
         for (int t0 = (int)blockIdx.y * GATHER_TB; t0 < g.t_max; t0 += (int)gridDim.y * GATHER_TB) {
             const int t1 = t0 + GATHER_TB < g.t_max ? t0 + GATHER_TB : g.t_max;
             for (int t = t0; t < t1; t++) out[(size_t)t * ld_out + p] = y[(size_t)t * g.ld + s];
diff --git a/anofox-forecast_amd/csrc/kernels.hpp b/anofox-forecast_amd/csrc/kernels.hpp
--- a/anofox-forecast_amd/csrc/kernels.hpp
+++ b/anofox-forecast_amd/csrc/kernels.hpp
@@ -40,7 +40,14 @@
     double *sim;
     double *fs;
     int32_t *phase, *evals, *iters, *passes, *done;
-};
+    uint8_t *far;
+};
+
+__host__ __device__ inline int far_map_pos(int p, int n_act, int n_back, int cap)
+{
+    const int n_front = n_act - n_back;
+    return p < n_front ? p : cap - 1 - (p - n_front);
+}
 
 struct FitArgs {
     const double *y; size_t ld; const int32_t *len; int n_series;
@@ -48,6 +55,10 @@
     const double *y_round; size_t ld_round;
     const int32_t *series_of;
     const int32_t *n_active;
+    const int32_t *n_back;
+    int map_cap;
+    int far_route;
+    unsigned long long *far_stats;
     int budget, first_round;
     const int32_t *m_col;
     int spec_below;
@@ -489,13 +500,17 @@
     int n_slots, n_series;
     const int32_t *prev[GROUP_MAX_SLOTS], *n_prev[GROUP_MAX_SLOTS], *done[GROUP_MAX_SLOTS];
     int32_t *next[GROUP_MAX_SLOTS], *n_next[GROUP_MAX_SLOTS], *n_clear[GROUP_MAX_SLOTS];
+    const uint8_t *far[GROUP_MAX_SLOTS];
+    int32_t *far_cnt[GROUP_MAX_SLOTS];
+    int round, cap;
 };
 void launch_group_compact(const GroupCompactArgs &g, hipStream_t);
-void launch_group_zero3(int n, int32_t *const *zero, hipStream_t);
+void launch_group_zero3(int n, int32_t *const *zero, hipStream_t, int32_t *const *far_cnt = nullptr);
 struct GroupGatherArgs {
     int n_slots, t_max, elem_bytes;
     const void *y; size_t ld;
     const int32_t *series_of[GROUP_MAX_SLOTS], *n_active[GROUP_MAX_SLOTS];
+    const int32_t *n_back[GROUP_MAX_SLOTS]; int map_cap;
     void *out[GROUP_MAX_SLOTS]; size_t ld_out[GROUP_MAX_SLOTS]; int cap[GROUP_MAX_SLOTS];
 };
 void launch_group_gather(const GroupGatherArgs &g, int n_cols_max, hipStream_t);
diff --git a/anofox-forecast_amd/csrc/nm.hpp b/anofox-forecast_amd/csrc/nm.hpp
--- a/anofox-forecast_amd/csrc/nm.hpp
+++ b/anofox-forecast_amd/csrc/nm.hpp
@@ -1,5 +1,6 @@
 #pragma once
 #include <hip/hip_runtime.h>
+#include <type_traits>
 
 namespace anofox {
 
@@ -15,8 +16,24 @@
 
 enum { NM_INIT0 = 0, NM_INIT1 = 1, NM_ITER = 2, NM_SHRINK = 3, NM_SEQ_INIT = 4, NM_SEQ_E = 5, NM_SEQ_OC = 6, NM_SEQ_IC = 7, NM_SEQ_SHRINK = 8 };
 
-struct NmRun { int phase; int evals; int iters; int passes; bool done; };
+struct NmRun {
+    int phase; int evals; int iters; int passes; bool done;
+    bool route_on, far_prone, far_seen;
+    int live, wp_guarded, wp_branchy, redo;
+};
 struct NmStats { int iters; int evals; int passes; };
+
+struct NmRoute { bool guarded, tripped, far; };
+template <class M, class = void> struct nm_far_route { static constexpr bool value = false; };
+template <class M> struct nm_far_route<M, std::void_t<decltype(M::FAR_ROUTE)>> { static constexpr bool value = M::FAR_ROUTE; };
+constexpr int NM_FAR_WINDOW = 40;
+
+__device__ __forceinline__ int nm_or4(int v)
+{
+    v |= __shfl_xor(v, 1);
+    v |= __shfl_xor(v, 2);
+    return v;
+}
 
 template <int D> constexpr int nm_lds_doubles() { return ((D + 1) * D + (D + 1)) * NM_BLOCK; }
 
@@ -149,6 +166,8 @@
     r.iters = 1;
     r.passes = 0;
     r.done = !active;
+    r.route_on = false; r.far_prone = true; r.far_seen = false;
+    r.live = 0; r.wp_guarded = 0; r.wp_branchy = 0; r.redo = 0;
 }
 
 template <class Model>
@@ -162,6 +181,10 @@
     int phase = r.phase, evals = r.evals, iters = r.iters, passes = r.passes;
     bool done = r.done, parked = false;
     double cand[NM_K][D], fc[NM_K];
+    constexpr bool FR = nm_far_route<Model>::value;
+    const bool far_prone = r.far_prone;
+    bool redo = false, far_seen = false;
+    int live_n = 0, n_redo = 0, wp_guarded = 0, wp_branchy = 0;
 
     for (int pass = 0;; pass++) {
         if (!done && !parked) {
@@ -194,11 +217,22 @@
         if (!done && pass >= budget && (phase == NM_ITER || phase == NM_INIT0)) parked = true;
         if (__all(done || parked)) break;
 
-        mdl.eval(cand, fc);
-        passes += (done || parked) ? 0 : 1;
+        const bool live = !(done || parked);
+        if constexpr (FR) {
+            NmRoute rt;
+            rt.guarded = r.route_on && !__any(live && (far_prone || redo));
+            rt.tripped = false; rt.far = false;
+            mdl.eval_routed(cand, fc, rt);
+            redo = live && nm_or4(rt.tripped ? 1 : 0) != 0;
+            if (live && (redo || nm_or4(rt.far ? 1 : 0) != 0)) far_seen = true;
+            live_n += live ? 1 : 0;
+            n_redo += redo ? 1 : 0;
+            if (rt.guarded) wp_guarded++; else wp_branchy++;
+        } else mdl.eval(cand, fc);
+        passes += (!live || redo) ? 0 : 1;
         nm_fence();
 
-        if (!done && !parked) {
+        if (live && !redo) {
             NmSimplex<D> S;
             nm_load<D>(st, lane, S);
             if (phase == NM_INIT0) {
@@ -251,6 +285,7 @@
         }
     }
     r.phase = phase; r.evals = evals; r.iters = iters; r.passes = passes; r.done = done;
+    if constexpr (FR) { r.far_seen = far_seen; r.live = live_n; r.redo = n_redo; r.wp_guarded = wp_guarded; r.wp_branchy = wp_branchy; }
 }
 
 template <int D> __device__ __forceinline__ void nm_hypothesis(int hh, int &P, int &j)
@@ -321,6 +356,9 @@
     int hp = 0, hj = 0;
     nm_hypothesis<D>(hh < NH ? hh : 0, hp, hj);
     double x[D];
+    constexpr bool FR = nm_far_route<Model>::value;
+    bool far_prone = r.far_prone, redo = false, far_seen = false, far_win = false;
+    int win = 0, live_n = 0, n_redo = 0, wp_guarded = 0, wp_branchy = 0;
 
     for (int pass = 0;; pass++) {
         if (!done && !parked) {
@@ -353,7 +391,22 @@
         if (!done && pass >= budget && (phase == NM_ITER || phase == NM_INIT0)) parked = true;
         if (done || parked) break;
 
-        const double f = mdl.eval1(x);
+        double f;
+        unsigned long long tripped = 0ull, far = 0ull;
+        if constexpr (FR) {
+            NmRoute rt;
+            rt.guarded = r.route_on && !__any(far_prone || redo);
+            rt.tripped = false; rt.far = false;
+            f = mdl.eval1_routed(x, rt);
+            tripped = __ballot(rt.tripped);
+            far = __ballot(rt.far);
+            redo = (tripped & 0xfull) != 0ull;
+            if (redo || (far & 0xfull) != 0ull) far_win = true;
+            live_n += 1;
+            n_redo += redo ? 1 : 0;
+            if (rt.guarded) wp_guarded++; else wp_branchy++;
+            if (redo) { nm_fence(); continue; }
+        } else f = mdl.eval1(x);
         passes += 1;
         nm_fence();
         double fc[NM_K];
@@ -362,6 +415,8 @@
 
         NmSimplex<D> S;
         nm_load<D>(st, lane, S);
+        const int evals0 = evals, iters0 = iters;
+        bool drop = false;
         if (phase == NM_INIT0) {
 #pragma unroll
             for (int k = 0; k < NM_K; k++)
@@ -391,8 +446,13 @@
                 for (int k = 0; k < NM_K; k++) fc2[k] = __shfl(f, NM_K + 4 * hstar + k);
                 nm_accept<D>(S, which, fnew, lo, hi);
                 iters += 1;
+                const unsigned second = NM_K + 4 * hstar < NM_BLOCK ? (unsigned)(NM_K + 4 * hstar) : 0u;
                 if (!(evals < maxfun && iters < maxiter) || nm_converged<D>(S)) done = true;
-                else if (NM_K + 4 * NH <= NM_BLOCK) {
+                else if (FR && ((tripped >> second) & 0xfull) != 0ull) {
+                    evals = evals0; iters = iters0; passes -= 1;
+                    redo = true; far_win = true; n_redo += 1; drop = true;
+                } else if (NM_K + 4 * NH <= NM_BLOCK) {
+                    if (FR && ((far >> second) & 0xfull) != 0ull) far_win = true;
                     if (!nm_decide<D>(S, fc2, evals, which, fnew)) {
                         nm_shrink_vertices<D>(S, lo, hi);
                         phase = NM_SHRINK;
@@ -411,9 +471,14 @@
             phase = NM_ITER;
             nm_sort_all<D>(S);
         }
+        if (drop) continue;
         nm_store<D>(st, lane, S);
+        if constexpr (FR) {
+            if (++win == NM_FAR_WINDOW) { far_prone = far_win; far_seen = far_seen || far_win; far_win = false; win = 0; }
+        }
     }
     r.phase = phase; r.evals = evals; r.iters = iters; r.passes = passes; r.done = done;
+    if constexpr (FR) { r.far_seen = far_seen || far_win; r.live = live_n; r.redo = n_redo; r.wp_guarded = wp_guarded; r.wp_branchy = wp_branchy; }
 }
 
 template <class Model>
@@ -429,6 +494,10 @@
     int vi = 0;
     double fxr = 0.0;
     double x[D];
+    constexpr bool FR = nm_far_route<Model>::value;
+    const bool far_prone = r.far_prone;
+    bool redo = false, far_seen = false;
+    int live_n = 0, n_redo = 0, wp_guarded = 0, wp_branchy = 0;
 
     for (int pass = 0;; pass++) {
         if (!done && !parked) {
@@ -454,11 +523,23 @@
         if (!done && pass >= budget && (phase == NM_ITER || phase == NM_INIT0)) parked = true;
         if (__all(done || parked)) break;
 
-        const double f = mdl.eval1(x);
-        passes += (done || parked) ? 0 : 1;
+        const bool live = !(done || parked);
+        double f;
+        if constexpr (FR) {
+            NmRoute rt;
+            rt.guarded = r.route_on && !__any(live && (far_prone || redo));
+            rt.tripped = false; rt.far = false;
+            f = mdl.eval1_routed(x, rt);
+            redo = live && rt.tripped;
+            if (live && (rt.tripped || rt.far)) far_seen = true;
+            live_n += live ? 1 : 0;
+            n_redo += redo ? 1 : 0;
+            if (rt.guarded) wp_guarded++; else wp_branchy++;
+        } else f = mdl.eval1(x);
+        passes += (!live || redo) ? 0 : 1;
         nm_fence();
 
-        if (!done && !parked) {
+        if (live && !redo) {
             if (phase == NM_SEQ_INIT || phase == NM_SEQ_SHRINK) {
                 const bool init = phase == NM_SEQ_INIT;
                 nm_store_set_f<D>(st, lane, init ? vi : 1 + vi, f);
@@ -508,6 +589,7 @@
         }
     }
     r.phase = phase; r.evals = evals; r.iters = iters; r.passes = passes; r.done = done;
+    if constexpr (FR) { r.far_seen = far_seen; r.live = live_n; r.redo = n_redo; r.wp_guarded = wp_guarded; r.wp_branchy = wp_branchy; }
 }
 
 template <class Model>
diff --git a/anofox-forecast_amd/device.py b/anofox-forecast_amd/device.py
--- a/anofox-forecast_amd/device.py
+++ b/anofox-forecast_amd/device.py
@@ -506,6 +506,14 @@
             out["by_spec"][name] = {"wave_passes": int(s.slot_wave_passes[k]), "lane_efficiency": eff(int(s.slot_live_lane_passes[k]), int(s.slot_wave_passes[k]))}
         return out
 
+    def far_route_stats(self) -> dict:
+        c = (C.c_uint64 * 4)()
+        if not self.L.anofox_hip_batch_far_route_stats(self.handle, c):
+            raise RuntimeError("anofox_hip_batch_far_route_stats failed")
+        g, o = int(c[0]), int(c[1])
+        return {"guarded_wave_passes": g, "branchy_wave_passes": o, "redo_lane_passes": int(c[2]), "flagged_problems": int(c[3]),
+                "guarded_share": round(g / (g + o), 4) if g + o else None}
+
     def results(self) -> dict:
         ptrs = [C.c_void_p() for _ in range(5)]
         self.L.anofox_hip_batch_device_results(self.handle, *[C.byref(p) for p in ptrs])
diff --git a/anofox-forecast_amd/lib.py b/anofox-forecast_amd/lib.py
--- a/anofox-forecast_amd/lib.py
+++ b/anofox-forecast_amd/lib.py
@@ -360,7 +360,7 @@
     "anofox_hip_batch_n_series", "anofox_hip_batch_periods", "anofox_hip_batch_set_fixed_params",
     "anofox_hip_set_devices", "anofox_hip_get_devices", "anofox_hip_set_min_series_per_device", "anofox_hip_shard_range",
     "anofox_hip_set_default_arima_method", "anofox_hip_batch_set_arima_method", "anofox_hip_release_caches",
-    "anofox_hip_batch_run_many", "anofox_hip_batch_lane_stats", "anofox_hip_selftest_recip",
+    "anofox_hip_batch_run_many", "anofox_hip_batch_lane_stats", "anofox_hip_batch_far_route_stats", "anofox_hip_selftest_recip",
     "anofox_ts_mstl_decomposition", "anofox_free_mstl_result", "anofox_hip_mstl_decompose_batch", "anofox_hip_mstl_decompose_device",
     "anofox_ts_forecast_exog", "anofox_ts_forecast_exog_batch", "anofox_hip_batch_set_exog_device", "anofox_hip_batch_exog_coefficients",
     "anofox_ts_detect_changepoints_bocpd", "anofox_free_bocpd_result", "anofox_hip_changepoints_batch", "anofox_hip_changepoints_device",
@@ -440,6 +440,8 @@
     L.anofox_hip_batch_stats.argtypes = [C.c_void_p, P(AnofoxHipStats)]
     L.anofox_hip_selftest_recip.restype = C.c_bool
     L.anofox_hip_selftest_recip.argtypes = [C.c_uint64, C.c_uint64, P(C.c_uint64), P(C.c_double)]
+    L.anofox_hip_batch_far_route_stats.restype = C.c_bool
+    L.anofox_hip_batch_far_route_stats.argtypes = [C.c_void_p, P(C.c_uint64)]
     L.anofox_hip_batch_lane_stats.restype = C.c_bool
     L.anofox_hip_batch_lane_stats.argtypes = [C.c_void_p, P(AnofoxHipLaneStats), C.c_size_t]
     L.anofox_hip_batch_device_results.restype = C.c_bool
diff --git a/include/anofox_fcst_hip.h b/include/anofox_fcst_hip.h
--- a/include/anofox_fcst_hip.h
+++ b/include/anofox_fcst_hip.h
@@ -1068,6 +1068,8 @@
 
 bool anofox_hip_batch_lane_stats(AnofoxHipBatch *batch, AnofoxHipLaneStats *out, size_t struct_size);
 
+bool anofox_hip_batch_far_route_stats(AnofoxHipBatch *batch, uint64_t out[4]);
+
 bool anofox_hip_batch_run(AnofoxHipBatch *batch, void *stream,
                           struct AnofoxError *out_error);
 
```

New measurement: 79190. 2.0% lower.
